# BaeHann/feature_level_style_transfer_for_TSC

Measured on AMD Instinct MI355X. Metric: train-step samples/sec (univariate TS, len=512, batch=256) at 1/2/4/8 MI355X, higher is better.
Workload: dtype bf16x3

## Files before the change

### feature_level_style_transfer_for_tsc_amd/_lib.py

```python
from __future__ import annotations

import ctypes
import os
from ctypes import POINTER, Structure, c_char_p, c_float, c_int, c_int32, c_int64, c_void_p
from typing import Optional

import torch

ABI_VERSION = 16
_LIB_NAME = "libfst_hip.so"
_HERE = os.path.dirname(os.path.abspath(__file__))
LIB_PATH = os.environ.get("FST_HIP_LIB", os.path.join(_HERE, _LIB_NAME))


class FstLibraryError(RuntimeError):
    pass


class WSrc(Structure):
    _fields_ = [("w", c_void_p), ("off0", c_int64), ("sm", c_int64), ("sc", c_int64), ("st", c_int64)]


_P = c_void_p
_I32P = c_void_p
_SIGNATURES = {
    "fst_version": (c_int, []),
    "fst_last_error": (c_char_p, []),
    "fst_pack_weights": (c_int, [_I32P, _I32P, c_int, POINTER(WSrc), POINTER(WSrc), c_int, c_int, c_int, c_int, _P, c_void_p]),
    "fst_pack_weights_bf16x3": (c_int, [_I32P, _I32P, c_int, POINTER(WSrc), POINTER(WSrc), c_int, c_int, c_int, c_int, _P, c_void_p]),
    "fst_unpack_weights": (c_int, [_I32P, _I32P, c_int, _P, c_int, _P, c_int64, c_int64, c_int64, c_int64,
                                   _P, c_int64, c_int64, c_int64, c_int64, c_int, c_void_p]),
    "fst_mask_taps": (c_int, [_P, _I32P, _I32P, c_int, c_int, c_int, c_void_p]),
    "fst_conv_gemm": (c_int, [_P, c_int64, _P, c_int64, _P, _I32P, _I32P, c_int, _P, _P, c_int64, _P, c_int64,
                              _P, c_int64, c_int, c_int, c_int, c_int, c_int, c_int, c_int, c_int, c_void_p]),
    "fst_conv_wgrad": (c_int, [_P, c_int64, _P, c_int64, _P, c_int64, _P, c_int64, c_int, _P, _I32P, _I32P, c_int,
                               c_int, c_int, c_int, c_int, c_int, c_int64, c_void_p]),
    "fst_conv_last_route": (c_int, [POINTER(c_int32)]),
    "fst_row_sum": (c_int, [_P, c_int64, c_int, c_int, c_int, _P, c_void_p]),
    "fst_bn_stats": (c_int, [_P, c_int, c_int, c_int, _P, c_int64, c_void_p]),
    "fst_bn_finalize": (c_int, [_P, c_int, _P, _P, _P, _P, c_int, c_int, c_float, c_float, _P, c_void_p]),
    "fst_bn_apply": (c_int, [_P, _P, _P, _P, _P, c_int, c_int, c_int, c_int, c_int64, c_void_p]),
    "fst_bn_bwd_reduce": (c_int, [_P, _P, _P, _P, c_int, c_int, c_int, c_int, _P, c_int64, c_void_p]),
    "fst_bn_bwd_apply": (c_int, [_P, _P, _P, _P, _P, c_int, _P, _P, _P, c_int, c_int, c_int, c_int, c_int, c_int, c_int64, c_void_p]),
    "fst_bn_bwd_reduce_join": (c_int, [_P, _P, _P, _P, _P, c_int, c_int, c_int, _P, _P, c_int64, c_void_p]),
    "fst_bn_bwd_apply_join": (c_int, [_P, _P, _P, _P, _P, _P, _P, c_int, _P, _P, _P, _P, _P, _P, c_int, c_int, c_int, c_int, c_int,
                                      c_int64, c_void_p]),
    "fst_gate_fwd": (c_int, [_P, _P, c_int, c_int, c_int, c_int64, c_void_p]),
    "fst_gate_bwd": (c_int, [_P, _P, _P, c_int, c_int, c_int, c_int64, c_void_p]),
    "fst_coupling_sum_slots": (c_int64, [c_int, c_int, c_int]),
    "fst_coupling_fwd": (c_int, [_P, _P, _P, c_int, c_int, c_int, c_int64, _P, c_void_p]),
    "fst_coupling_bwd": (c_int, [_P, _P, _P, _P, _P, _P, _P, _P, c_int, c_int, c_int, c_int64, c_void_p]),
    "fst_coupling_inv_fwd": (c_int, [_P, _P, _P, c_int, c_int, c_int, c_int64, c_void_p]),
    "fst_coupling_inv_bwd": (c_int, [_P, _P, _P, _P, _P, c_int, c_int, c_int, c_int64, c_void_p]),
    "fst_rmsprop_multi": (c_int, [_P, _P, _P, _P, _P, c_int, c_float, c_float, c_void_p]),
    "fst_adam_multi": (c_int, [_P, _P, _P, _P, _P, c_int, _P, c_float, c_float, c_float, c_float, c_void_p]),
    "fst_rmsprop_multi_dev": (c_int, [_P, _P, _P, _P, _P, c_int, c_float, c_float, c_void_p]),
    "fst_adam_multi_dev": (c_int, [_P, _P, _P, _P, _P, c_int, _P, _P, c_float, c_float, c_float, c_void_p]),
    "fst_wn_stack_fwd_ok": (c_int, [c_int, c_int, c_int, c_int]),
    "fst_wn_stack_fwd": (c_int, [_P, _P, _P, c_int64, _P, _P, _P, c_int64, _P, c_int, c_int, c_int, c_int, c_int, c_int64, c_void_p]),
    "fst_wn_stack_bwd_ok": (c_int, [c_int, c_int, c_int, c_int]),
    "fst_wn_stack_bwd": (c_int, [_P, _P, _P, _P, _P, _P, _P, _P, _P, c_int64, c_int, c_int, c_int, c_int, c_int, c_int64, c_void_p]),
    "fst_wn_wgrad_ok": (c_int, [c_int, c_int, c_int, c_int, c_int, c_int]),
    "fst_wn_wgrad_workspace_floats": (c_int64, [c_int, c_int, c_int, c_int, c_int, c_int]),
    "fst_wn_wgrad_in": (c_int, [_P, _P, _P, c_int, c_int64, _P, _P, _P, c_int64, c_int, c_int, c_int, c_int, c_int, c_int, c_int64,
                                c_void_p]),
    "fst_wn_wgrad_rs": (c_int, [_P, _P, _P, c_int, _P, _P, c_int64, c_int, c_int, c_int, c_int, c_int64, c_void_p]),
    "fst_nt_gemm_workspace_floats": (c_int64, [c_int, c_int, c_int]),
    "fst_nt_gemm": (c_int, [_P, _P, _P, _P, c_int64, c_int, c_int, c_int, _P, _P, c_int, c_float, _P, c_void_p]),
    "fst_tap_wgrad_ok": (c_int, [c_int, c_int, c_int, c_int, c_int, c_int, c_int]),
    "fst_tap_wgrad_workspace_floats": (c_int64, [c_int, c_int, c_int, c_int, c_int]),
    "fst_tap_wgrad": (c_int, [_P, _P, _P, _P, c_int64, c_int, c_int, c_int, c_int, c_int, c_int, c_int, c_int, c_int64, c_int64, c_void_p]),
    "fst_dense_tap_wgrad_ok": (c_int, [c_int, c_int, c_int, c_int, c_int, c_int]),
    "fst_dense_tap_wgrad_workspace_floats": (c_int64, [c_int, c_int, c_int, c_int, c_int]),
    "fst_dense_tap_wgrad": (c_int, [_P, _P, _P, _P, c_int64, c_int, c_int, c_int, c_int, c_int, c_int, c_int64, c_int64, c_void_p]),
    "fst_wn_last_route": (c_int, [POINTER(c_int32)]),
    "fst_relu_bwd": (c_int, [_P, _P, _P, c_int64, c_void_p]),
    "fst_gemm_workspace_floats": (c_int64, [c_int, c_int, c_int]),
    "fst_gemm": (c_int, [_P, c_int64, c_int, _P, c_int64, c_int, _P, c_int64, c_int, c_int, c_int, _P, c_int, c_float, _P, c_int64,
                         c_void_p]),
    "fst_act_bwd": (c_int, [_P, _P, _P, c_int64, c_float, c_void_p]),
    "fst_batch_sum": (c_int, [_P, _P, _P, c_int, c_int64, c_int, c_void_p]),
    "fst_noise_transfer_fwd": (c_int, [_P, c_int, c_int, _P, _P, c_float, c_float, _P, _P, _P, _P, _P, _P, _P, c_int, c_int, c_void_p]),
    "fst_bcast_add": (c_int, [_P, _P, _P, c_int, c_int64, c_void_p]),
    "fst_noise_transfer_bwd": (c_int, [_P, c_int, _P, _P, _P, _P, c_int, c_int, c_void_p]),
    "fst_noise_transfer_dw": (c_int, [_P, _P, _P, _P, c_int, c_int, c_void_p]),
    "fst_noise_transfer_bwd_apply": (c_int, [_P, _P, _P, _P, c_float, c_float, c_int, _P, _P, c_int64, c_void_p]),
    "fst_wn_fold_fwd": (c_int, [_P, c_int, _P, _P, c_void_p]),
    "fst_wn_fold_bwd": (c_int, [_P, c_int, _P, _P, _P, c_void_p]),
    "fst_logdet_inv": (c_int, [_P, c_int, _P, _P, c_void_p]),
    "fst_wn_image_bytes": (c_int64, [c_int, c_int]),
    "fst_wn_pack": (c_int, [_P, _P, _P, _P, _P, _P, c_int, c_int, c_int, c_int, _P, c_int64, c_void_p]),
    "fst_wn_layer_fwd": (c_int, [_P, c_int64, _P, c_int64, _P, c_int64, _P, _P, _P, _P, c_int, c_int, c_int, c_int, c_int, c_int,
                                 c_int, c_int64, c_void_p]),
    "fst_wn_bwd_image_bytes": (c_int64, [c_int, c_int]),
    "fst_wn_pack_bwd": (c_int, [_P, c_int, c_int, c_int, _P, c_int64, c_void_p]),
    "fst_wn_layer_bwd": (c_int, [_P, _P, _P, _P, c_int64, _P, _P, c_int64, c_int, c_int, c_int, c_int, c_int64, c_void_p]),
    "fst_wn_dgrad_image_bytes": (c_int64, [c_int]),
    "fst_wn_pack_dgrad": (c_int, [_P, _P, c_int, c_int, c_int, _P, c_int64, c_void_p]),
    "fst_wn_dgrad_fits": (c_int, [c_int, c_int, c_int]),
    "fst_wn_layer_dgrad": (c_int, [_P, _P, c_int64, _P, _P, _P, _P, c_int64, c_int, c_int, c_int, c_int, c_int, c_int64, c_int64,
                                   c_void_p]),
    "fst_gru_fwd": (c_int, [_P, _P, _P, _P, _P, _I32P, c_int, c_int, c_int, c_int, c_int64, c_void_p]),
    "fst_gru_bwd": (c_int, [_P, _P, _P, _P, _I32P, c_int, _P, _P, c_int, c_int, c_int, c_int64, c_void_p]),
    "fst_lstm2_fwd": (c_int, [_P, _P, _P, _P, c_int, c_int, c_int64, c_void_p]),
    "fst_lstm2_bwd": (c_int, [_P, _P, _P, _P, _P, c_int, c_int, c_int64, c_void_p]),
    "fst_axpy": (c_int, [_P, _P, c_float, c_int64, c_void_p]),
    "fst_add_slices": (c_int, [_P, c_int64, _P, c_int64, _P, c_int64, c_int, c_int, c_int, c_void_p]),
    "fst_cpc_workspace_floats": (c_int64, [c_int, c_int, c_int, c_int]),
    "fst_cpc_nce_slots": (c_int64, [c_int, c_int, c_int, c_int]),
    "fst_cpc_nce_fwd": (c_int, [_P, c_int64, c_int64, c_int64, _I32P, _P, c_int, c_int, c_int, c_int, c_int, _P, _P, _P, c_void_p]),
    "fst_cpc_nce_bwd": (c_int, [_P, c_int64, c_int64, c_int64, _I32P, _P, _P, c_int, c_int, c_int, c_int, c_int, _P, _P, _P,
                                c_void_p]),
}
EXPORTED_SYMBOLS = tuple(_SIGNATURES)

_lib: Optional[ctypes.CDLL] = None


def load(path: Optional[str] = None) -> ctypes.CDLL:
    global _lib
    if _lib is not None and path is None:
        return _lib
    p = path or LIB_PATH
    if not os.path.exists(p):
        raise FstLibraryError(
            f"{p} not found — build it with `python -c 'import __graft_entry__ as g; g.build()'` "
            "(hipcc --offload-arch=gfx950).  There is no CPU fallback.")
    try:
        lib = ctypes.CDLL(p)
    except OSError as e:
        raise FstLibraryError(f"cannot load {p}: {e}") from e
    for name, (res, args) in _SIGNATURES.items():
        try:
            fn = getattr(lib, name)
        except AttributeError as e:
            raise FstLibraryError(f"{p} does not export {name}; rebuild the library") from e
        fn.restype, fn.argtypes = res, args
    if lib.fst_version() != ABI_VERSION:
        raise FstLibraryError(f"{p}: ABI version {lib.fst_version()} != expected {ABI_VERSION}; rebuild")
    if path is None:
        _lib = lib
    return lib


def check(rc: int, what: str) -> None:
    if rc != 0:
        msg = load().fst_last_error()
        raise RuntimeError(f"{what} failed (rc={rc}): {msg.decode() if msg else '?'}")


def stream_ptr() -> int:
    return torch.cuda.current_stream().cuda_stream


def ptr(t: Optional[torch.Tensor]) -> Optional[int]:
    return None if t is None else t.data_ptr()


def require_gpu_tensor(t: torch.Tensor, name: str) -> None:
    if not t.is_cuda:
        raise FstLibraryError(f"{name} lives on {t.device}; the fst ops run on an MI355X only (no CPU fallback)")
    if t.dtype != torch.float32:
        raise TypeError(f"{name} must be float32, got {t.dtype}")
```

### feature_level_style_transfer_for_tsc_amd/csrc/wn_fused.hip

```cpp
#include "fst_device.h"
#include <type_traits>

#define WS_MAXL 10
#define WN_TN 128
#define WN_A_BYTES (8 * 2048)
#define WN_TILE_BYTES (32 * 36 * 4)
#define WN_FWD_LDS(NW) (3 * (WN_A_BYTES + 2 * (((NW) + 1) * 1024 + 128)))

__device__ __forceinline__ float wn_sigmoid(float x) {
  return __builtin_amdgcn_rcpf(1.0f + __builtin_amdgcn_exp2f(-1.44269504f * x));
}
__device__ __forceinline__ float wn_tanh(float x) {
  return 1.0f - 2.0f * __builtin_amdgcn_rcpf(1.0f + __builtin_amdgcn_exp2f(2.88539008f * x));
}

constexpr int WN_GRP = 2;
__host__ __device__ __forceinline__ void wn_stage_chunk_tap(int k, int CH, int& c, int& tap) {
  const int g = k / (3 * WN_GRP), rem = k - g * 3 * WN_GRP;
  const int gs = CH - g * WN_GRP < WN_GRP ? CH - g * WN_GRP : WN_GRP;
  tap = rem / gs;
  c = g * WN_GRP + rem - gs * tap;
}

struct WnPackParams {
  const float* in_w;
  const float* cond_w;
  const float* in_b;
  const float* cond_b;
  const float* rs_w;
  const float* rs_b;
  int n, h, last, CH, CH2;
  uint4* img;
};

__global__ __launch_bounds__(64) void wn_pack_kernel(WnPackParams p) {
  const int lane = threadIdx.x, blk = blockIdx.x & 7, st = blockIdx.x >> 3;
  const int S1 = 3 * p.CH + p.CH2, n = p.n, h = p.h;
  const int hh = lane >> 5, rowb = (blk & 3) * 32 + (lane & 31);
  const bool row_ok = rowb < n;
  float v[8];
  if (st < S1) {
    const int row = (blk < 4 ? 0 : n) + rowb;
#pragma unroll
    for (int j = 0; j < 8; ++j) {
      float w = 0.f;
      if (row_ok) {
        if (st < 3 * p.CH) {
          int cc, tap;
          wn_stage_chunk_tap(st, p.CH, cc, tap);
          const int c = cc * 16 + 8 * hh + j;
          if (c < n) w = p.in_w[((long long)row * n + c) * 3 + tap];
        } else {
          const int c = (st - 3 * p.CH) * 16 + 8 * hh + j;
          if (c < h) w = p.cond_w[(long long)row * h + c];
          else if (c == h) w = p.in_b[row] + p.cond_b[row];
        }
      }
      v[j] = w;
    }
  } else {
    const int ks = st - S1, kb = ks >> 1, s = ks & 1;
    const bool skip = blk >= 4;
    const bool live = row_ok && (!p.last || skip);
    const int row = (skip && !p.last ? n : 0) + rowb;
#pragma unroll
    for (int j = 0; j < 8; ++j) {
      const int k = kb * 32 + 16 * s + 8 * (j >> 2) + 4 * hh + (j & 3);
      float w = 0.f;
      if (live) {
        if (k < n) w = p.rs_w[(long long)row * n + k];
        else if (k == n) w = p.rs_b[row];
      }
      v[j] = w;
    }
  }
  unsigned hi[4], lo[4];
#pragma unroll
  for (int j = 0; j < 4; ++j) split_bf16_pair(v[2 * j], v[2 * j + 1], hi[j], lo[j]);
  uint4* dst = p.img + ((long long)st * 8 + blk) * 128 + lane;
  dst[0] = make_uint4(hi[0], hi[1], hi[2], hi[3]);
  dst[64] = make_uint4(lo[0], lo[1], lo[2], lo[3]);
  if (blockIdx.x == 0 && lane < 2) {
    const unsigned one = lane ? 0x3f800000u : 0u;
    p.img[(long long)(S1 + 8) * 8 * 128 + lane] = make_uint4(one, one, one, one);
  }
}

static inline int wn_ch(int n) { return (n + 15) / 16; }
static inline int wn_ch2(int h) { return (h + 1 + 15) / 16; }

extern "C" int64_t fst_wn_image_bytes(int n, int h) {
  if (n <= 0 || h <= 0) return -1;
  return (int64_t)(3 * wn_ch(n) + wn_ch2(h) + 8) * WN_A_BYTES + 32;
}

extern "C" int fst_wn_pack(const float* in_w, const float* cond_w, const float* in_b, const float* cond_b,
                           const float* rs_w, const float* rs_b, int n, int h, int ntaps, int last, void* image,
                           int64_t image_bytes, void* stream) {
  FST_REQUIRE(in_w && cond_w && in_b && cond_b && rs_w && rs_b && image, "fst_wn_pack: null operand");
  FST_REQUIRE(ntaps == 3, "fst_wn_pack: the fused WN kernels are 3-tap (in_w [2n][n][3]); got %d taps", ntaps);
  FST_REQUIRE(n > 0 && n < 128 && h > 0, "fst_wn_pack: needs 0 < n < 128 (one spare K row carries the bias), h > 0; n=%d h=%d", n, h);
  FST_REQUIRE(image_bytes == fst_wn_image_bytes(n, h), "fst_wn_pack: image is %lld bytes, expected %lld",
              (long long)image_bytes, (long long)fst_wn_image_bytes(n, h));
  FST_REQUIRE(fst_aligned16(image), "fst_wn_pack: image must be 16-byte aligned");
  WnPackParams p = {in_w, cond_w, in_b, cond_b, rs_w, rs_b, n, h, last ? 1 : 0, wn_ch(n), wn_ch2(h), static_cast<uint4*>(image)};
  const int stages = 3 * p.CH + p.CH2 + 8;
  hipLaunchKernelGGL(wn_pack_kernel, dim3((unsigned)(stages * 8)), dim3(64), 0, (hipStream_t)stream, p);
  FST_LAUNCH_CHECK();
  return 0;
}

#ifdef FST_STAMPS
__device__ unsigned long long wn_stamps[12];
extern "C" int fst_debug_wn_stamps(unsigned long long* out_host, int reset) { return fst_read_stamps(wn_stamps, out_host, reset); }
#endif

struct WnFwdParams {
  const float* a;
  long long a_bs;
  const float* u0;
  long long u0_bs;
  const char* img;
  float* ts;
  float* acts;
  float* a_next;
  float* out;
  int B, L, n, h, dil, first, last;
  int CH, CH2, tiles_per_seq, n_wg;
};

template <int MODE>
__device__ __forceinline__ void wn_store_tile(const float (&v)[16], float* tile, float* dst_rows, const float* res_rows,
                                              int rows_valid, int L, int t, int lane) {
  const int half = lane >> 5, l31 = lane & 31;
#pragma unroll
  for (int r = 0; r < 16; ++r) tile[((r & 3) + 8 * (r >> 2) + 4 * half) * 36 + l31] = v[r];
  const int rrow = lane >> 3, c4 = (lane & 7) * 4;
  const bool t_ok = t + c4 < L;
  float4 o[4], e[4];
#pragma unroll
  for (int j = 0; j < 4; ++j) {
    const int row = rrow + 8 * j;
    o[j] = *reinterpret_cast<const float4*>(tile + row * 36 + c4);
    e[j] = make_float4(0.f, 0.f, 0.f, 0.f);
    if (MODE != 0 && t_ok && row < rows_valid) {
      const float* src = (MODE == 1 ? res_rows : dst_rows) + (long long)row * L + t + c4;
      e[j] = *reinterpret_cast<const float4*>(src);
    }
  }
#pragma unroll
  for (int j = 0; j < 4; ++j) {
    const int row = rrow + 8 * j;
    if (t_ok && row < rows_valid) {
      float4 w = o[j];
      w.x += e[j].x; w.y += e[j].y; w.z += e[j].z; w.w += e[j].w;
      *reinterpret_cast<float4*>(dst_rows + (long long)row * L + t + c4) = w;
    }
  }
}

__device__ __forceinline__ void wn_fetch_tile(float4 (&q)[4], const float* src_rows, int rows_valid, int L, int t, int lane) {
  const int rrow = lane >> 3, c4 = (lane & 7) * 4;
  const bool t_ok = t + c4 < L;
#pragma unroll
  for (int j = 0; j < 4; ++j) {
    const int row = rrow + 8 * j;
    q[j] = make_float4(0.f, 0.f, 0.f, 0.f);
    if (t_ok && row < rows_valid) q[j] = *reinterpret_cast<const float4*>(src_rows + (long long)row * L + t + c4);
  }
}
__device__ __forceinline__ void wn_acc_load(f32x16& v, const float* src_rows, int rows_valid, int L, int t, int lane) {
  const int half = lane >> 5, l31 = lane & 31;
  const bool t_ok = t + l31 < L && src_rows != nullptr;
  const float* lp = src_rows + ((long long)(4 * half) * L + t + l31);
  const int rv = rows_valid - 4 * half;
#pragma unroll
  for (int r = 0; r < 16; ++r) {
    const int row = (r & 3) + 8 * (r >> 2);
    v[r] = (t_ok && row < rv) ? lp[(long long)row * L] : 0.f;
  }
}
__device__ __forceinline__ void wn_acc_store(const f32x16& v, float* dst_rows, int rows_valid, int L, int t, int lane) {
  const int half = lane >> 5, l31 = lane & 31;
  const bool t_ok = t + l31 < L;
  float* lp = dst_rows + ((long long)(4 * half) * L + t + l31);
  const int rv = rows_valid - 4 * half;
#pragma unroll
  for (int r = 0; r < 16; ++r) {
    const int row = (r & 3) + 8 * (r >> 2);
    if (t_ok && row < rv) lp[(long long)row * L] = v[r];
  }
}
__device__ __forceinline__ void wn_acc_store(const float (&v)[16], float* dst_rows, int rows_valid, int L, int t, int lane) {
  const int half = lane >> 5, l31 = lane & 31;
  const bool t_ok = t + l31 < L;
  float* lp = dst_rows + ((long long)(4 * half) * L + t + l31);
  const int rv = rows_valid - 4 * half;
#pragma unroll
  for (int r = 0; r < 16; ++r) {
    const int row = (r & 3) + 8 * (r >> 2);
    if (t_ok && row < rv) lp[(long long)row * L] = v[r];
  }
}
__device__ __forceinline__ void wn_tile_to_acc(float (&v)[16], const float4 (&q)[4], float* tile, int lane) {
  const int rrow = lane >> 3, c4 = (lane & 7) * 4, half = lane >> 5, l31 = lane & 31;
#pragma unroll
  for (int j = 0; j < 4; ++j) *reinterpret_cast<float4*>(tile + (rrow + 8 * j) * 36 + c4) = q[j];
#pragma unroll
  for (int r = 0; r < 16; ++r) v[r] = tile[((r & 3) + 8 * (r >> 2) + 4 * half) * 36 + l31];
}

#define WS_OOB 0x80000000u
__device__ __forceinline__ __amdgpu_buffer_rsrc_t ws_rsrc(const void* base) {
  return __builtin_amdgcn_make_buffer_rsrc(const_cast<void*>(base), 0, 0x40000000, 0x00020000);
}
struct WsLane { unsigned vo, vo_lo; };
__device__ __forceinline__ WsLane ws_lane(unsigned vlane, int tcol, int L, int lane) {
  WsLane w;
  w.vo = tcol + (lane & 31) < L ? vlane : WS_OOB;
  w.vo_lo = lane < 32 ? w.vo : WS_OOB;
  return w;
}
__device__ __forceinline__ int ws_opaque(int x) {
  asm volatile("" : "+s"(x));
  return x;
}
__device__ __forceinline__ void ws_acc_load(f32x16& v, __amdgpu_buffer_rsrc_t rs, const WsLane w, int row0, int tcol, int rv, int L) {
  L = ws_opaque(L);
  rv = ws_opaque(rv);
  const int sbase = (row0 * L + tcol) * 4;
  if (rv >= 32) {
#pragma unroll
    for (int r = 0; r < 16; ++r)
      v[r] = __builtin_bit_cast(float, __builtin_amdgcn_raw_buffer_load_b32(rs, w.vo, sbase + ((r & 3) + 8 * (r >> 2)) * L * 4, 0));
  } else {
#pragma unroll
    for (int r = 0; r < 16; ++r) {
      const int row = (r & 3) + 8 * (r >> 2);
      float x = 0.f;
      if (row < rv) x = __builtin_bit_cast(float, __builtin_amdgcn_raw_buffer_load_b32(rs, row + 4 < rv ? w.vo : w.vo_lo, sbase + row * L * 4, 0));
      v[r] = x;
    }
  }
}
template <class V>
__device__ __forceinline__ void ws_acc_store(const V& v, __amdgpu_buffer_rsrc_t rs, const WsLane w, int row0, int tcol, int rv, int L) {
  L = ws_opaque(L);
  rv = ws_opaque(rv);
  const int sbase = (row0 * L + tcol) * 4;
  if (rv >= 32) {
#pragma unroll
    for (int r = 0; r < 16; ++r)
      __builtin_amdgcn_raw_buffer_store_b32(__builtin_bit_cast(unsigned, (float)v[r]), rs, w.vo, sbase + ((r & 3) + 8 * (r >> 2)) * L * 4, 0);
  } else {
#pragma unroll
    for (int r = 0; r < 16; ++r) {
      const int row = (r & 3) + 8 * (r >> 2);
      if (row < rv)
        __builtin_amdgcn_raw_buffer_store_b32(__builtin_bit_cast(unsigned, (float)v[r]), rs, row + 4 < rv ? w.vo : w.vo_lo, sbase + row * L * 4, 0);
    }
// ... 224 lines not shown
#pragma unroll
    for (int mb = 0; mb < 8; ++mb) {
      if (mb + 1 < 8 && !(p.last && mb + 1 < 4)) a_frag(mb + 1);
      if (!(p.last && mb < 4)) mfma_bf3(acc[mb], fah[mb % 2], fal[mb % 2], bh2[ks], bl2[ks]);
      if (more && mb >= 4) {
        __builtin_amdgcn_sched_barrier(0);
        issue_piece(nxt, mb - 4);
        __builtin_amdgcn_sched_barrier(0);
      }
    }
    slot = slot == 2 ? 0 : slot + 1;
  }

  FST_T(tg2);
  FST_ACC(7, tg1, tg2);
#pragma unroll
  for (int blk = 0; blk < 4; ++blk) {
    const int rows_e = n - blk * 32;
    if (!p.last) ws_acc_store(acc[blk], an_rs, wl, blk * 32, tcol, rows_e, L);
    ws_acc_store(acc[blk + 4], out_rs, wl, blk * 32, tcol, rows_e, L);
  }
  FST_T(tg3);
  FST_ACC(8, tg2, tg3);
  FST_ACC(9, ts0, tg3);
  FST_FLUSH(wn_stamps);
}

template <int NW>
__global__ __launch_bounds__(64 * NW, NW == 4 ? 2 : 1) void wn_layer_fwd_kernel(WnFwdParams p) {
  extern __shared__ __attribute__((aligned(16))) float lds[];
  int wg = blockIdx.x;
  if ((p.n_wg & 7) == 0) wg = (wg & 7) * (p.n_wg >> 3) + (wg >> 3);
  const int b = wg / p.tiles_per_seq;
  const int t0 = (wg - b * p.tiles_per_seq) * (32 * NW);
  wn_fwd_tile<NW>(*(WnFwdArgs*)__builtin_amdgcn_kernarg_segment_ptr(), b, t0, reinterpret_cast<char*>(lds));
}

struct WnFwdStackParams {
  WnFwdParams layer[WS_MAXL];
  int nl;
};

__global__ __launch_bounds__(512, 1) void wn_stack_fwd_kernel(WnFwdStackParams ps_by_value) {
  extern __shared__ __attribute__((aligned(16))) float lds[];
  typedef const __attribute__((address_space(4))) WnFwdStackParams StackArgs;
  StackArgs& ps = *(StackArgs*)__builtin_amdgcn_kernarg_segment_ptr();
  (void)ps_by_value;
  char* const ldsb = reinterpret_cast<char*>(lds);
  const int B = ps.layer[0].B, passes = ps.layer[0].tiles_per_seq;
  for (int b = blockIdx.x; b < B; b += gridDim.x) {
    for (int layer = 0; layer < ps.nl; ++layer) {
      for (int pass = 0; pass < passes; ++pass) {
        WnFwdArgs* qp = &ps.layer[layer];
        asm volatile("" : "+s"(qp));
        wn_fwd_tile<8>(*qp, b, pass * 256, ldsb);
        wait_vmcnt<0>();
        __syncthreads();
      }
    }
  }
}

extern "C" int fst_wn_stack_fwd_ok(int n, int h, int L, int nl) {
  return n > 0 && n < 128 && h > 0 && L > 0 && L % 256 == 0 && nl >= 1 && nl <= WS_MAXL;
}

extern "C" int fst_wn_stack_fwd(const float* const* a_in, const int64_t* a_bs, const void* const* images, int64_t image_bytes,
                                float* const* ts, float* const* a_next, const float* u0, int64_t u0_bs, float* out, int nl, int B,
                                int L, int n, int h, int64_t numel_a, void* stream) {
  fst_wn_clear_route();
  FST_REQUIRE(a_in && a_bs && images && ts && a_next && u0 && out, "fst_wn_stack_fwd: null operand");
  FST_REQUIRE(fst_wn_stack_fwd_ok(n, h, L, nl) && B > 0, "fst_wn_stack_fwd: B=%d L=%d n=%d h=%d nl=%d (needs n < 128, L %% 256 == 0, "
              "1 <= nl <= %d)", B, L, n, h, nl, WS_MAXL);
  FST_REQUIRE((long long)B * n * L == (long long)numel_a, "fst_wn_stack_fwd: B*n*L = %d*%d*%d does not match the element count %lld "
              "of the [B, n, L] tensors", B, n, L, (long long)numel_a);
  FST_REQUIRE(image_bytes == fst_wn_image_bytes(n, h), "fst_wn_stack_fwd: images are %lld bytes, expected %lld",
              (long long)image_bytes, (long long)fst_wn_image_bytes(n, h));
  FST_REQUIRE(B == 1 || u0_bs >= (int64_t)h * L, "fst_wn_stack_fwd: batch stride of u0 smaller than a sample");
  FST_REQUIRE(u0_bs % 4 == 0 && fst_aligned16(u0) && fst_aligned16(out), "fst_wn_stack_fwd: needs 16-byte aligned tensors");
  WnFwdStackParams p = {};
  for (int i = 0; i < nl; ++i) {
    FST_REQUIRE(a_in[i] && images[i] && ts[i] && (a_next[i] || i == nl - 1), "fst_wn_stack_fwd: null operand of layer %d", i);
    FST_REQUIRE(a_bs[i] >= (int64_t)n * L && a_bs[i] % 4 == 0 && fst_aligned16(a_in[i]) && fst_aligned16(images[i]) && fst_aligned16(ts[i]) && fst_aligned16(a_next[i]),
                "fst_wn_stack_fwd: layer %d: batch stride %lld smaller than a sample, or an operand that is not 16-byte aligned", i,
                (long long)a_bs[i]);
    FST_REQUIRE(i == nl - 1 || a_in[i + 1] == a_next[i], "fst_wn_stack_fwd: the input of layer %d is not the a_next of layer %d",
                i + 1, i);
    WnFwdParams& q = p.layer[i];
    q.a = a_in[i]; q.a_bs = a_bs[i]; q.u0 = u0; q.u0_bs = u0_bs; q.img = static_cast<const char*>(images[i]);
    q.ts = ts[i]; q.acts = nullptr; q.a_next = i == nl - 1 ? nullptr : a_next[i]; q.out = out;
    q.B = B; q.L = L; q.n = n; q.h = h; q.dil = 1 << i; q.first = i == 0; q.last = i == nl - 1;
    q.CH = wn_ch(n); q.CH2 = wn_ch2(h); q.tiles_per_seq = L / 256; q.n_wg = 0;
  }
  p.nl = nl;
  const int cus = fst_cu_count_or(256);
  if (int rc = fst_allow_full_lds((const void*)wn_stack_fwd_kernel, "fst_wn_stack_fwd")) return rc;
  fst_wn_set_route(FST_WN_ROUTE_STACK_FWD, 8, 0, 0, 0, B < cus ? B : cus, 1, 1, L / 256, 3, nl, WN_FWD_LDS(8));
  hipLaunchKernelGGL(wn_stack_fwd_kernel, dim3((unsigned)(B < cus ? B : cus)), dim3(512), WN_FWD_LDS(8), (hipStream_t)stream, p);
  FST_LAUNCH_CHECK();
  return 0;
}

extern "C" int fst_wn_layer_fwd(const float* a, int64_t a_bs, const float* u0, int64_t u0_bs, const void* image,
                                int64_t image_bytes, float* ts, float* acts, float* a_next, float* out, int first, int last,
                                int B, int L, int n, int h, int dil, int64_t numel_a, void* stream) {
  fst_wn_clear_route();
  FST_REQUIRE(a && u0 && image && ts && out && (last || a_next), "fst_wn_layer_fwd: null operand");
  FST_REQUIRE(B > 0 && L > 0 && n > 0 && n < 128 && h > 0 && dil > 0, "fst_wn_layer_fwd: B=%d L=%d n=%d h=%d dil=%d (needs n < 128)",
              B, L, n, h, dil);
  FST_REQUIRE((long long)B * n * L == (long long)numel_a, "fst_wn_layer_fwd: B*n*L = %d*%d*%d does not match the element count %lld "
              "of the [B, n, L] tensors", B, n, L, (long long)numel_a);
  FST_REQUIRE(image_bytes == fst_wn_image_bytes(n, h), "fst_wn_layer_fwd: image is %lld bytes, expected %lld",
              (long long)image_bytes, (long long)fst_wn_image_bytes(n, h));
  FST_REQUIRE(B == 1 || (a_bs >= (int64_t)n * L && u0_bs >= (int64_t)h * L), "fst_wn_layer_fwd: batch stride smaller than a sample");
  FST_REQUIRE(L % 4 == 0 && a_bs % 4 == 0 && u0_bs % 4 == 0 && fst_aligned16(a) && fst_aligned16(u0) && fst_aligned16(image) && fst_aligned16(ts) && fst_aligned16(acts) &&
              fst_aligned16(a_next) && fst_aligned16(out), "fst_wn_layer_fwd: needs L %% 4 == 0 and 16-byte aligned tensors (L=%d)", L);
  WnFwdParams p;
  p.a = a; p.a_bs = a_bs; p.u0 = u0; p.u0_bs = u0_bs; p.img = static_cast<const char*>(image);
  p.ts = ts; p.acts = acts; p.a_next = a_next; p.out = out;
  p.B = B; p.L = L; p.n = n; p.h = h; p.dil = dil; p.first = first ? 1 : 0; p.last = last ? 1 : 0;
  p.CH = wn_ch(n); p.CH2 = wn_ch2(h);
  const int cus = fst_cu_count_or(256);
  const int nw = (L % 256 == 0 && (long long)B * (L / 256) >= cus) ? 8 : 4;
  const int tn = 32 * nw;
  p.tiles_per_seq = (L + tn - 1) / tn;
  p.n_wg = B * p.tiles_per_seq;
  if (nw == 8) {
    if (int rc = fst_allow_full_lds((const void*)wn_layer_fwd_kernel<8>, "fst_wn_layer_fwd")) return rc;
    fst_wn_set_route(FST_WN_ROUTE_LAYER_FWD, 8, 0, 0, 0, p.n_wg, 1, 1, p.tiles_per_seq, 3, 1, WN_FWD_LDS(8));
    hipLaunchKernelGGL(wn_layer_fwd_kernel<8>, dim3((unsigned)p.n_wg), dim3(512), WN_FWD_LDS(8), (hipStream_t)stream, p);
  } else {
    if (int rc = fst_allow_full_lds((const void*)wn_layer_fwd_kernel<4>, "fst_wn_layer_fwd")) return rc;
    fst_wn_set_route(FST_WN_ROUTE_LAYER_FWD, 4, 0, 0, 0, p.n_wg, 1, 1, p.tiles_per_seq, 3, 1, WN_FWD_LDS(4));
    hipLaunchKernelGGL(wn_layer_fwd_kernel<4>, dim3((unsigned)p.n_wg), dim3(256), WN_FWD_LDS(4), (hipStream_t)stream, p);
  }
  FST_LAUNCH_CHECK();
  return 0;
}

constexpr int WN_BWD_OCC = 2;
#define WN_BW_NB 4
#define WN_BW_GS (WN_BW_NB * 1024 + 128)
#define WN_BW_A (4 * 2048)
#define WN_BW_SLOT (WN_BW_A + 2 * WN_BW_GS)
#define WN_BW_LDS (3 * WN_BW_SLOT)

struct WnPackBwdParams {
  const float* rs_w;
  int n, last, CH;
  uint4* img;
  int acc_order;
};

__global__ __launch_bounds__(64) void wn_pack_bwd_kernel(WnPackBwdParams p) {
  const int lane = threadIdx.x, blk = blockIdx.x & 3, st = blockIdx.x >> 2;
  const int n = p.n, hh = lane >> 5, m = blk * 32 + (lane & 31);
  const int src = p.last ? 0 : st / p.CH, c = st - src * p.CH;
  float v[8];
#pragma unroll
  for (int j = 0; j < 8; ++j) {
    const bool perm = p.acc_order && !p.last && src == 0;
    const int ch = 16 * c + (perm ? 8 * (j >> 2) + 4 * hh + (j & 3) : 8 * hh + j);
    v[j] = (m < n && ch < n) ? p.rs_w[(long long)(src * n + ch) * n + m] : 0.f;
  }
  unsigned hi[4], lo[4];
#pragma unroll
  for (int j = 0; j < 4; ++j) split_bf16_pair(v[2 * j], v[2 * j + 1], hi[j], lo[j]);
  uint4* dst = p.img + ((long long)st * 4 + blk) * 128 + lane;
  dst[0] = make_uint4(hi[0], hi[1], hi[2], hi[3]);
  dst[64] = make_uint4(lo[0], lo[1], lo[2], lo[3]);
  if (blockIdx.x == 0 && lane == 0) p.img[(long long)gridDim.x * 128] = make_uint4(0u, 0u, 0u, 0u);
}

extern "C" int64_t fst_wn_bwd_image_bytes(int n, int last) {
  if (n <= 0) return -1;
  return (int64_t)(last ? 1 : 2) * wn_ch(n) * WN_BW_A + 16;
}

extern "C" int fst_wn_pack_bwd(const float* rs_w, int n, int last, int acc_order, void* image, int64_t image_bytes, void* stream) {
  FST_REQUIRE(rs_w && image && n > 0 && n <= 128, "fst_wn_pack_bwd: bad arguments (n=%d, needs n <= 128)", n);
  FST_REQUIRE(image_bytes == fst_wn_bwd_image_bytes(n, last), "fst_wn_pack_bwd: image is %lld bytes, expected %lld",
              (long long)image_bytes, (long long)fst_wn_bwd_image_bytes(n, last));
  FST_REQUIRE(fst_aligned16(image), "fst_wn_pack_bwd: image must be 16-byte aligned");
  WnPackBwdParams p = {rs_w, n, last ? 1 : 0, wn_ch(n), static_cast<uint4*>(image), acc_order ? 1 : 0};
  const int stages = (last ? 1 : 2) * p.CH;
  hipLaunchKernelGGL(wn_pack_bwd_kernel, dim3((unsigned)(stages * 4)), dim3(64), 0, (hipStream_t)stream, p);
  FST_LAUNCH_CHECK();
  return 0;
}

struct WnBwdParams {
  const float* d_a;
  const float* d_out;
  const float* ts;
  const char* img;
  float* dg;
  float* row_sums;
  int B, L, n, last, CH, tiles_per_seq, n_wg;
};

__device__ __forceinline__ void wn_bwd_multiply(f32x16 (&acc)[4], const char* base, int lane, bf16x8 bh, bf16x8 bl) {
#pragma unroll
  for (int mb = 0; mb < 4; ++mb) {
    bf16x8 ah, al;
    lds_read_a_frag(base, mb, lane, ah, al);
    mfma_bf3(acc[mb], ah, al, bh, bl);
  }
}

__device__ __forceinline__ void wn_reduce_row_sums(const float* rsum, int R, float* out, int stride, int col, int tid) {
  __syncthreads();
  if (tid < R) {
    float s8 = 0.f;
#pragma unroll
    for (int w = 0; w < 8; ++w) s8 += rsum[w * R + tid];
    out[(long long)tid * stride + col] = s8;
  }
}

__global__ __launch_bounds__(256, WN_BWD_OCC) void wn_layer_bwd_kernel(WnBwdParams p) {
  extern __shared__ __attribute__((aligned(16))) float lds[];
  char* const ldsb = reinterpret_cast<char*>(lds);
  const int tid = threadIdx.x, lane = tid & 63;
  const int half = lane >> 5, l31 = lane & 31;
  const int wave_s = __builtin_amdgcn_readfirstlane(tid >> 6);
  int wg = blockIdx.x;
  if ((p.n_wg & 7) == 0) wg = (wg & 7) * (p.n_wg >> 3) + (wg >> 3);
  const int b = wg / p.tiles_per_seq;
  const int t0 = (wg - b * p.tiles_per_seq) * WN_TN;
  const int wave_n0 = wave_s * 32;
  const int L = p.L, n = p.n, CH = p.CH;
  const int S3 = (p.last ? 1 : 2) * CH;
  const char* const zero16 = p.img + (long long)S3 * WN_BW_A;
  const float* const ts_b = p.ts + (long long)b * (2 * n) * L;
  const int tcol = t0 + wave_n0;

  auto issue = [&](int k, int slot) {
    char* const sl = ldsb + slot * WN_BW_SLOT;
    const char* asrc = p.img + (long long)k * WN_BW_A;
    const bool from_da = !p.last && k < CH;
    const int c = from_da ? k : k - (p.last ? 0 : CH);
    const float* xb = (from_da ? p.d_a : p.d_out) + ((long long)b * n + 16 * c) * L;
    const int c_count = min(16, n - 16 * c);
#pragma unroll
    for (int i = 0; i < 4; ++i) {
      const int idx = wave_s + 4 * i;
      if (idx < 8) {
        lds_dma16(asrc + idx * 1024 + lane * 16, sl + idx * 1024);
      } else {
        const int bi = idx - 8;
        const int gq = bi >> 2, m = bi & 3;
        const int row = 8 * gq + (lane >> 3);
        const int t = t0 + 32 * m + 4 * (lane & 7);
        const bool ok = row < c_count && t < L;
        const char* src = ok ? reinterpret_cast<const char*>(xb + ((long long)row * L + t)) : zero16;
        lds_dma16(src, sl + WN_BW_A + gq * WN_BW_GS + m * 1024);
      }
    }
  };

  f32x16 acc[4];
#pragma unroll
  for (int mb = 0; mb < 4; ++mb)
#pragma unroll
    for (int r = 0; r < 16; ++r) acc[mb][r] = 0.f;

  float4 qt[4], qs[4];
  wn_fetch_tile(qt, ts_b, n, L, tcol, lane);
  wn_fetch_tile(qs, ts_b + (long long)n * L, n, L, tcol, lane);
  asm volatile("" ::: "memory");
  issue(0, 0);
  if (S3 > 1) issue(1, 1);
  int slot = 0;
  for (int k = 0; k < S3; ++k) {
    if (k + 1 < S3) wait_vmcnt<4>(); else wait_vmcnt<0>();
    __builtin_amdgcn_s_barrier();
    if (k + 2 < S3) issue(k + 2, slot >= 1 ? slot - 1 : 2);
    const char* base = ldsb + slot * WN_BW_SLOT;
    const int colx = wave_n0 + l31;
    const char* bp = base + WN_BW_A + half * WN_BW_GS + (colx >> 5) * 1024 + (colx & 31) * 4;
    float v[8];
#pragma unroll
    for (int j = 0; j < 8; ++j) v[j] = *reinterpret_cast<const float*>(bp + j * 128);
    bf16x8 bh, bl;
    split_bf16x8(v, bh, bl);
    wn_bwd_multiply(acc, base, lane, bh, bl);
    slot = slot == 2 ? 0 : slot + 1;
  }
  __syncthreads();
  float* const tile = reinterpret_cast<float*>(ldsb + wave_s * WN_TILE_BYTES);
  float* const rsum = reinterpret_cast<float*>(ldsb + 4 * WN_TILE_BYTES);
  float* const rsum_w = rsum + wave_s * 256;
  if (p.row_sums) {
#pragma unroll
    for (int w = 0; w < 4; ++w) rsum[w * 256 + tid] = 0.f;
    __syncthreads();
  }
  float* const dg_b = p.dg + (long long)b * (2 * n) * L;
#pragma unroll
  for (int blk = 0; blk < 4; ++blk) {
    const int rows_valid = n - blk * 32;
    float tv[16], sv[16], gt[16], gs[16];
    wn_tile_to_acc(tv, qt, tile, lane);
    wn_tile_to_acc(sv, qs, tile, lane);
    if (blk < 3) {
      wn_fetch_tile(qt, ts_b + (long long)((blk + 1) * 32) * L, n - (blk + 1) * 32, L, tcol, lane);
      wn_fetch_tile(qs, ts_b + (long long)(n + (blk + 1) * 32) * L, n - (blk + 1) * 32, L, tcol, lane);
    }
#pragma unroll
    for (int r = 0; r < 16; ++r) {
      const float d = acc[blk][r], t = tv[r], s = sv[r];
      gt[r] = d * s * (1.f - t * t);
      gs[r] = d * t * s * (1.f - s);
    }
    wn_store_tile<0>(gt, tile, dg_b + (long long)(blk * 32) * L, nullptr, rows_valid, L, tcol, lane);
    if (p.row_sums) wn_tile_row_sums(tile, rsum_w, blk * 32, rows_valid, L, tcol, lane);
    wn_store_tile<0>(gs, tile, dg_b + (long long)(n + blk * 32) * L, nullptr, rows_valid, L, tcol, lane);
    if (p.row_sums) wn_tile_row_sums(tile, rsum_w, n + blk * 32, rows_valid, L, tcol, lane);
  }
  if (p.row_sums) {
    __syncthreads();
    p.row_sums[(long long)tid * p.n_wg + wg] = (rsum[tid] + rsum[256 + tid]) + (rsum[512 + tid] + rsum[768 + tid]);
  }
}

extern "C" int fst_wn_layer_bwd(const float* d_a, const float* d_out, const float* ts, const void* image, int64_t image_bytes,
                                float* dg, float* row_sums, int64_t row_sums_rows, int last, int B, int L, int n,
                                int64_t numel_a, void* stream) {
  fst_wn_clear_route();
  FST_REQUIRE(d_out && ts && image && dg && (last || d_a), "fst_wn_layer_bwd: null operand");
  FST_REQUIRE(B > 0 && L > 0 && n > 0 && n <= 128, "fst_wn_layer_bwd: B=%d L=%d n=%d (needs n <= 128)", B, L, n);
  FST_REQUIRE((long long)B * n * L == (long long)numel_a, "fst_wn_layer_bwd: B*n*L = %d*%d*%d does not match the element count %lld "
              "of the [B, n, L] tensors", B, n, L, (long long)numel_a);
  FST_REQUIRE(image_bytes == fst_wn_bwd_image_bytes(n, last), "fst_wn_layer_bwd: image is %lld bytes, expected %lld",
              (long long)image_bytes, (long long)fst_wn_bwd_image_bytes(n, last));
  FST_REQUIRE(L % 4 == 0 && fst_aligned16(d_a) && fst_aligned16(d_out) && fst_aligned16(ts) && fst_aligned16(image) && fst_aligned16(dg),
              "fst_wn_layer_bwd: needs L %% 4 == 0 and 16-byte aligned tensors (L=%d)", L);
  WnBwdParams p;
  p.d_a = last ? nullptr : d_a; p.d_out = d_out; p.ts = ts; p.img = static_cast<const char*>(image); p.dg = dg;
  p.row_sums = row_sums;
  p.B = B; p.L = L; p.n = n; p.last = last ? 1 : 0; p.CH = wn_ch(n);
  p.tiles_per_seq = (L + WN_TN - 1) / WN_TN;
  p.n_wg = B * p.tiles_per_seq;
  FST_REQUIRE(row_sums == nullptr || row_sums_rows == p.n_wg, "fst_wn_layer_bwd: row_sums has %lld rows, the launch has %d "
              "workgroups (B x ceil(L/128))", (long long)row_sums_rows, p.n_wg);
  if (int rc = fst_allow_full_lds((const void*)wn_layer_bwd_kernel, "fst_wn_layer_bwd")) return rc;
  fst_wn_set_route(FST_WN_ROUTE_LAYER_BWD, 0, 0, 0, 0, p.n_wg, 1, 1, p.tiles_per_seq, 3, 1, WN_BW_LDS);
  hipLaunchKernelGGL(wn_layer_bwd_kernel, dim3((unsigned)p.n_wg), dim3(256), WN_BW_LDS, (hipStream_t)stream, p);
  FST_LAUNCH_CHECK();
  return 0;
}

#define DG_NCB 2
#define DG_TN (8 * 32 * DG_NCB)
#define DG_A_BLOCKS 13
#define DG_A_BYTES (DG_A_BLOCKS * 2048)

struct WnPackDgradParams {
  const float* in_w;
  const float* cond_w;
  int n, h, CHK;
  uint4* img;
};

__global__ __launch_bounds__(64) void wn_pack_dgrad_kernel(WnPackDgradParams p) {
  const int lane = threadIdx.x, ab = blockIdx.x % DG_A_BLOCKS, c = blockIdx.x / DG_A_BLOCKS;
  const int n = p.n, h = p.h, hh = lane >> 5, l31 = lane & 31;
  int tap, blk;
  if (ab < 4) { tap = 0; blk = ab; } else if (ab < 9) { tap = 1; blk = ab - 4; } else { tap = 2; blk = ab - 9; }
  float v[8];
#pragma unroll
  for (int j = 0; j < 8; ++j) {
    const int k = 16 * c + 8 * hh + j;
    float w = 0.f;
    if (k < 2 * n) {
      if (blk < 4) {
        const int m = blk * 32 + l31;
        if (m < n) w = p.in_w[((long long)k * n + m) * 3 + tap];
      } else {
        if (l31 < h) w = p.cond_w[(long long)k * h + l31];
      }
    }
    v[j] = w;
  }
  unsigned hi[4], lo[4];
#pragma unroll
  for (int j = 0; j < 4; ++j) split_bf16_pair(v[2 * j], v[2 * j + 1], hi[j], lo[j]);
  uint4* dst = p.img + (long long)blockIdx.x * 128 + lane;
  dst[0] = make_uint4(hi[0], hi[1], hi[2], hi[3]);
  dst[64] = make_uint4(lo[0], lo[1], lo[2], lo[3]);
  if (blockIdx.x == 0 && lane == 0) p.img[(long long)gridDim.x * 128] = make_uint4(0u, 0u, 0u, 0u);
}

extern "C" int64_t fst_wn_dgrad_image_bytes(int n) {
  if (n <= 0) return -1;
  return (int64_t)((2 * n + 15) / 16) * DG_A_BYTES + 16;
}

extern "C" int fst_wn_pack_dgrad(const float* in_w, const float* cond_w, int n, int h, int ntaps, void* image, int64_t image_bytes,
                                 void* stream) {
  FST_REQUIRE(in_w && cond_w && image && n > 0 && n <= 128 && h > 0 && h <= 32, "fst_wn_pack_dgrad: needs n <= 128, h <= 32 (n=%d h=%d)", n, h);
  FST_REQUIRE(ntaps == 3, "fst_wn_pack_dgrad: the fused WN kernels are 3-tap (in_w [2n][n][3]); got %d taps", ntaps);
  FST_REQUIRE(image_bytes == fst_wn_dgrad_image_bytes(n), "fst_wn_pack_dgrad: image is %lld bytes, expected %lld",
              (long long)image_bytes, (long long)fst_wn_dgrad_image_bytes(n));
  FST_REQUIRE(fst_aligned16(image), "fst_wn_pack_dgrad: image must be 16-byte aligned");
  WnPackDgradParams p = {in_w, cond_w, n, h, (2 * n + 15) / 16, static_cast<uint4*>(image)};
  hipLaunchKernelGGL(wn_pack_dgrad_kernel, dim3((unsigned)(p.CHK * DG_A_BLOCKS)), dim3(64), 0, (hipStream_t)stream, p);
  FST_LAUNCH_CHECK();
  return 0;
}

__device__ __forceinline__ void wn_dgrad_issue(char* sl, const char* img, const float* dg_b, int c, int t0, int n, int L, int dil,
                                               int nblkw, int gsw, int wave_s, int lane) {
  const char* asrc = img + (long long)c * DG_A_BYTES;
  const char* const zero16 = img + (long long)((2 * n + 15) / 16) * DG_A_BYTES;
  const float* xb = dg_b + (long long)(16 * c) * L;
  const int c_count = min(16, 2 * n - 16 * c);
  const int w4 = (t0 - dil) & ~3;
  const int NI = DG_A_BLOCKS * 2 + 2 * nblkw;
  for (int idx = wave_s; idx < NI; idx += 8) {
    if (idx < 2 * DG_A_BLOCKS) {
      lds_dma16(asrc + idx * 1024 + lane * 16, sl + idx * 1024);
    } else {
      const int bi = idx - 2 * DG_A_BLOCKS;
      const int gq = bi >= nblkw ? 1 : 0, m = bi - gq * nblkw;
      const int row = 8 * gq + (lane >> 3);
      const int t = w4 + 32 * m + 4 * (lane & 7);
      const bool ok = row < c_count && t >= 0 && t < L;
      const char* src = ok ? reinterpret_cast<const char*>(xb + ((long long)row * L + t)) : zero16;
      lds_dma16(src, sl + DG_A_BYTES + gq * gsw + m * 1024);
    }
  }
}

__device__ __forceinline__ void wn_dgrad_stage(f32x16 (&acc)[5][DG_NCB], const char* base, int gsw, int wave_n0, int dil, int sub,
                                               int lane) {
  const int half = lane >> 5, l31 = lane & 31;
#pragma unroll
  for (int tap = 0; tap < 3; ++tap) {
    bf16x8 bh[DG_NCB], bl[DG_NCB];
#pragma unroll
    for (int cb = 0; cb < DG_NCB; ++cb) {
      const int colx = wave_n0 + 32 * cb + l31 + (2 - tap) * dil + sub;
      const char* bp = base + DG_A_BYTES + half * gsw + (colx >> 5) * 1024 + (colx & 31) * 4;
      float v8[8];
#pragma unroll
      for (int j = 0; j < 8; ++j) v8[j] = *reinterpret_cast<const float*>(bp + j * 128);
      split_bf16x8(v8, bh[cb], bl[cb]);
    }
    const char* ab = base + (tap == 0 ? 0 : (tap == 1 ? 4 : 9)) * 2048;
#pragma unroll
    for (int mb = 0; mb < 5; ++mb) {
      if (mb == 4 && tap != 1) continue;
      bf16x8 ah, al;
      lds_read_a_frag(ab, mb, lane, ah, al);
#pragma unroll
      for (int cb = 0; cb < DG_NCB; ++cb) mfma_bf3(acc[mb][cb], ah, al, bh[cb], bl[cb]);
    }
  }
}

struct WnDgradParams {
  const float* dg;
  const char* img;
  const float* d_a;
  float* d_a_new;
  float* d_u0;
  long long d_u0_bs;
  float* row_sums;
  int B, L, n, h, dil, CHK, tiles_per_seq, n_wg;
  int nblkw;
  int gsw;
  int slot;
  int ns;
};

template <int N>
__device__ __forceinline__ void wn_wait_sw(int n) {
  if (n == N) { wait_vmcnt<N>(); return; }
  if constexpr (N > 0) wn_wait_sw<N - 1>(n);
}

__global__ __launch_bounds__(512, 2) void wn_layer_dgrad_kernel(WnDgradParams p) {
  extern __shared__ __attribute__((aligned(16))) float lds[];
  char* const ldsb = reinterpret_cast<char*>(lds);
  const int tid = threadIdx.x, lane = tid & 63;
  const int half = lane >> 5, l31 = lane & 31;
  const int wave_s = __builtin_amdgcn_readfirstlane(tid >> 6);
  const int wave_n0 = wave_s * (32 * DG_NCB);
  const int L = p.L, n = p.n, CHK = p.CHK, dil = p.dil;
  const int NI = DG_A_BLOCKS * 2 + 2 * p.nblkw;
  const int my_pieces = (NI - wave_s + 7) >> 3;
  const int depth = p.ns - 1;

  auto tile_of = [&](int v, int& b, int& t0) {
    int wg = v;
    if ((p.n_wg & 7) == 0) wg = (wg & 7) * (p.n_wg >> 3) + (wg >> 3);
    b = wg / p.tiles_per_seq;
    t0 = (wg - b * p.tiles_per_seq) * DG_TN;
    return wg;
  };
  auto issue = [&](int b, int t0, int c, int slot) {
    wn_dgrad_issue(ldsb + slot * p.slot, p.img, p.dg + (long long)b * (2 * n) * L, c, t0, n, L, dil, p.nblkw, p.gsw, wave_s, lane);
  };

  int first_slot = 0;
  for (int v = blockIdx.x; v < p.n_wg; v += gridDim.x) {
    int b, t0;
    const int wg = tile_of(v, b, t0);
    const int sub = (t0 - dil) & 3;
    f32x16 acc[5][DG_NCB];
#pragma unroll
    for (int mb = 0; mb < 5; ++mb)
#pragma unroll
      for (int cb = 0; cb < DG_NCB; ++cb) {
        const float* src = mb < 4 ? (p.d_a ? p.d_a + ((long long)b * n + mb * 32) * L : nullptr) : p.d_u0 + (long long)b * p.d_u0_bs;
        const int rows = mb < 4 ? (p.d_a ? n - mb * 32 : 0) : p.h;
        wn_acc_load(acc[mb][cb], src, rows, L, t0 + wave_n0 + 32 * cb, lane);
      }
    if (first_slot == 0)
      for (int d = 0; d < depth && d < CHK; ++d) issue(b, t0, d, d);

    int slot = first_slot;
    for (int c = 0; c < CHK; ++c) {
      const int newer = min(depth - 1, CHK - 1 - c);
      wn_wait_sw<16>(newer * my_pieces);
      __builtin_amdgcn_s_barrier();
      if (c + depth < CHK) issue(b, t0, c + depth, (slot + depth) % p.ns);
      wn_dgrad_stage(acc, ldsb + slot * p.slot, p.gsw, wave_n0, dil, sub, lane);
      slot = slot + 1 == p.ns ? 0 : slot + 1;
    }
    __syncthreads();
    if (v + (int)gridDim.x < p.n_wg) {
      int bn, tn;
      tile_of(v + gridDim.x, bn, tn);
      for (int d = 0; d < depth && d < CHK; ++d) issue(bn, tn, d, 1 + d);
      first_slot = 1;
    }
    float* const tile = reinterpret_cast<float*>(ldsb + wave_s * WN_TILE_BYTES);
    float* const rsum = reinterpret_cast<float*>(ldsb + 8 * WN_TILE_BYTES);
    float* const rsum_w = rsum + wave_s * 128;
    if (p.row_sums) {
      rsum[tid] = 0.f; rsum[512 + tid] = 0.f;
      __syncthreads();
    }
#pragma unroll
    for (int k = 0; k < 5 * DG_NCB; ++k) {
      const int i = k / DG_NCB, cb = k % DG_NCB, tcol = t0 + wave_n0 + 32 * cb;
      float* dst = i < 4 ? p.d_a_new + ((long long)b * n + i * 32) * L : p.d_u0 + (long long)b * p.d_u0_bs;
      const int rows = i < 4 ? n - i * 32 : p.h;
      wn_acc_store(acc[i][cb], dst, rows, L, tcol, lane);
      if (p.row_sums && i < 4) {
#pragma unroll
        for (int r = 0; r < 16; ++r) tile[((r & 3) + 8 * (r >> 2) + 4 * half) * 36 + l31] = acc[i][cb][r];
        wn_tile_row_sums(tile, rsum_w, i * 32, rows, L, tcol, lane);
      }
    }
    if (p.row_sums) wn_reduce_row_sums(rsum, 128, p.row_sums, p.n_wg, wg, tid);
  }
}
// ... 349 lines not shown
```

### feature_level_style_transfer_for_tsc_amd/csrc/wn_wgrad.hip

```cpp
#include <stdlib.h>
#include <type_traits>

#include "fst_device.h"

#define WW_TT 32
#define WW_MROWS 256
#define WW_ND 3
#define WW_NX 2
#define WW_MAX_NX 5

__device__ __attribute__((aligned(16))) float ww_zero16[4] = {0.f, 0.f, 0.f, 0.f};

#define WW_MAX_SETS 3
struct WwSeg {
  const float* ptr[WW_MAX_SETS];
  long long bs;
  long long mul_off;
  int rows, shift;
  int out, out_off, out_sc, out_sm;
};

struct WwParams {
  WwSeg dy[2];
  WwSeg x[4];
// ... 239 lines not shown
      const int nxu = (p.xr * 4 > 512 + tid) ? 2 : 1;
#pragma unroll
      for (int i = 0; i < 2; ++i) {
        const int r = r0 + 128 * i;
        da[i][0] = dw + ww_lds_off(r, 2 * u); da[i][1] = dw + ww_lds_off(r, 2 * u + 1);
        d[i][0] = ww_lds_read16(ww_lds_addr(da[i][0])); d[i][1] = ww_lds_read16(ww_lds_addr(da[i][1]));
        xa[i][0] = xw + ww_lds_off(r, 2 * u); xa[i][1] = xw + ww_lds_off(r, 2 * u + 1);
        if (i < nxu && r < p.xr) {
          xq[i][0] = ww_lds_read16(ww_lds_addr(xa[i][0])); xq[i][1] = ww_lds_read16(ww_lds_addr(xa[i][1]));
          if constexpr (MUL) {
            xm[i][0] = ww_lds_read16(ww_lds_addr(xa[i][0] + (p.xr << 7))); xm[i][1] = ww_lds_read16(ww_lds_addr(xa[i][1] + (p.xr << 7)));
          }
        }
      }
      ww_lds_wait();
#pragma unroll
      for (int i = 0; i < 2; ++i) {
        const int r = r0 + 128 * i;
        if constexpr (NE > 0)
          ev[i] += (d[i][0].x * e0.x + d[i][0].y * e0.y) + (d[i][0].z * e0.z + d[i][0].w * e0.w) +
                   (d[i][1].x * e1.x + d[i][1].y * e1.y) + (d[i][1].z * e1.z + d[i][1].w * e1.w);
        u32x4 h4, l4;
        ww_split8u(d[i][0], d[i][1], h4, l4);
        ww_lds_write16(ww_lds_addr(da[i][0]), h4); ww_lds_write16(ww_lds_addr(da[i][1]), l4);
        if (i < nxu && r < p.xr) {
          if constexpr (MUL) { xq[i][0] *= xm[i][0]; xq[i][1] *= xm[i][1]; }
          ww_split8u(xq[i][0], xq[i][1], h4, l4);
          ww_lds_write16(ww_lds_addr(xa[i][0]), h4); ww_lds_write16(ww_lds_addr(xa[i][1]), l4);
        }
      }
      asm volatile("s_waitcnt lgkmcnt(0)" ::: "memory");
    }
    __builtin_amdgcn_s_barrier();
#pragma unroll
    for (int ks = 0; ks < 2; ++ks) {
      f32x4 araw[MT][2], braw[KT][2];
#pragma unroll
      for (int i = 0; i < MT; ++i) {
        const char* ap = dsl + a_off + ((i * 32) << 7);
        araw[i][0] = ww_lds_read16(ww_lds_addr(ap + pc[ks][0]));
        araw[i][1] = ww_lds_read16(ww_lds_addr(ap + pc[ks][1]));
      }
#pragma unroll
      for (int j = 0; j < KT; ++j) {
        const char* bp = xsl + x_off + ((j * 32) << 7);
        braw[j][0] = ww_lds_read16(ww_lds_addr(bp + pc[ks][0]));
        braw[j][1] = ww_lds_read16(ww_lds_addr(bp + pc[ks][1]));
      }
      ww_lds_wait();
      issue_pos(5 * ks);
#pragma unroll
      for (int j = 0; j < KT; ++j) {
        if (FULL || wk * KT + j < k_blocks_here) {
          const bf16x8 bh = __builtin_bit_cast(bf16x8, braw[j][0]), bl = __builtin_bit_cast(bf16x8, braw[j][1]);
#pragma unroll
          for (int i = 0; i < MT; ++i) {
            if (!FULL && wm * MT + i >= m_blocks) break;
            const bf16x8 ah = __builtin_bit_cast(bf16x8, araw[i][0]), al = __builtin_bit_cast(bf16x8, araw[i][1]);
            mfma_bf3(acc[i][j], ah, al, bh, bl);
          }
        }
        issue_pos(5 * ks + 1 + j);
      }
      if constexpr (KT < 3) issue_pos(5 * ks + 3);
      issue_pos(5 * ks + 4);
    }
    dslot = dslot == WW_ND - 1 ? 0 : dslot + 1;
    xslot ^= 1;
  }

  float* const slab = p.slab + (long long)blockIdx.x * WW_MROWS * p.Kcols;
#pragma unroll
  for (int i = 0; i < MT; ++i) {
    if (wm * MT + i >= m_blocks) break;
#pragma unroll
    for (int j = 0; j < KT; ++j) {
      if (wk * KT + j >= k_blocks_here) break;
      float* dst = slab + (long long)((wm * MT + i) * 32 + 4 * half) * p.Kcols + g * p.xr + (wk * KT + j) * 32 + l31;
#pragma unroll
      for (int r = 0; r < 16; ++r) dst[(long long)((r & 3) + 8 * (r >> 2)) * p.Kcols] = acc[i][j][r];
    }
  }
  if (do_extra) {
#pragma unroll
    for (int i = 0; i < 2; ++i) {
      float sv = ev[i];
      sv += __shfl_xor(sv, 1, 64);
      sv += __shfl_xor(sv, 2, 64);
      if ((tid & 3) == 0) p.slab_extra[((long long)blockIdx.x * WW_MROWS + (tid >> 2) + 128 * i) * 2] = sv;
    }
  }
}

__device__ __forceinline__ void ww_scatter(const WwParams& p, int m, int kk, float v) {
  int si = 0, c = kk;
#pragma unroll
  for (int j = 0; j < 3; ++j)
    if (si + 1 < p.n_x && c >= p.x[si].rows) { c -= p.x[si].rows; ++si; }
  int out = p.x[0].out, off = p.x[0].out_off, sc = p.x[0].out_sc, sm = p.x[0].out_sm;
  if (si == 1) { out = p.x[1].out; off = p.x[1].out_off; sc = p.x[1].out_sc; sm = p.x[1].out_sm; }
  if (si == 2) { out = p.x[2].out; off = p.x[2].out_off; sc = p.x[2].out_sc; sm = p.x[2].out_sm; }
  if (si == 3) { out = p.x[3].out; off = p.x[3].out_off; sc = p.x[3].out_sc; sm = p.x[3].out_sm; }
  float* w = out == 0 ? p.w[0] : p.w[1];
  const long long at = (long long)m * sm + (long long)c * sc + off;
  if (p.epi_p) {
    float sd = 0.f;
    for (int j = 0; j < p.epi_ncls; ++j) sd += p.epi_p[m * p.epi_ncls + j] * p.epi_r1[(long long)j * sm + c];
    if (p.epi_raw) p.epi_raw[at] = v;
    v = v * p.epi_scale * sd;
  }
  w[at] = v;
}

__global__ __launch_bounds__(256) void wn_wgrad_reduce_kernel(WwParams p) {
  __shared__ float4 part[4][64];
  const int m = blockIdx.y, cx = threadIdx.x & 63, sg = threadIdx.x >> 6;
  const int kk0 = blockIdx.x * 256 + cx * 4;
  float4 s = make_float4(0.f, 0.f, 0.f, 0.f);
  if (kk0 < p.Kcols) {
    const long long st = (long long)WW_MROWS * p.Kcols;
    const float* q = p.slab + (long long)m * p.Kcols + kk0;
    int sl = sg;
    for (; sl + 28 < p.ksplit; sl += 32) {
      float4 v[8];
#pragma unroll
      for (int u = 0; u < 8; ++u) v[u] = *reinterpret_cast<const float4*>(q + (sl + 4 * u) * st);
#pragma unroll
      for (int u = 0; u < 8; ++u) { s.x += v[u].x; s.y += v[u].y; s.z += v[u].z; s.w += v[u].w; }
    }
    for (; sl < p.ksplit; sl += 4) {
      const float4 v = *reinterpret_cast<const float4*>(q + sl * st);
      s.x += v.x; s.y += v.y; s.z += v.z; s.w += v.w;
    }
  }
  part[sg][cx] = s;
  __syncthreads();
  if (sg == 0 && kk0 < p.Kcols) {
    float4 t = part[0][cx];
#pragma unroll
    for (int g2 = 1; g2 < 4; ++g2) { const float4 o = part[g2][cx]; t.x += o.x; t.y += o.y; t.z += o.z; t.w += o.w; }
    const float tv[4] = {t.x, t.y, t.z, t.w};
#pragma unroll
    for (int j = 0; j < 4; ++j)
      if (kk0 + j < p.K_main) ww_scatter(p, m, kk0 + j, tv[j]);
  }
  if (blockIdx.x == gridDim.x - 1 && sg == 1 && cx < p.n_extra && p.K_main < p.K) {
    const float* q = p.slab_extra + (long long)m * 2 + cx;
    float e = 0.f;
    for (int sl = 0; sl < p.ksplit; ++sl) e += q[(long long)sl * WW_MROWS * 2];
    ww_scatter(p, m, p.K_main + cx, e);
  }
}


static thread_local int32_t g_wn_route[FST_WN_ROUTE_LEN] = {0};

void fst_wn_set_route(int family, int t1, int t2, int t3, int t4, int gx, int gy, int gz, int a8, int a9, int a10, int lds) {
  const int32_t r[FST_WN_ROUTE_LEN] = {family, t1, t2, t3, t4, gx, gy, gz, a8, a9, a10, lds};
  for (int i = 0; i < FST_WN_ROUTE_LEN; ++i) g_wn_route[i] = r[i];
}

extern "C" int fst_wn_last_route(int32_t out[FST_WN_ROUTE_LEN]) {
  FST_REQUIRE(out != nullptr, "fst_wn_last_route: null output");
  for (int i = 0; i < FST_WN_ROUTE_LEN; ++i) out[i] = g_wn_route[i];
  return g_wn_route[0] != 0 ? 0 : -1;
}

static int ww_geometry(int kind, int B, int L, int n, int h, int last, int n_sets, WwParams* p) {
  const int KT = kind == 0 ? 3 : 2;
  p->M = kind == 0 ? 2 * n : (last ? n : 2 * n);
  p->K = kind == 0 ? 3 * n + h : n;
  const int rem = p->K & 31;
  p->n_extra = (kind == 0 && rem == 1) ? 1 : 0;
  p->K_main = p->n_extra ? p->K - rem : p->K;
  p->xr = 32 * 2 * KT;
  const int kb = (p->K_main + 31) / 32;
  p->n_groups = (kb + 2 * KT - 1) / (2 * KT);
  p->mul = kind == 1;
  p->RX = p->xr * (1 + p->mul) + (p->n_extra ? 8 : 0);
  p->Kcols = p->n_groups * p->xr;
  p->B = B; p->L = L;
  p->tiles_per_seq = L / WW_TT;
  p->n_tiles = B * p->tiles_per_seq;
  const int cus = fst_cu_count_or(256);
  int ks = cus / p->n_groups;
  if (ks > p->n_tiles * n_sets) ks = p->n_tiles * n_sets;
  if (ks < n_sets) ks = n_sets;
  p->ksplit = ks;
  p->n_sets = n_sets;
  return KT;
}

extern "C" int fst_wn_wgrad_ok(int kind, int B, int L, int n, int h, int dil) {
  if (!(B > 0 && L > 0 && L % WW_TT == 0 && n > 0 && n < 128)) return 0;
  if (kind == 0) {
    if (!(h > 0 && h <= 32 && dil > 0 && (3 * n + h + 31) / 32 <= 18)) return 0;
    return dil % 4 == 0 ? 1 : (dil < 4 ? 2 : 0);
  }
  return kind == 1;
}

extern "C" int64_t fst_wn_wgrad_workspace_floats(int kind, int B, int L, int n, int h, int last) {
  if (!fst_wn_wgrad_ok(kind, B, L, n, h, 4)) return -1;
  WwParams p;
  ww_geometry(kind, B, L, n, h, last, WW_MAX_SETS, &p);
  return (int64_t)p.ksplit * WW_MROWS * (p.Kcols + 2);
}

static int ww_launch(WwParams& p, int KT, void* stream, bool reduce = true) {
  const size_t lds = (size_t)WW_ND * WW_MROWS * 128 + (size_t)WW_NX * p.RX * 128;
  FST_REQUIRE(lds <= 160 * 1024 && (p.RX >> 3) <= 8 * WW_MAX_NX, "fst_wn_wgrad: %d staged k-rows per stage do not fit (LDS %zu B)", p.RX, lds);
  const bool full = (p.M + 31) / 32 == 8 && ((p.K_main + 31) / 32) % (2 * KT) == 0;
  void (*fn)(WwParams);
  if (KT == 3) {
    if (p.n_extra) fn = full ? wn_wgrad_kernel<2, 3, true, false, 1> : wn_wgrad_kernel<2, 3, false, false, 1>;
    else fn = full ? wn_wgrad_kernel<2, 3, true, false, 0> : wn_wgrad_kernel<2, 3, false, false, 0>;
  } else if (p.mul) {
    fn = full ? wn_wgrad_kernel<2, 2, true, true, 0> : wn_wgrad_kernel<2, 2, false, true, 0>;
  } else {
    fn = full ? wn_wgrad_kernel<2, 2, true, false, 0> : wn_wgrad_kernel<2, 2, false, false, 0>;
  }
  if (int rc = fst_allow_full_lds((const void*)fn, "fst_wn_wgrad")) return rc;
  fst_wn_set_route(FST_WN_ROUTE_WGRAD, KT, (int)full, p.mul, p.n_extra, p.ksplit, p.n_groups, 1, p.n_sets, p.misaligned, (int)reduce, (int)lds);
  hipLaunchKernelGGL(fn, dim3((unsigned)p.ksplit, (unsigned)p.n_groups), dim3(512), lds, (hipStream_t)stream, p);
  FST_LAUNCH_CHECK();
  if (!reduce) return 0;
  hipLaunchKernelGGL(wn_wgrad_reduce_kernel, dim3((unsigned)((p.Kcols + 255) / 256), (unsigned)p.M), dim3(256), 0, (hipStream_t)stream, p);
  FST_LAUNCH_CHECK();
  return 0;
}

extern "C" int fst_wn_wgrad_in(const float* const* dg, const float* const* a, const float* const* u0, int n_sets, int64_t u0_bs,
                               float* dw_in, float* dw_cond, float* workspace, int64_t workspace_floats, int B, int L, int n, int h,
                               int dil, int a_slack, int64_t numel_a, void* stream) {
  fst_wn_clear_route();
  FST_REQUIRE(dg && a && u0 && dw_in && dw_cond && workspace, "fst_wn_wgrad_in: null operand");
  FST_REQUIRE(n_sets >= 1 && n_sets <= WW_MAX_SETS, "fst_wn_wgrad_in: %d operand sets (1..%d)", n_sets, WW_MAX_SETS);
  const int served = fst_wn_wgrad_ok(0, B, L, n, h, dil);
  FST_REQUIRE(served == 1 || (served == 2 && a_slack), "fst_wn_wgrad_in: unsupported shape B=%d L=%d n=%d h=%d dil=%d (needs L %% 32 == 0, "
              "n < 128, h <= 32, and dil %% 4 == 0 or — with 16 readable bytes either side of a — dil < 4)", B, L, n, h, dil);
  FST_REQUIRE((long long)B * n * L == (long long)numel_a, "fst_wn_wgrad_in: B*n*L does not match the element count %lld of a", (long long)numel_a);
  FST_REQUIRE(B == 1 || u0_bs >= (int64_t)h * L, "fst_wn_wgrad_in: u0 batch stride %lld < h*L", (long long)u0_bs);
  FST_REQUIRE(u0_bs % 4 == 0 && fst_aligned16(workspace), "fst_wn_wgrad_in: operands must be 16-byte aligned");
  WwParams p = {};
  const int KT = ww_geometry(0, B, L, n, h, 0, n_sets, &p);
  FST_REQUIRE(workspace_floats >= (int64_t)p.ksplit * WW_MROWS * (p.Kcols + 2), "fst_wn_wgrad_in: workspace of %lld floats is too small",
              (long long)workspace_floats);
  p.n_dy = 1;
  p.dy[0] = {{}, (long long)2 * n * L, 0, 2 * n, 0, 0, 0, 0, 0};
  p.n_x = 4;
  for (int tap = 0; tap < 3; ++tap) p.x[tap] = {{}, (long long)n * L, 0, n, (tap - 1) * dil, 0, tap, 3, 3 * n};
  p.x[3] = {{}, (long long)u0_bs, 0, h, 0, 1, 0, 1, h};
  for (int s = 0; s < n_sets; ++s) {
    FST_REQUIRE(dg[s] && a[s] && u0[s], "fst_wn_wgrad_in: null operand in set %d", s);
    FST_REQUIRE(fst_aligned16(dg[s]) && fst_aligned16(a[s]) && fst_aligned16(u0[s]), "fst_wn_wgrad_in: operands must be 16-byte aligned");
    p.dy[0].ptr[s] = dg[s];
    for (int tap = 0; tap < 3; ++tap) p.x[tap].ptr[s] = a[s];
    p.x[3].ptr[s] = u0[s];
  }
  p.misaligned = dil % 4 != 0;
  p.slab = workspace;
  p.slab_extra = workspace + (long long)p.ksplit * WW_MROWS * p.Kcols;
  p.w[0] = dw_in; p.w[1] = dw_cond;
  return ww_launch(p, KT, stream);
}

extern "C" int fst_wn_wgrad_rs(const float* const* d_a, const float* const* d_out, const float* const* ts, int n_sets, float* dw_rs,
                               float* workspace, int64_t workspace_floats, int last, int B, int L, int n, int64_t numel_a,
                               void* stream) {
  fst_wn_clear_route();
  FST_REQUIRE(d_out && ts && dw_rs && workspace && (last || d_a), "fst_wn_wgrad_rs: null operand");
  FST_REQUIRE(n_sets >= 1 && n_sets <= WW_MAX_SETS, "fst_wn_wgrad_rs: %d operand sets (1..%d)", n_sets, WW_MAX_SETS);
  FST_REQUIRE(fst_wn_wgrad_ok(1, B, L, n, 0, 4), "fst_wn_wgrad_rs: unsupported shape B=%d L=%d n=%d (needs L %% 32 == 0, n < 128)", B, L, n);
  FST_REQUIRE((long long)B * n * L == (long long)numel_a, "fst_wn_wgrad_rs: B*n*L does not match the element count %lld", (long long)numel_a);
  FST_REQUIRE(fst_aligned16(workspace), "fst_wn_wgrad_rs: operands must be 16-byte aligned");
  WwParams p = {};
  const int KT = ww_geometry(1, B, L, n, 0, last, n_sets, &p);
  FST_REQUIRE(workspace_floats >= (int64_t)p.ksplit * WW_MROWS * (p.Kcols + 2), "fst_wn_wgrad_rs: workspace of %lld floats is too small",
              (long long)workspace_floats);
  p.n_dy = last ? 1 : 2;
  p.dy[0] = {{}, (long long)n * L, 0, n, 0, 0, 0, 0, 0};
  p.dy[1] = {{}, (long long)n * L, 0, n, 0, 0, 0, 0, 0};
  p.n_x = 1;
  p.x[0] = {{}, (long long)2 * n * L, (long long)n * L, n, 0, 0, 0, 1, n};
  for (int s = 0; s < n_sets; ++s) {
    FST_REQUIRE(d_out[s] && ts[s] && (last || d_a[s]), "fst_wn_wgrad_rs: null operand in set %d", s);
    FST_REQUIRE(fst_aligned16(d_out[s]) && fst_aligned16(ts[s]) && (last || fst_aligned16(d_a[s])), "fst_wn_wgrad_rs: operands must be 16-byte aligned");
    if (last) p.dy[0].ptr[s] = d_out[s];
    else { p.dy[0].ptr[s] = d_a[s]; p.dy[1].ptr[s] = d_out[s]; }
    p.x[0].ptr[s] = ts[s];
  }
  p.slab = workspace;
  p.slab_extra = workspace + (long long)p.ksplit * WW_MROWS * p.Kcols;
  p.w[0] = dw_rs; p.w[1] = nullptr;
  return ww_launch(p, KT, stream);
}

extern "C" int64_t fst_nt_gemm_workspace_floats(int M, int N, int K) {
  if (!(M > 0 && M <= WW_MROWS && N > 0 && K > 0 && K % WW_TT == 0)) return -1;
  const int n_groups = ((N + 31) / 32 + 3) / 4;
  const int cus = fst_cu_count_or(256);
  int ks = cus / n_groups;
  if (ks > K / WW_TT) ks = K / WW_TT;
  if (ks < 1) ks = 1;
  return (int64_t)ks * WW_MROWS * (n_groups * 128 + 2);
}

extern "C" int fst_nt_gemm(const float* A, const float* Bm, float* C, float* workspace, int64_t workspace_floats, int M, int N, int K,
                           const float* epi_p, const float* epi_r1, int epi_ncls, float epi_scale, float* epi_raw, void* stream) {
  fst_wn_clear_route();
  FST_REQUIRE(A && Bm && C && workspace, "fst_nt_gemm: null operand");
  FST_REQUIRE(M > 0 && M <= WW_MROWS && N > 0 && K > 0 && K % WW_TT == 0, "fst_nt_gemm: M=%d N=%d K=%d (needs M <= 256, K %% 32 == 0)", M, N, K);
  FST_REQUIRE((long long)N * K < (1LL << 31) * 4 && (long long)M * N < (1LL << 31), "fst_nt_gemm: operand too large");
  FST_REQUIRE(fst_aligned16(A) && fst_aligned16(Bm) && fst_aligned16(workspace), "fst_nt_gemm: operands must be 16-byte aligned");
  FST_REQUIRE((epi_p == nullptr) == (epi_r1 == nullptr) && (epi_p == nullptr || epi_ncls > 0) && (epi_p != nullptr || epi_raw == nullptr),
              "fst_nt_gemm: the epilogue takes p [M][ncls] and r1 [ncls][N] together (and the raw product only with them)");
  WwParams p = {};
  p.M = M; p.K = N; p.K_main = N; p.n_extra = 0;
  p.xr = 128;
  p.n_groups = ((N + 31) / 32 + 3) / 4;
  p.mul = 0;
  p.RX = p.xr;
  p.Kcols = p.n_groups * p.xr;
  p.B = 1; p.L = K;
  p.tiles_per_seq = K / WW_TT;
  p.n_tiles = p.tiles_per_seq;
  const int cus = fst_cu_count_or(256);
  int ks = cus / p.n_groups;
  if (ks > p.n_tiles) ks = p.n_tiles;
  if (ks < 1) ks = 1;
  p.ksplit = ks;
  p.n_sets = 1;
  FST_REQUIRE(workspace_floats >= (int64_t)p.ksplit * WW_MROWS * (p.Kcols + 2), "fst_nt_gemm: workspace of %lld floats is too small",
              (long long)workspace_floats);
  p.n_dy = 1;
  p.dy[0] = {{A, nullptr, nullptr}, 0, 0, M, 0, 0, 0, 0, 0};
  p.n_x = 1;
  p.x[0] = {{Bm, nullptr, nullptr}, 0, 0, N, 0, 0, 0, 1, N};
  p.slab = workspace;
  p.slab_extra = workspace + (long long)p.ksplit * WW_MROWS * p.Kcols;
  p.w[0] = C; p.w[1] = nullptr;
  p.epi_p = epi_p; p.epi_r1 = epi_r1; p.epi_ncls = epi_ncls; p.epi_scale = epi_scale; p.epi_raw = epi_raw;
  const bool direct = p.ksplit == 1 && M == WW_MROWS && p.Kcols == N && !epi_p;
  if (direct) p.slab = C;
  return ww_launch(p, 2, stream, !direct);
}

extern "C" int fst_tap_wgrad_ok(int B, int L, int M, int C, int ntaps, int dil, int pad_left) {
  if (!(B > 0 && L > 0 && L % WW_TT == 0 && M > 0 && M <= WW_MROWS && C > 0 && ntaps >= 1 && ntaps <= 4 && dil > 0)) return 0;
  if (((long long)ntaps * C + 31) / 32 > 18) return 0;
  int need_slack = 0;
  for (int tap = 0; tap < ntaps; ++tap) {
    const int sh = tap * dil - pad_left;
    if (sh % 4 != 0) {
      if (sh <= -4 || sh >= 4) return 0;
      need_slack = 1;
    }
  }
  return need_slack ? 2 : 1;
}

static void tap_geometry(int B, int L, int M, int C, int ntaps, WwParams* p) {
  p->M = M; p->K = ntaps * C; p->K_main = p->K; p->n_extra = 0;
  p->xr = 192;
  p->n_groups = ((p->K + 31) / 32 + 5) / 6;
  p->mul = 0;
  p->RX = p->xr;
  p->Kcols = p->n_groups * p->xr;
  p->B = B; p->L = L;
  p->tiles_per_seq = L / WW_TT;
  p->n_tiles = B * p->tiles_per_seq;
  const int cus = fst_cu_count_or(256);
  int ks = cus / p->n_groups;
  if (ks > p->n_tiles) ks = p->n_tiles;
  if (ks < 1) ks = 1;
  p->ksplit = ks;
  p->n_sets = 1;
}

extern "C" int64_t fst_tap_wgrad_workspace_floats(int B, int L, int M, int C, int ntaps) {
  if (!fst_tap_wgrad_ok(B, L, M, C, ntaps, 4, 0)) return -1;
  WwParams p = {};
  tap_geometry(B, L, M, C, ntaps, &p);
  return (int64_t)p.ksplit * WW_MROWS * (p.Kcols + 2);
}

extern "C" int fst_tap_wgrad(const float* dy, const float* x, float* dw, float* workspace, int64_t workspace_floats, int B, int L, int M,
                             int C, int ntaps, int dil, int pad_left, int x_slack, int64_t numel_dy, int64_t numel_x, void* stream) {
  fst_wn_clear_route();
  FST_REQUIRE(dy && x && dw && workspace, "fst_tap_wgrad: null operand");
  const int served = fst_tap_wgrad_ok(B, L, M, C, ntaps, dil, pad_left);
  FST_REQUIRE(served == 1 || (served == 2 && x_slack), "fst_tap_wgrad: unsupported shape B=%d L=%d M=%d C=%d ntaps=%d dil=%d pad_left=%d "
              "(needs L %% 32 == 0, M <= 256, at most 4 taps, tap shifts multiples of 4 or — with 16 readable bytes either side of x — "
              "within 3 samples)", B, L, M, C, ntaps, dil, pad_left);
  FST_REQUIRE((long long)B * M * L == (long long)numel_dy && (long long)B * C * L == (long long)numel_x,
              "fst_tap_wgrad: B*M*L / B*C*L do not match the element counts %lld / %lld", (long long)numel_dy, (long long)numel_x);
  FST_REQUIRE(fst_aligned16(dy) && fst_aligned16(x) && fst_aligned16(workspace), "fst_tap_wgrad: operands must be 16-byte aligned");
  WwParams p = {};
  tap_geometry(B, L, M, C, ntaps, &p);
  FST_REQUIRE(workspace_floats >= (int64_t)p.ksplit * WW_MROWS * (p.Kcols + 2), "fst_tap_wgrad: workspace of %lld floats is too small",
              (long long)workspace_floats);
  p.n_dy = 1;
  p.dy[0] = {{dy, nullptr, nullptr}, (long long)M * L, 0, M, 0, 0, 0, 0, 0};
  p.n_x = ntaps;
  p.misaligned = 0;
  for (int tap = 0; tap < ntaps; ++tap) {
    const int sh = tap * dil - pad_left;
    p.x[tap] = {{x, nullptr, nullptr}, (long long)C * L, 0, C, sh, 0, tap, ntaps, C * ntaps};
    if (sh % 4 != 0) p.misaligned = 1;
  }
  p.slab = workspace;
  p.slab_extra = workspace + (long long)p.ksplit * WW_MROWS * p.Kcols;
  p.w[0] = dw; p.w[1] = nullptr;
  return ww_launch(p, 3, stream);
}

#define TZ_CPB 288
#define TZ_XRAW 1024
#define TZ_ND 4

struct TzParams {
  const float* dy;
  const float* x;
  float* slab;
  float* dw;
  int B, L, M, C, K, P4;
  int off0;
  int n_groups, ksplit, tiles_per_seq, n_tiles, Kcols;
  int m_halves;
};

#ifdef FST_STAMPS
__device__ unsigned long long tz_stamps[12];
extern "C" int fst_debug_tz_stamps(unsigned long long* out_host, int reset) { return fst_read_stamps(tz_stamps, out_host, reset); }
#endif


template <int MP, bool FULL>
__global__ __launch_bounds__(512, 2) void tz_wgrad_kernel(TzParams p) {
  constexpr int CW = 8 / MP;
  constexpr int NDW = MP == 2 ? 2 : 1;
  constexpr int DSLOT = (MP == 2 ? 128 : 64) * 128;
  constexpr int XSLOT = CW * TZ_XRAW;
  constexpr int LO = CW * 8 * TZ_CPB, COPIES = 2 * LO;
  constexpr int X0 = TZ_ND * DSLOT, C0 = X0 + TZ_ND * XSLOT;
  constexpr int XU = (128 * CW) / 512;
  extern __shared__ __attribute__((aligned(16))) char tz_lds[];
  const unsigned lds0 = ww_lds_addr(tz_lds);
// ... 296 lines not shown
```

### feature_level_style_transfer_for_tsc_amd/ops.py

```python
from __future__ import annotations

import ctypes
import math
import os
from typing import Dict, List, Optional, Sequence, Tuple

import torch

from . import _lib
from . import dist as _dist
from ._lib import WSrc, check, ptr, stream_ptr
from .plan import Plan, Segment, build_plan, pick_mb

EPI_RELU, EPI_ACC2, EPI_ATOMIC, EPI_ACC1 = 1, 2, 4, 8
GEMM_BF16X3 = 16
WGRAD_SLABS = 32
MATH = os.environ.get("FST_MATH", "bf16x3")
LDS_BUDGET = 96 * 1024
LDS_MULTI_CHUNK = 44 * 1024
PIPE_C = 16

_PARTIAL_BACKWARD = False


# ... 696 lines not shown
        return None, red[C:], red[:C]
    dx = torch.empty_like(y)
    rs = torch.empty(B, C, device=y.device, dtype=torch.float32)
    if training and _dist.global_batch_active():
        red = part.sum(dim=2).view(2 * C)
        red_g = red.clone()
        B_total = _dist.sum_over_ranks_(red_g) * B
        check(lib.fst_bn_bwd_apply(ptr(dy), ptr(y), ptr(out), ptr(stats), ptr(red_g), 1, None, ptr(dx), ptr(rs), B, C, L, int(relu),
                                   int(training), B_total, _same_numel(dy, y, out, dx), stream_ptr()), "fst_bn_bwd_apply")
    else:
        red = torch.empty(2 * C, device=y.device, dtype=torch.float32)
        check(lib.fst_bn_bwd_apply(ptr(dy), ptr(y), ptr(out), ptr(stats), ptr(part), BN_SLOTS, ptr(red), ptr(dx), ptr(rs), B, C, L,
                                   int(relu), int(training), B, _same_numel(dy, y, out, dx), stream_ptr()), "fst_bn_bwd_apply")
    _ROW_SUMS.attach(dx, rs)
    return dx, red[C:], red[:C]


def _bn_backward_join(dy: Tensor, ya: Tensor, yb: Tensor, sa: Tensor, sb: Tensor, training: bool, need_dxa: bool,
                      need_dxb: bool):
    lib = _lib.load()
    B, C, L = ya.shape
    dev = ya.device
    parts = torch.empty(2, 2, C, BN_SLOTS, device=dev, dtype=torch.float32)
    check(lib.fst_bn_bwd_reduce_join(ptr(dy), ptr(ya), ptr(yb), ptr(sa), ptr(sb), B, C, L, ptr(parts[0]), ptr(parts[1]),
                                     _same_numel(dy, ya, yb), stream_ptr()), "fst_bn_bwd_reduce_join")
    need = (need_dxa, need_dxb)
    dx = [torch.empty_like(y) if n else None for y, n in zip((ya, yb), need)]
    rs = [torch.empty(B, C, device=dev, dtype=torch.float32) if n else None for n in need]
    red = [None, None]
    if any(need):
        if training and _dist.global_batch_active():
            local = parts.sum(dim=3).view(2, 2 * C)
            red_g = local.clone()
            B_total = _dist.sum_over_ranks_(red_g) * B
            check(lib.fst_bn_bwd_apply_join(ptr(dy), ptr(ya), ptr(yb), ptr(sa), ptr(sb), ptr(red_g[0]), ptr(red_g[1]), 1, None, None,
                                            ptr(dx[0]), ptr(dx[1]), ptr(rs[0]), ptr(rs[1]), B, C, L, int(training), B_total,
                                            _same_numel(dy, ya, yb, *dx), stream_ptr()), "fst_bn_bwd_apply_join")
            red = [local[i] if need[i] else None for i in range(2)]
        else:
            sums = torch.empty(2, 2 * C, device=dev, dtype=torch.float32)
            check(lib.fst_bn_bwd_apply_join(ptr(dy), ptr(ya), ptr(yb), ptr(sa), ptr(sb), ptr(parts[0]), ptr(parts[1]), BN_SLOTS,
                                            ptr(sums[0]) if need[0] else None, ptr(sums[1]) if need[1] else None,
                                            ptr(dx[0]), ptr(dx[1]), ptr(rs[0]), ptr(rs[1]), B, C, L, int(training), B,
                                            _same_numel(dy, ya, yb, *dx), stream_ptr()), "fst_bn_bwd_apply_join")
            red = [sums[i] if need[i] else None for i in range(2)]
    res = []
    for i in range(2):
        if need[i]:
            _ROW_SUMS.attach(dx[i], rs[i])
        else:
            red[i] = _bn_slot_sum(parts[i]).view(2 * C)
        res.append((dx[i], red[i][C:], red[i][:C]))
    return res


class BNActFn(torch.autograd.Function):

    @staticmethod
    def forward(ctx, y, gamma, beta, rmean, rvar, training: bool, relu: bool, eps: float, momentum: float):
        lib = _lib.load()
        y = y.contiguous()
        B, C, L = y.shape
        stats = _bn_stats(y, gamma, beta, rmean, rvar, training, eps, momentum)
        out = torch.empty_like(y)
        check(lib.fst_bn_apply(ptr(y), ptr(stats), None, None, ptr(out), B, C, L, int(relu), _same_numel(y, out), stream_ptr()),
              "fst_bn_apply")
        ctx.save_for_backward(y, stats)
        ctx.relu, ctx.training = relu, training
        return out

    @staticmethod
    def backward(ctx, dout):
        y, stats = ctx.saved_tensors
        dx, dg, db = _bn_backward(dout.contiguous(), y, None, stats, ctx.relu, ctx.training, ctx.needs_input_grad[0])
        return dx, dg, db, None, None, None, None, None, None


class BNAddBNReluFn(torch.autograd.Function):

    @staticmethod
    def forward(ctx, ya, ga, ba, rma, rva, yb, gb, bb, rmb, rvb, training: bool, eps: float, momentum: float):
        lib = _lib.load()
        ya, yb = ya.contiguous(), yb.contiguous()
        B, C, L = ya.shape
        sa = _bn_stats(ya, ga, ba, rma, rva, training, eps, momentum)
        sb = _bn_stats(yb, gb, bb, rmb, rvb, training, eps, momentum)
        out = torch.empty_like(ya)
        check(lib.fst_bn_apply(ptr(ya), ptr(sa), ptr(yb), ptr(sb), ptr(out), B, C, L, 1, _same_numel(ya, yb, out), stream_ptr()),
              "fst_bn_apply")
        ctx.save_for_backward(ya, yb, sa, sb)
        ctx.training = training
        return out

    @staticmethod
    def backward(ctx, dout):
        ya, yb, sa, sb = ctx.saved_tensors
        (dxa, dga, dba), (dxb, dgb, dbb) = _bn_backward_join(dout.contiguous(), ya, yb, sa, sb, ctx.training,
                                                             ctx.needs_input_grad[0], ctx.needs_input_grad[5])
        return dxa, dga, dba, None, None, dxb, dgb, dbb, None, None, None, None, None


class WNSpecs:

    def __init__(self, h: int, n: int, n_layers: int = 8, kernel: int = 3):
        self.h, self.n, self.n_layers, self.kernel = h, n, n_layers, kernel
        self.start = ConvSpec(n, h)
        self.ins = [ConvSpec(2 * n, n, kernel, 2 ** i, int((kernel * 2 ** i - 2 ** i) / 2), C1=h) for i in range(n_layers)]
        self.rs = [ConvSpec(2 * n if i < n_layers - 1 else n, n) for i in range(n_layers)]
        self.end = ConvSpec(2 * h, n)
        self.rs_T = build_plan(n, [Segment(0, n, 0, 1), Segment(1, n, 0, 1)], 1, 1, 0, chunk_c=PIPE_C)
        self.rs_T_last = build_plan(n, [Segment(0, n, 0, 1)], 1, 1, 0, chunk_c=PIPE_C)
        nl = n_layers
        self.shapes = ([(n, h, 1), (n,), (2 * n * nl, h, 1), (2 * n * nl,), (2 * h, n, 1), (2 * h,)]
                       + [(2 * n, n, kernel)] * nl + [(2 * n,)] * nl
                       + [(2 * n if i < nl - 1 else n, n, 1) for i in range(nl)] + [(2 * n if i < nl - 1 else n,) for i in range(nl)])
        self.offsets = [0]
        for sh in self.shapes:
            self.offsets.append(self.offsets[-1] + int(math.prod(sh)))
        self.flat_numel = self.offsets[-1]

    def flatten(self, weights: Sequence[Tensor]) -> Tensor:
        assert len(weights) == len(self.shapes) and all(tuple(w.shape) == sh for w, sh in zip(weights, self.shapes))
        return torch.cat([w.reshape(-1) for w in weights])

    def unflatten(self, flat: Tensor) -> List[Tensor]:
        assert flat.numel() == self.flat_numel and flat.is_contiguous()
        return [flat[self.offsets[i]: self.offsets[i + 1]].view(sh) for i, sh in enumerate(self.shapes)]


def wn_wgrad_ok(kind: int, B: int, L: int, n: int, h: int, dil: int, a: Optional[Tensor] = None) -> bool:
    if MATH != "bf16x3" or os.environ.get("FST_WN_WGRAD", "1") == "0":
        return False
    served = _lib.load().fst_wn_wgrad_ok(kind, B, L, n, h, dil)
    return served == 1 or (served == 2 and a is not None and has_slack(a))


def empty_with_slack(B: int, C: int, L: int, device) -> Tensor:
    buf = torch.empty(B * C * L + 8, device=device, dtype=torch.float32)
    return buf[4: 4 + B * C * L].view(B, C, L)


def has_slack(t: Tensor) -> bool:
    off = t.storage_offset()
    return t.is_contiguous() and off >= 4 and t.untyped_storage().nbytes() >= (off + t.numel() + 4) * 4


WN_WGRAD_MAX_SETS = 3


def _sets(x) -> list:
    return list(x) if isinstance(x, (list, tuple)) else [x]


def wn_wgrad_in(dg, a, u0, dw_in: Tensor, dw_cond: Tensor, n: int, h: int, dil: int) -> None:
    lib = _lib.load()
    dgs, as_, u0s = _sets(dg), _sets(a), _sets(u0)
    if not (1 <= len(dgs) <= WN_WGRAD_MAX_SETS and len(as_) == len(dgs) and len(u0s) == len(dgs)):
        raise ValueError(f"wn_wgrad_in: {len(dgs)}/{len(as_)}/{len(u0s)} operand sets (1..{WN_WGRAD_MAX_SETS}, equally many)")
    B, _, L = dgs[0].shape
    u0_bs, _ = _ncl(u0s[0], "u0")
    numel = _same_numel(*as_)
    slack = True
    for dg_s, a_s, u0_s in zip(dgs, as_, u0s):
        if dg_s.numel() != 2 * numel or not dg_s.is_contiguous() or tuple(a_s.shape) != (B, n, L) or tuple(u0_s.shape) != (B, h, L):
            raise ValueError("wn_wgrad_in: dg must be contiguous [B, 2n, L], a [B, n, L], u0 [B, h, L]")
        if _ncl(u0_s, "u0")[0] != u0_bs:
            raise ValueError("wn_wgrad_in: the operand sets' u0 tensors must share one batch stride")
        slack = slack and has_slack(a_s)
    for t, sh in ((dw_in, (2 * n, n, 3)), (dw_cond, (2 * n, h, 1))):
        if tuple(t.shape) != sh or not t.is_contiguous() or t.dtype != torch.float32:
            raise ValueError(f"wn_wgrad_in: gradient target of shape {tuple(t.shape)}, expected contiguous {sh}")
    ws_n = lib.fst_wn_wgrad_workspace_floats(0, B, L, n, h, 0)
    ws = torch.empty(ws_n, device=dgs[0].device, dtype=torch.float32)
    ns = len(dgs)
    t0 = KERNEL_TIMER.begin() if KERNEL_TIMER is not None else None
    check(lib.fst_wn_wgrad_in(_ptr_sets(dgs), _ptr_sets(as_), _ptr_sets(u0s), ns, u0_bs, ptr(dw_in), ptr(dw_cond), ptr(ws), ws_n, B, L,
                              n, h, dil, int(slack), numel, stream_ptr()), "fst_wn_wgrad_in")
    if t0 is not None:
        KERNEL_TIMER.end("wn_wgrad_kernel<2, 3> bf3", t0, 2.0 * ns * B * L * 2 * n * (3 * n + h), 4.0 * ns * B * L * (2 * n + n + h))


def wn_wgrad_rs(d_a, d_out, ts, dw_rs: Tensor, last: bool, n: int) -> None:
    lib = _lib.load()
    d_outs, tss = _sets(d_out), _sets(ts)
    d_as = [None] * len(d_outs) if d_a is None else _sets(d_a)
    if not (1 <= len(d_outs) <= WN_WGRAD_MAX_SETS and len(tss) == len(d_outs) and len(d_as) == len(d_outs)):
        raise ValueError(f"wn_wgrad_rs: {len(d_as)}/{len(d_outs)}/{len(tss)} operand sets (1..{WN_WGRAD_MAX_SETS}, equally many)")
    B, _, L = d_outs[0].shape
    numel = _same_numel(*d_outs, *[t for t in d_as if t is not None])
    M = n if last else 2 * n
    for da_s, ts_s in zip(d_as, tss):
        if ts_s.numel() != 2 * numel or not ts_s.is_contiguous() or (da_s is None) != bool(last):
            raise ValueError("wn_wgrad_rs: ts must be contiguous [B, 2n, L]; d_a is None exactly on the last layer")
    if tuple(dw_rs.shape) != (M, n, 1) or not dw_rs.is_contiguous() or dw_rs.dtype != torch.float32:
        raise ValueError(f"wn_wgrad_rs: gradient target of shape {tuple(dw_rs.shape)}, expected contiguous {(M, n, 1)}")
    ws_n = lib.fst_wn_wgrad_workspace_floats(1, B, L, n, 0, int(last))
    ws = torch.empty(ws_n, device=d_outs[0].device, dtype=torch.float32)
    ns = len(d_outs)
    t0 = KERNEL_TIMER.begin() if KERNEL_TIMER is not None else None
    check(lib.fst_wn_wgrad_rs(None if last else _ptr_sets(d_as), _ptr_sets(d_outs), _ptr_sets(tss), ns, ptr(dw_rs), ptr(ws), ws_n,
                              int(last), B, L, n, numel, stream_ptr()), "fst_wn_wgrad_rs")
    if t0 is not None:
        KERNEL_TIMER.end("wn_wgrad_kernel<2, 2> bf3", t0, 2.0 * ns * B * L * M * n, 4.0 * ns * B * L * (M + 2 * n))


def dense_tap_wgrad(dy: Tensor, x: Tensor, dw: Tensor, M: int, C: int, K: int, pad_left: int) -> None:
    lib = _lib.load()
    B, _, L = dy.shape
    if tuple(dy.shape) != (B, M, L) or tuple(x.shape) != (B, C, L) or not (dy.is_contiguous() and x.is_contiguous()):
        raise ValueError(f"dense_tap_wgrad: dy {tuple(dy.shape)} / x {tuple(x.shape)} must be contiguous [B, {M}, L] / [B, {C}, L]")
    if tuple(dw.shape) != (M, C, K) or not dw.is_contiguous() or dw.dtype != torch.float32:
        raise ValueError(f"dense_tap_wgrad: gradient target of shape {tuple(dw.shape)}, expected contiguous {(M, C, K)}")
    ws_n = lib.fst_dense_tap_wgrad_workspace_floats(B, L, M, C, K)
    if ws_n <= 0:
        raise ValueError(f"dense_tap_wgrad: unsupported shape B={B} L={L} M={M} C={C} K={K}")
    ws = torch.empty(ws_n, device=dy.device, dtype=torch.float32)
    t0 = KERNEL_TIMER.begin() if KERNEL_TIMER is not None else None
    check(lib.fst_dense_tap_wgrad(ptr(dy), ptr(x), ptr(dw), ptr(ws), ws_n, B, L, M, C, K, pad_left, dy.numel(), x.numel(), stream_ptr()),
          "fst_dense_tap_wgrad")
    if t0 is not None:
        KERNEL_TIMER.end(f"tz_wgrad_kernel M={M} C={C} bf3", t0, 2.0 * B * L * M * C * K, 4.0 * B * L * (M + C))


def tap_wgrad(dy: Tensor, x: Tensor, dw: Tensor, M: int, C: int, ntaps: int, dil: int, pad_left: int) -> None:
    lib = _lib.load()
    B, _, L = dy.shape
    if tuple(dy.shape) != (B, M, L) or tuple(x.shape) != (B, C, L) or not (dy.is_contiguous() and x.is_contiguous()):
        raise ValueError(f"tap_wgrad: dy {tuple(dy.shape)} / x {tuple(x.shape)} must be contiguous [B, {M}, L] / [B, {C}, L]")
    if tuple(dw.shape) != (M, C, ntaps) or not dw.is_contiguous() or dw.dtype != torch.float32:
        raise ValueError(f"tap_wgrad: gradient target of shape {tuple(dw.shape)}, expected contiguous {(M, C, ntaps)}")
    ws_n = lib.fst_tap_wgrad_workspace_floats(B, L, M, C, ntaps)
    if ws_n <= 0:
        raise ValueError(f"tap_wgrad: unsupported shape B={B} L={L} M={M} C={C} ntaps={ntaps}")
    ws = torch.empty(ws_n, device=dy.device, dtype=torch.float32)
    t0 = KERNEL_TIMER.begin() if KERNEL_TIMER is not None else None
    check(lib.fst_tap_wgrad(ptr(dy), ptr(x), ptr(dw), ptr(ws), ws_n, B, L, M, C, ntaps, dil, pad_left, int(has_slack(x)), dy.numel(),
                            x.numel(), stream_ptr()), "fst_tap_wgrad")
    if t0 is not None:
        KERNEL_TIMER.end("tap_wgrad (wn_wgrad_kernel<2, 3>) bf3", t0, 2.0 * B * L * M * C * ntaps, 4.0 * B * L * (M + C))


def _ptr_sets(ts: Sequence[Tensor]):
    arr = (ctypes.c_void_p * len(ts))()
    for i, t in enumerate(ts):
        if t.dtype != torch.float32 or not t.is_cuda:
            raise ValueError("operand sets must be fp32 device tensors")
        arr[i] = t.data_ptr()
    return arr


class WNGradPool:

    def __init__(self):
        self.pending: dict = {}
        self.task = None

    def add(self, key, operands) -> None:
        task = torch._C._current_graph_task_id()
        if task != self.task:
            self.pending, self.task = {}, task
        self.pending.setdefault(key, []).append(operands)

    def take(self) -> dict:
        pending, self.pending = self.pending, {}
        return pending if self.task == torch._C._current_graph_task_id() else {}


class WGradJoinFn(torch.autograd.Function):

    @staticmethod
    def forward(ctx, pool: WNGradPool, specs: "WNSpecs", flat: Tensor):
        ctx.pool, ctx.specs = pool, specs
        return flat.view_as(flat)

    @staticmethod
    def backward(ctx, g):
        S, pool = ctx.specs, ctx.pool
        pending = pool.take()
        if not pending:
            return None, None, g
        g = g.contiguous()
        nl, n, h = S.n_layers, S.n, S.h
        dw = S.unflatten(g)
        g_cond_w, g_in_w, g_rs_w = dw[2], dw[6: 6 + nl], dw[6 + 2 * nl: 6 + 3 * nl]
        for (kind, i), sets in pending.items():
            for c0 in range(0, len(sets), WN_WGRAD_MAX_SETS):
                chunk = sets[c0: c0 + WN_WGRAD_MAX_SETS]
                cols = [list(col) for col in zip(*chunk)]
                if kind == 0:
                    t_in, t_cond = g_in_w[i], g_cond_w[2 * n * i: 2 * n * (i + 1)]
                    if c0:
                        t_in, t_cond = torch.empty_like(t_in), torch.empty_like(t_cond)
                    wn_wgrad_in(cols[0], cols[1], cols[2], t_in, t_cond, n, h, 2 ** i)
                    if c0:
                        g_in_w[i].add_(t_in)
                        g_cond_w[2 * n * i: 2 * n * (i + 1)].add_(t_cond)
                else:
                    last = i == nl - 1
                    t_rs = torch.empty_like(g_rs_w[i]) if c0 else g_rs_w[i]
                    wn_wgrad_rs(None if last else cols[0], cols[1], cols[2], t_rs, last, n)
                    if c0:
                        g_rs_w[i].add_(t_rs)
        return None, None, g


class WNFoldPlan:

    def __init__(self, specs: "WNSpecs", normed: Sequence[bool]):
        assert len(normed) == len(specs.shapes)
        self.specs, self.normed = specs, list(normed)
        self._key, self._table = None, None
        self.n_rows = sum(sh[0] if nm else 1 for sh, nm in zip(specs.shapes, normed))
        self.grad_offsets, off = [], 0
        for sh, nm in zip(specs.shapes, normed):
            numel = int(math.prod(sh))
            self.grad_offsets.append(off)
            off += numel
            if nm:
                self.grad_offsets.append(off)
                off += sh[0]
        self.grad_numel = off

    def n_inputs(self) -> int:
        return len(self.grad_offsets)

    def table(self, tensors: Sequence[Tensor]) -> Tensor:
        import numpy as np
        key = tuple(t.data_ptr() for t in tensors) + (str(tensors[0].device),)
        if key == self._key:
            return self._table
        rows, it, gi = [], iter(tensors), 0
        for i, (sh, nm) in enumerate(zip(self.specs.shapes, self.normed)):
            dst, numel = self.specs.offsets[i], int(math.prod(sh))
            if nm:
                v, g = next(it), next(it)
                M, rowlen = sh[0], numel // sh[0]
                assert v.is_contiguous() and g.is_contiguous() and tuple(v.shape) == tuple(sh) and g.numel() == M
                m = np.arange(M, dtype=np.int64)
                blk = np.stack([v.data_ptr() + 4 * rowlen * m, g.data_ptr() + 4 * m, dst + rowlen * m, np.full(M, rowlen, np.int64),
                                self.grad_offsets[gi] + rowlen * m, self.grad_offsets[gi + 1] + m], axis=1)
                gi += 2
            else:
                t = next(it)
                assert t.is_contiguous() and t.numel() == numel
                blk = np.array([[t.data_ptr(), 0, dst, numel, self.grad_offsets[gi], 0]], dtype=np.int64)
                gi += 1
            rows.append(blk)
        tab = np.concatenate(rows, axis=0)
        assert tab.shape == (self.n_rows, 6)
        self._table = torch.from_numpy(tab).to(tensors[0].device)
        self._key = key
        return self._table


class WNFoldFn(torch.autograd.Function):

    @staticmethod
    def forward(ctx, plan: WNFoldPlan, *tensors: Tensor):
        lib = _lib.load()
        assert len(tensors) == plan.n_inputs()
        for t in tensors:
            _lib.require_gpu_tensor(t, "WN parameter")
        tab = plan.table(tensors)
        dev = tensors[0].device
        flat = torch.empty(plan.specs.flat_numel, device=dev, dtype=torch.float32)
        norms = torch.empty(plan.n_rows, device=dev, dtype=torch.float32)
        check(lib.fst_wn_fold_fwd(ptr(tab), plan.n_rows, ptr(flat), ptr(norms), stream_ptr()), "fst_wn_fold_fwd")
        ctx.plan, ctx.tab = plan, tab
        ctx.shapes = [tuple(t.shape) for t in tensors]
        ctx.save_for_backward(norms)
        return flat

    @staticmethod
    def backward(ctx, d_flat):
        lib = _lib.load()
        (norms,) = ctx.saved_tensors
        plan: WNFoldPlan = ctx.plan
        d_flat = d_flat.contiguous()
        dpar = torch.empty(plan.grad_numel, device=d_flat.device, dtype=torch.float32)
        check(lib.fst_wn_fold_bwd(ptr(ctx.tab), plan.n_rows, ptr(d_flat), ptr(norms), ptr(dpar), stream_ptr()), "fst_wn_fold_bwd")
        grads = []
        for off, sh in zip(plan.grad_offsets, ctx.shapes):
            grads.append(dpar[off: off + int(math.prod(sh))].view(sh))
        return (None, *grads)


def wn_fused_ok(n: int, h: int, L: int, *tensors: Tensor, kernel: int = 3) -> bool:
    if MATH != "bf16x3" or kernel != 3 or not (0 < n < 128) or L % 4 != 0 or os.environ.get("FST_WN_FUSED", "1") == "0":
        return False
    return all(t.data_ptr() % 16 == 0 and t.stride(0) % 4 == 0 for t in tensors)


def wn_pack_layer(in_w: Tensor, cond_w: Tensor, in_b: Tensor, cond_b: Tensor, rs_w: Tensor, rs_b: Tensor, n: int, h: int,
                  last: bool) -> Tensor:
    lib = _lib.load()
    if in_w.dim() != 3 or in_w.size(0) != 2 * n or in_w.size(1) != n:
        raise ValueError(f"wn_pack_layer: in_w must be [2n, n, taps], got {tuple(in_w.shape)} for n={n}")
    key = None
    if _PACK_CACHE is not None:
        key = ("wn", n, h, last) + tuple((t.data_ptr(), t._version) for t in (in_w, cond_w, in_b, cond_b, rs_w, rs_b))
        hit = _PACK_CACHE.get(key)
        if hit is not None:
            return hit[0]
    nbytes = lib.fst_wn_image_bytes(n, h)
    img = torch.empty(nbytes // 4, device=in_w.device, dtype=torch.float32)
    src = [t.contiguous() for t in (in_w, cond_w, in_b, cond_b, rs_w, rs_b)]
    check(lib.fst_wn_pack(*[ptr(t) for t in src], n, h, in_w.size(2), int(last), ptr(img), nbytes, stream_ptr()), "fst_wn_pack")
    if key is not None:
        _PACK_CACHE[key] = (img, in_w, cond_w, in_b, cond_b, rs_w, rs_b, src)
    return img


def wn_layer_fwd(a: Tensor, u0: Tensor, img: Tensor, ts: Tensor, acts: Optional[Tensor], a_next: Optional[Tensor], out: Tensor,
                 first: bool, last: bool, n: int, h: int, dil: int) -> None:
    lib = _lib.load()
    a_bs, L = _ncl(a, "a")
    u0_bs, _ = _ncl(u0, "u0")
    B = a.size(0)
    numel = _same_numel(a, out, acts, a_next)
    if ts.numel() != 2 * numel or not ts.is_contiguous():
        raise ValueError("wn_layer_fwd: ts must be the contiguous [B, 2n, L] partner of a")
    t0 = KERNEL_TIMER.begin() if KERNEL_TIMER is not None else None
    check(lib.fst_wn_layer_fwd(ptr(a), a_bs, ptr(u0), u0_bs, ptr(img), img.numel() * 4, ptr(ts), ptr(acts), ptr(a_next), ptr(out),
                               int(first), int(last), B, L, n, h, dil, numel, stream_ptr()), "fst_wn_layer_fwd")
    if t0 is not None:
        rs_rows = n if last else 2 * n
        flops = 2.0 * B * L * (2 * n * (3 * n + h) + rs_rows * n)
        rows = n + h + (0 if first else n) + (0 if last else n) + n + 2 * n + (n if acts is not None else 0)
        KERNEL_TIMER.end("wn_layer_fwd_kernel", t0, flops, 4.0 * B * L * rows)


def wn_pack_bwd(rs_w: Tensor, n: int, last: bool, acc_order: bool = False) -> Tensor:
    lib = _lib.load()
    key = None
    if _PACK_CACHE is not None:
        key = ("wn_bwd", n, last, acc_order, rs_w.data_ptr(), rs_w._version)
        hit = _PACK_CACHE.get(key)
        if hit is not None:
            return hit[0]
    nbytes = lib.fst_wn_bwd_image_bytes(n, int(last))
    img = torch.empty(nbytes // 4, device=rs_w.device, dtype=torch.float32)
    src = rs_w.contiguous()
    check(lib.fst_wn_pack_bwd(ptr(src), n, int(last), int(acc_order), ptr(img), nbytes, stream_ptr()), "fst_wn_pack_bwd")
    if key is not None:
        _PACK_CACHE[key] = (img, rs_w, src)
    return img


def wn_bwd_partials(n_layers: int, B: int, L: int, device) -> Tensor:
    return torch.empty(n_layers, 256, B * ((L + 127) // 128), device=device, dtype=torch.float32)


def wn_layer_bwd(d_a: Optional[Tensor], d_out: Tensor, ts: Tensor, img: Tensor, dg: Tensor, last: bool, n: int,
                 want_row_sums: bool = False, sums_out: Optional[Tensor] = None, part: Optional[Tensor] = None) -> Optional[Tensor]:
    lib = _lib.load()
    B, _, L = d_out.shape
    deferred = part is not None
    if part is None and want_row_sums:
        part = torch.empty(256, B * ((L + 127) // 128), device=dg.device, dtype=torch.float32)
    numel = _same_numel(d_out, d_a)
    for t in (ts, dg):
        if t.numel() != 2 * numel or not t.is_contiguous():
            raise ValueError("wn_layer_bwd: ts / dg must be contiguous [B, 2n, L]")
    if part is not None and (part.shape != (256, B * ((L + 127) // 128)) or not part.is_contiguous()):
        raise ValueError(f"wn_layer_bwd: partial-sum slab of shape {tuple(part.shape)}")
    t0 = KERNEL_TIMER.begin() if KERNEL_TIMER is not None else None
    check(lib.fst_wn_layer_bwd(ptr(d_a), ptr(d_out), ptr(ts), ptr(img), img.numel() * 4, ptr(dg), ptr(part),
                               0 if part is None else part.size(1), int(last), B, L, n, numel, stream_ptr()), "fst_wn_layer_bwd")
    if t0 is not None:
        k = n if last else 2 * n
        KERNEL_TIMER.end("wn_layer_bwd_kernel", t0, 2.0 * B * L * n * k, 4.0 * B * L * (k + 4 * n))
    if part is None or deferred:
        return None
    if sums_out is not None:
        return torch.sum(part[: 2 * n], dim=1, out=sums_out)
    return part.sum(dim=1)[: 2 * n]


def wn_pack_dgrad(in_w: Tensor, cond_w: Tensor, n: int, h: int) -> Tensor:
    lib = _lib.load()
    key = None
    if _PACK_CACHE is not None:
        key = ("wn_dgrad", n, h, in_w.data_ptr(), in_w._version, cond_w.data_ptr(), cond_w._version)
        hit = _PACK_CACHE.get(key)
        if hit is not None:
            return hit[0]
    nbytes = lib.fst_wn_dgrad_image_bytes(n)
    img = torch.empty(nbytes // 4, device=in_w.device, dtype=torch.float32)
    src = (in_w.contiguous(), cond_w.contiguous())
    check(lib.fst_wn_pack_dgrad(ptr(src[0]), ptr(src[1]), n, h, in_w.size(2), ptr(img), nbytes, stream_ptr()), "fst_wn_pack_dgrad")
    if key is not None:
        _PACK_CACHE[key] = (img, in_w, cond_w, src)
    return img


WN_DGRAD_TILE = 512


def wn_dgrad_ok(n: int, h: int, dil: int) -> bool:
    return bool(_lib.load().fst_wn_dgrad_fits(n, h, dil))


def wn_dgrad_partials(n_layers: int, B: int, L: int, device) -> Tensor:
    return torch.empty(n_layers, 128, B * ((L + WN_DGRAD_TILE - 1) // WN_DGRAD_TILE), device=device, dtype=torch.float32)


def wn_layer_dgrad(dg: Tensor, img: Tensor, d_a: Optional[Tensor], d_u0: Tensor, n: int, h: int, dil: int,
                   want_row_sums: bool = False, sums_out: Optional[Tensor] = None, part: Optional[Tensor] = None):
    lib = _lib.load()
    B, _, L = dg.shape
    deferred = part is not None
    if part is None and want_row_sums:
        part = torch.empty(128, B * ((L + WN_DGRAD_TILE - 1) // WN_DGRAD_TILE), device=dg.device, dtype=torch.float32)
    d_a_new = torch.empty(B, n, L, device=dg.device, dtype=torch.float32)
    numel = _same_numel(d_a_new, d_a)
    if dg.numel() != 2 * numel or not dg.is_contiguous():
        raise ValueError("wn_layer_dgrad: dg must be contiguous [B, 2n, L]")
    d_u0_bs, _ = _ncl(d_u0, "d_u0")
    if tuple(d_u0.shape) != (B, h, L):
        raise ValueError(f"wn_layer_dgrad: d_u0 must be [B, h, L] = {(B, h, L)}, got {tuple(d_u0.shape)}")
    if part is not None and (part.shape != (128, B * ((L + WN_DGRAD_TILE - 1) // WN_DGRAD_TILE)) or not part.is_contiguous()):
        raise ValueError(f"wn_layer_dgrad: partial-sum slab of shape {tuple(part.shape)}")
    t0 = KERNEL_TIMER.begin() if KERNEL_TIMER is not None else None
    check(lib.fst_wn_layer_dgrad(ptr(dg), ptr(img), img.numel() * 4, ptr(d_a), ptr(d_a_new), ptr(d_u0), ptr(part),
                                 0 if part is None else part.size(1), B, L, n, h, dil, numel, d_u0_bs, stream_ptr()),
          "fst_wn_layer_dgrad")
    if t0 is not None:
        KERNEL_TIMER.end("wn_layer_dgrad_kernel", t0, 2.0 * B * L * 2 * n * (3 * n + h),
                         4.0 * B * L * (2 * n + (n if d_a is not None else 0) + n + 2 * h))
    if part is None:
        return d_a_new
    if deferred:
        return d_a_new, None
    if sums_out is not None:
        return d_a_new, torch.sum(part[:n], dim=1, out=sums_out)
    return d_a_new, part.sum(dim=1)[:n]


def wn_stack_bwd_ok(n: int, h: int, L: int, nl: int) -> bool:
    if os.environ.get("FST_WN_STACK", "1") == "0":
        return False
    return bool(_lib.load().fst_wn_stack_bwd_ok(n, h, L, nl))


def wn_stack_fwd_ok(n: int, h: int, L: int, nl: int, B: int) -> bool:
    if os.environ.get("FST_WN_STACK_FWD", "1") == "0":
        return False
    lib = _lib.load()
    return bool(lib.fst_wn_stack_fwd_ok(n, h, L, nl)) and B * (L // 256) >= 2 * 256 and B >= 256


def wn_stack_fwd(a_list: Sequence[Tensor], u0: Tensor, imgs: Sequence[Tensor], ts_list: Sequence[Tensor], out: Tensor, n: int,
                 h: int) -> None:
    lib = _lib.load()
    nl = len(imgs)
    B, L = u0.size(0), u0.size(2)
    u0_bs, _ = _ncl(u0, "u0")
    numel = _same_numel(out, *a_list)
    bs = (ctypes.c_int64 * nl)(*[_ncl(a, "a")[0] for a in a_list])
    for ts in ts_list:
        if ts.numel() != 2 * numel or not ts.is_contiguous():
            raise ValueError("wn_stack_fwd: every ts must be the contiguous [B, 2n, L] partner of a")
    t0 = KERNEL_TIMER.begin() if KERNEL_TIMER is not None else None
    check(lib.fst_wn_stack_fwd(_ptr_table(a_list), bs, _ptr_table(imgs), imgs[0].numel() * 4, _ptr_table(ts_list),
                               _ptr_table(list(a_list[1:]) + [None]), ptr(u0), u0_bs, ptr(out), nl, B, L, n, h, numel, stream_ptr()),
          "fst_wn_stack_fwd")
    if t0 is not None:
        flops = 2.0 * B * L * (nl * 2 * n * (3 * n + h) + (2 * nl - 1) * n * n)
        rows = nl * (n + h + 2 * n) + (nl - 1) * (n + 2 * n) + n
        KERNEL_TIMER.end("wn_stack_fwd_kernel", t0, flops, 4.0 * B * L * rows)


def _ptr_table(ts: Sequence[Optional[Tensor]]):
    arr = (ctypes.c_void_p * len(ts))()
    for i, t in enumerate(ts):
        arr[i] = None if t is None else t.data_ptr()
    return arr


def wn_stack_bwd(ts_list: Sequence[Tensor], imgs_b: Sequence[Tensor], imgs_d: Sequence[Tensor], dgs: Sequence[Tensor],
                 da_out: Sequence[Optional[Tensor]], d_out: Tensor, d_u0: Tensor, n: int, h: int,
                 part_b: Optional[Tensor] = None, part_d: Optional[Tensor] = None) -> None:
    lib = _lib.load()
    nl = len(ts_list)
    B, _, L = d_out.shape
    numel = _same_numel(d_out, *[t for t in da_out if t is not None])
    for t in list(ts_list) + list(dgs):
        if t.numel() != 2 * numel or not t.is_contiguous():
            raise ValueError("wn_stack_bwd: ts / dg must be contiguous [B, 2n, L]")
    d_u0_bs, _ = _ncl(d_u0, "d_u0")
    if tuple(d_u0.shape) != (B, h, L):
        raise ValueError(f"wn_stack_bwd: d_u0 must be [B, h, L] = {(B, h, L)}, got {tuple(d_u0.shape)}")
    if (part_b is None) != (part_d is None):
        raise ValueError("wn_stack_bwd: row sums of both kinds or of neither")
    if part_b is not None and (tuple(part_b.shape) != (nl, 256, B) or tuple(part_d.shape) != (nl, 128, B)
                               or not (part_b.is_contiguous() and part_d.is_contiguous())):
        raise ValueError("wn_stack_bwd: row-sum slabs must be contiguous [nl, 256, B] and [nl, 128, B]")
    t0 = KERNEL_TIMER.begin() if KERNEL_TIMER is not None else None
    rs_b = None if part_b is None else _ptr_table([part_b[i] for i in range(nl)])
    rs_d = None if part_d is None else _ptr_table([part_d[i] for i in range(nl)])
    check(lib.fst_wn_stack_bwd(_ptr_table(ts_list), _ptr_table(imgs_b), _ptr_table(imgs_d), _ptr_table(dgs), _ptr_table(da_out),
                               rs_b, rs_d, ptr(d_out), ptr(d_u0), d_u0_bs, nl, B, L, n, h, numel, stream_ptr()),
          "fst_wn_stack_bwd")
    if t0 is not None:
        flops = 2.0 * B * L * (n * (2 * n * nl - n) + nl * 2 * n * (3 * n + h))
        rows = nl * (2 * n + n + 2 * 2 * n + 2 * h) + n * sum(t is not None for t in da_out)
        KERNEL_TIMER.end("wn_stack_bwd_kernel", t0, flops, 4.0 * B * L * rows)


def _wn_layer(S: WNSpecs, ts: Sequence[Tensor], i: int):
    n, nl = S.n, S.n_layers
    rows = slice(2 * n * i, 2 * n * (i + 1))
    return ts[6 + i], ts[2][rows], ts[6 + nl + i], ts[3][rows], ts[6 + 2 * nl + i], ts[6 + 3 * nl + i]


def _wn_forward(specs: WNSpecs, u0: Tensor, flat: Tensor):
    S, nl, n, h = specs, specs.n_layers, specs.n, specs.h
    flat = flat.contiguous()
    W = S.unflatten(flat)
    B, _, L = u0.shape
    dev = u0.device
    a = S.start.forward(u0, None, W[0], None, W[1], y=empty_with_slack(B, n, L, dev))
    fused = wn_fused_ok(n, h, L, a, u0, kernel=S.kernel)
    if fused:
        out = torch.empty(B, n, L, device=dev, dtype=torch.float32)
        imgs = [wn_pack_layer(*_wn_layer(S, W, i), n, h, i == nl - 1) for i in range(nl)]
        a_list = [a] + [empty_with_slack(B, n, L, dev) for _ in range(nl - 1)]
        ts_list = [torch.empty(B, 2 * n, L, device=dev, dtype=torch.float32) for _ in range(nl)]
        if wn_stack_fwd_ok(n, h, L, nl, B):
            wn_stack_fwd(a_list, u0, imgs, ts_list, out, n, h)
        else:
            for i in range(nl):
                last = i == nl - 1
                wn_layer_fwd(a_list[i], u0, imgs[i], ts_list[i], None, None if last else a_list[i + 1], out, i == 0, last, n,
                             h, 2 ** i)
        acts_list = ts_list
    else:
        lib = _lib.load()
        out = torch.zeros(B, n, L, device=dev, dtype=torch.float32)
        bias_g = torch.stack(W[6 + nl: 6 + 2 * nl]) + W[3].view(nl, 2 * n)
        a_list, ts_list, acts_list = [a], [], []
        for i in range(nl):
            in_w, cond_w, _, _, rs_w, rs_b = _wn_layer(S, W, i)
            g = S.ins[i].forward(a, u0, in_w, cond_w, bias_g[i])
            acts = torch.empty(B, n, L, device=dev, dtype=torch.float32)
            check(lib.fst_gate_fwd(ptr(g), ptr(acts), B, n, L, _gate_numel(acts, g), stream_ptr()), "fst_gate_fwd")
            ts_list.append(g)
            acts_list.append(acts)
            if i < nl - 1:
                a_next = torch.empty_like(a)
                S.rs[i].forward(acts, None, rs_w, None, rs_b, y=a_next, res=a, y2=out, msplit=n, flags=EPI_ACC2)
                a = a_next
                a_list.append(a)
            else:
                S.rs[i].forward(acts, None, rs_w, None, rs_b, y=None, y2=out, msplit=0, flags=EPI_ACC2)
    o = S.end.forward(out, None, W[4], None, W[5])
    return o, fused, (u0, out, *a_list, *ts_list, *acts_list, flat)


def _wn_backward(S: WNSpecs, fused: bool, sv, do: Tensor, d_u0: Tensor, need_w: bool, pool: Optional["WNGradPool"] = None):
    nl, h, n = S.n_layers, S.h, S.n
    u0, out, flat = sv[0], sv[1], sv[2 + 3 * nl]
    a_list, ts_list, acts_list = sv[2: 2 + nl], sv[2 + nl: 2 + 2 * nl], sv[2 + 2 * nl: 2 + 3 * nl]
    W = S.unflatten(flat)
    B, _, L = u0.shape
    deferring = need_w and pool is not None and fused and any(
        wn_wgrad_ok(0, B, L, n, h, 2 ** i, a_list[i]) or wn_wgrad_ok(1, B, L, n, h, 2 ** i) for i in range(nl))
    d_flat = (torch.zeros_like(flat) if deferring else torch.empty_like(flat)) if need_w else None
    G = S.unflatten(d_flat) if need_w else None
    do = do.contiguous()

    d_out = S.end.grad_x0(do, W[4])
    da_sums = None
    if need_w:
        S.end.grad_w(out, None, do, out0=G[4])
        row_sum(do, out=G[5])
        d_out_sum = row_sum(d_out, out=G[6 + 4 * nl - 1])
        o0 = S.offsets[6 + 3 * nl]
        d_rs_b = d_flat[o0: o0 + (nl - 1) * 2 * n].view(nl - 1, 2 * n)
        d_rs_b[:, n:] = d_out_sum
        da_sums = [G[1]] + [d_rs_b[i, :n] for i in range(nl - 1)]
    part_b = part_d = None
    if not fused:
        d_a = _wn_backward_unfused(S, W, G, a_list, ts_list, acts_list, u0, d_out, d_u0, da_sums)
    elif all(wn_dgrad_ok(n, h, 2 ** i) for i in range(nl)) and wn_stack_bwd_ok(n, h, L, nl):
        d_a, part_b, part_d = _wn_backward_stack(S, W, G, a_list, ts_list, u0, d_out, d_u0, pool)
    else:
        d_a, part_b, part_d = _wn_backward_layers(S, W, G, a_list, ts_list, u0, d_out, d_u0, da_sums, pool)
    S.start.grad_x0(d_a, W[0], out=d_u0, flags=EPI_ACC1)
    if need_w:
        S.start.grad_w(u0, None, d_a, out0=G[0])
        o0 = S.offsets[6 + nl]
        if part_b is not None:
            torch.sum(part_b[:, : 2 * n, :], dim=2, out=d_flat[o0: o0 + nl * 2 * n].view(nl, 2 * n))
        if part_d is not None:
            if nl > 1:
                torch.sum(part_d[1:, :n, :], dim=2, out=d_rs_b[:, :n])
            torch.sum(part_d[0, :n, :], dim=1, out=G[1])
        G[3].copy_(d_flat[o0: o0 + nl * 2 * n])
    return d_flat


def _wn_wgrad_rs(S: WNSpecs, i: int, d_a: Optional[Tensor], d_out: Tensor, ts: Tensor, G, pool) -> None:
    n, B, L, last, g_rs_w = S.n, d_out.size(0), d_out.size(2), i == S.n_layers - 1, _wn_layer(S, G, i)[4]
    if wn_wgrad_ok(1, B, L, n, S.h, 2 ** i):
        if pool is not None:
            pool.add((1, i), (d_a, d_out, ts))
        else:
            wn_wgrad_rs(d_a, d_out, ts, g_rs_w, last, n)
    elif last:
        S.rs[i].grad_w(ts[:, :n], None, d_out, x0_mul_off=n * L, out0=g_rs_w)
    else:
        S.rs[i].grad_w(ts[:, :n], None, d_a, d_out, msplit=n, x0_mul_off=n * L, out0=g_rs_w)


def _wn_wgrad_in(S: WNSpecs, i: int, dg: Tensor, a: Tensor, u0: Tensor, G, pool) -> None:
    n, h, B, L = S.n, S.h, dg.size(0), dg.size(2)
    g_in_w, g_cond_w = _wn_layer(S, G, i)[:2]
    if wn_wgrad_ok(0, B, L, n, h, 2 ** i, a):
        if pool is not None:
            pool.add((0, i), (dg, a, u0))
        else:
            wn_wgrad_in(dg, a, u0, g_in_w, g_cond_w, n, h, 2 ** i)
    else:
        S.ins[i].grad_w(a, u0, dg, out0=g_in_w, out1=g_cond_w)


def _wn_backward_stack(S: WNSpecs, W, G, a_list, ts_list, u0: Tensor, d_out: Tensor, d_u0: Tensor, pool):
    nl, n, h = S.n_layers, S.n, S.h
    B, _, L = d_out.shape
    imgs_b = [wn_pack_bwd(_wn_layer(S, W, i)[4], n, i == nl - 1, acc_order=True) for i in range(nl)]
    imgs_d = [wn_pack_dgrad(*_wn_layer(S, W, i)[:2], n, h) for i in range(nl)]
    new = lambda *shape: torch.empty(*shape, device=d_out.device, dtype=torch.float32)
    if G is None:
        dgs, da_out = [new(B, 2 * n, L)] * nl, [new(B, n, L)] + [None] * (nl - 1)
        part_b = part_d = None
    else:
        dgs, da_out = [new(B, 2 * n, L) for _ in range(nl)], [new(B, n, L) for _ in range(nl)]
        part_b, part_d = new(nl, 256, B), new(nl, 128, B)
    wn_stack_bwd(ts_list, imgs_b, imgs_d, dgs, da_out, d_out, d_u0, n, h, part_b, part_d)
    if G is not None:
        for i in range(nl):
            _wn_wgrad_rs(S, i, da_out[i + 1] if i + 1 < nl else None, d_out, ts_list[i], G, pool)
            _wn_wgrad_in(S, i, dgs[i], a_list[i], u0, G, pool)
    return da_out[0], part_b, part_d


def _wn_backward_layers(S: WNSpecs, W, G, a_list, ts_list, u0: Tensor, d_out: Tensor, d_u0: Tensor, da_sums, pool):
    nl, n, h = S.n_layers, S.n, S.h
    B, _, L = d_out.shape
    dev = d_out.device
    fused_dg = [wn_dgrad_ok(n, h, 2 ** i) for i in range(nl)]
    part_b = wn_bwd_partials(nl, B, L, dev) if G is not None else None
    part_d = wn_dgrad_partials(nl, B, L, dev) if G is not None and all(fused_dg) else None
    d_a = None
    for i in reversed(range(nl)):
        last = i == nl - 1
        in_w, cond_w, _, _, rs_w, _ = _wn_layer(S, W, i)
        if G is not None:
            _wn_wgrad_rs(S, i, d_a, d_out, ts_list[i], G, pool)
        dg = torch.empty(B, 2 * n, L, device=dev, dtype=torch.float32)
        wn_layer_bwd(d_a, d_out, ts_list[i], wn_pack_bwd(rs_w, n, last), dg, last, n, part=None if part_b is None else part_b[i])
        if G is not None:
            _wn_wgrad_in(S, i, dg, a_list[i], u0, G, pool)
        if not fused_dg[i]:
            d_a = S.ins[i].grad_x01(dg, in_w, cond_w, d_a, d_u0)
            if G is not None:
                row_sum(d_a, out=da_sums[i])
        elif G is None:
            d_a = wn_layer_dgrad(dg, wn_pack_dgrad(in_w, cond_w, n, h), d_a, d_u0, n, h, 2 ** i)
        else:
            d_a = wn_layer_dgrad(dg, wn_pack_dgrad(in_w, cond_w, n, h), d_a, d_u0, n, h, 2 ** i, want_row_sums=True,
                                 sums_out=da_sums[i], part=None if part_d is None else part_d[i])[0]
    return d_a, part_b, part_d


def _wn_backward_unfused(S: WNSpecs, W, G, a_list, g_list, acts_list, u0: Tensor, d_out: Tensor, d_u0: Tensor, da_sums) -> Tensor:
    lib = _lib.load()
    nl, n = S.n_layers, S.n
    B, _, L = d_out.shape
    d_a = None
    for i in reversed(range(nl)):
        last = i == nl - 1
        in_w, cond_w, _, _, rs_w, _ = _wn_layer(S, W, i)
        dacts = torch.empty(B, n, L, device=d_out.device, dtype=torch.float32)
        plan = S.rs_T_last if last else S.rs_T
        bf3 = bf3_ok(plan, L)
        a_pk = pack_weights(plan, n, rs_w, (0, 1, n, 0), *(() if last else (rs_w, (n * n, 1, n, 0))), bf3=bf3)
        conv_gemm(plan, a_pk, d_out if last else d_a, None if last else d_out, None, B, L, n, dacts,
                  nb=S.start.nb_for(B, L, pick_mb(n), 0, 0), bf3=bf3)
        if G is not None:
            g_in_w, g_cond_w, g_in_b, _, g_rs_w, _ = _wn_layer(S, G, i)
            if last:
                S.rs[i].grad_w(acts_list[i], None, d_out, out0=g_rs_w)
            else:
                S.rs[i].grad_w(acts_list[i], None, d_a, d_out, msplit=n, out0=g_rs_w)
        dg = torch.empty(B, 2 * n, L, device=d_out.device, dtype=torch.float32)
        check(lib.fst_gate_bwd(ptr(g_list[i]), ptr(dacts), ptr(dg), B, n, L, _gate_numel(dacts, dg, g_list[i]), stream_ptr()),
              "fst_gate_bwd")
        if G is not None:
            S.ins[i].grad_w(a_list[i], u0, dg, out0=g_in_w, out1=g_cond_w)
            row_sum(dg, out=g_in_b)
        d_a = S.ins[i].grad_x01(dg, in_w, cond_w, d_a, d_u0)
        if G is not None:
            row_sum(d_a, out=da_sums[i])
    return d_a


class WNFn(torch.autograd.Function):

    @staticmethod
    def forward(ctx, specs: WNSpecs, u0: Tensor, flat: Tensor):
        o, fused, saved = _wn_forward(specs, u0, flat)
        ctx.specs, ctx.fused = specs, fused
        ctx.save_for_backward(*saved)
        return o

    @staticmethod
    def backward(ctx, do):
        u0 = ctx.saved_tensors[0]
        d_u0 = torch.zeros(u0.size(0), ctx.specs.h, u0.size(2), device=u0.device, dtype=torch.float32)
        d_flat = _wn_backward(ctx.specs, ctx.fused, ctx.saved_tensors, do, d_u0, ctx.needs_input_grad[2] and _want_weight_grad())
        return None, (d_u0 if ctx.needs_input_grad[1] else None), d_flat


def _coupling_forward(u: Tensor, o: Tensor):
    lib = _lib.load()
    B, C, L = u.shape
    xn = torch.empty_like(u)
    part = torch.empty(lib.fst_coupling_sum_slots(B, C // 2, L), 2, device=u.device, dtype=torch.float32)
    check(lib.fst_coupling_fwd(ptr(u), ptr(o), ptr(xn), B, C // 2, L, _same_numel(u, o, xn), ptr(part), stream_ptr()),
          "fst_coupling_fwd")
    sums = part.sum(dim=0)
    return xn, sums[0], sums[1]


def _scalar_f32(g: Optional[Tensor]) -> Optional[Tensor]:
    return None if g is None else g.contiguous().float()


def _coupling_backward(u: Tensor, o: Tensor, dxn: Optional[Tensor], g_ls: Optional[Tensor], g_sq: Optional[Tensor]):
    lib = _lib.load()
    B, C, L = u.shape
    if dxn is None and g_ls is None and g_sq is None:
        return torch.zeros_like(u), torch.zeros_like(o)
    du, d_o = torch.empty_like(u), torch.empty_like(o)
    dxn = None if dxn is None else dxn.contiguous()
    g_ls, g_sq = _scalar_f32(g_ls), _scalar_f32(g_sq)
    check(lib.fst_coupling_bwd(ptr(u), ptr(o), ptr(dxn), None, ptr(g_ls), ptr(g_sq), ptr(du), ptr(d_o), B, C // 2, L,
                               _same_numel(u, o, dxn, du, d_o), stream_ptr()), "fst_coupling_bwd")
    return du, d_o


class CouplingFn(torch.autograd.Function):

    @staticmethod
    def forward(ctx, u, o):
        u, o = u.contiguous(), o.contiguous()
        ctx.save_for_backward(u, o)
        ctx.set_materialize_grads(False)
        return _coupling_forward(u, o)

    @staticmethod
    def backward(ctx, dxn, g_ls, g_sq):
        u, o = ctx.saved_tensors
        return _coupling_backward(u, o, dxn, g_ls, g_sq)


class FlowFn(torch.autograd.Function):

    @staticmethod
    def forward(ctx, specs: WNSpecs, x: Tensor, flat: Tensor, inverse: bool, pool: Optional[WNGradPool] = None):
        lib = _lib.load()
        ctx.pool = pool
        x = x.contiguous()
        h = specs.h
        assert x.size(1) == 2 * h
        o, fused, saved = _wn_forward(specs, x[:, :h], flat)
        B, C, L = x.shape
        if inverse:
            xn = torch.empty_like(x)
            check(lib.fst_coupling_inv_fwd(ptr(x), ptr(o), ptr(xn), B, h, L, _same_numel(x, o, xn), stream_ptr()), "fst_coupling_inv_fwd")
            s_ls = s_sq = None
            keep = xn
        else:
# ... 354 lines not shown
```

### include/fst_hip.h

```cpp
#ifndef FST_HIP_H
#define FST_HIP_H

#include <stdint.h>

#ifdef __cplusplus
extern "C" {
#endif

#define FST_ABI_VERSION 16

int fst_version(void);
const char* fst_last_error(void);

#define FST_PLAN_HEADER 16

typedef struct {
  const float* w;
  int64_t off0, sm, sc, st;
} fst_wsrc;

int fst_pack_weights(const int32_t* plan_dev, const int32_t* plan_host, int plan_len,
                     const fst_wsrc* src0_host, const fst_wsrc* src1_host,
                     int M, int g_begin, int g_end , int row_base ,
                     float* a_packed, void* stream);

int fst_pack_weights_bf16x3(const int32_t* plan_dev, const int32_t* plan_host, int plan_len,
                            const fst_wsrc* src0_host, const fst_wsrc* src1_host,
                            int M, int g_begin, int g_end, int row_base, void* a_image, void* stream);

int fst_unpack_weights(const int32_t* plan_dev, const int32_t* plan_host, int plan_len,
                       const float* a_packed, int M,
                       float* dw0, int64_t off0_0, int64_t sm0, int64_t sc0, int64_t st0,
                       float* dw1, int64_t off0_1, int64_t sm1, int64_t sc1, int64_t st1,
                       int n_slabs ,
                       void* stream);

int fst_mask_taps(float* w, const int32_t* live_lo, const int32_t* live_hi, int M, int C, int K, void* stream);

#define FST_EPI_RELU    1
#define FST_EPI_ACC2    2
#define FST_EPI_ATOMIC  4
#define FST_EPI_ACC1    8
#define FST_GEMM_BF16X3 16
#define FST_WGRAD_SLABS 32
int fst_conv_gemm(const float* x0, int64_t x0_bs, const float* x1, int64_t x1_bs,
                  const float* a_packed, const int32_t* plan_dev, const int32_t* plan_host, int plan_len,
                  const float* bias,
                  float* y, int64_t y_bs, const float* res, int64_t res_bs,
                  float* y2, int64_t y2_bs, int msplit, int m2_start ,
                  int B, int L, int M, int nb_cfg, int ksplit, int flags, void* stream);

int fst_conv_wgrad(const float* x0, int64_t x0_bs, const float* x1, int64_t x1_bs,
                   const float* dy, int64_t dy_bs, const float* dy2, int64_t dy2_bs, int msplit,
                   float* da_packed, const int32_t* plan_dev, const int32_t* plan_host, int plan_len,
                   int B, int L, int M, int ksplit, int flags , int64_t x0_mul_off, void* stream);

#define FST_ROUTE_GEMM      1
#define FST_ROUTE_PIPE      2
#define FST_ROUTE_BF3       3
#define FST_ROUTE_WIN_BF3   4
#define FST_ROUTE_WIN_ROWS  5
#define FST_ROUTE_WGRAD     6
#define FST_ROUTE_EPI_PLAIN   0
#define FST_ROUTE_EPI_ADD     1
#define FST_ROUTE_EPI_ATOMIC  2
#define FST_ROUTE_EPI_VEC     3
#define FST_ROUTE_EPI_VEC_ADD 4
int fst_conv_last_route(int32_t out[8]);

int fst_row_sum(const float* x, int64_t x_bs, int B, int C, int L, float* out, void* stream);

#define FST_BN_SLOTS 16
int fst_bn_stats(const float* y, int B, int C, int L, float* part , int64_t numel, void* stream);
int fst_bn_finalize(const float* part, int n_slots, const float* gamma, const float* beta,
                    float* running_mean, float* running_var, int train, int C, float eps, float momentum,
                    float* stats, void* stream);
int fst_bn_apply(const float* y, const float* stats, const float* res, const float* res_stats,
                 float* out, int B, int C, int L, int relu, int64_t numel, void* stream);
int fst_bn_bwd_reduce(const float* dy, const float* y, const float* out, const float* stats,
                      int B, int C, int L, int relu, float* red , int64_t numel, void* stream);
int fst_bn_bwd_apply(const float* dy, const float* y, const float* out, const float* stats, const float* red, int n_slots,
                     float* red_out, float* dx, float* row_sums, int B, int C, int L, int relu, int train, int B_total,
                     int64_t numel, void* stream);
int fst_bn_bwd_reduce_join(const float* dy, const float* ya, const float* yb, const float* stats_a, const float* stats_b,
                           int B, int C, int L, float* red_a, float* red_b, int64_t numel, void* stream);
int fst_bn_bwd_apply_join(const float* dy, const float* ya, const float* yb, const float* stats_a, const float* stats_b,
                          const float* red_a, const float* red_b, int n_slots, float* red_out_a, float* red_out_b,
                          float* dxa, float* dxb, float* row_sums_a, float* row_sums_b, int B, int C, int L, int train,
                          int B_total, int64_t numel, void* stream);

int fst_gate_fwd(float* g_ts, float* acts, int B, int n, int L, int64_t numel_acts, void* stream);
int fst_gate_bwd(const float* ts, const float* dacts, float* dg, int B, int n, int L, int64_t numel_acts, void* stream);
int64_t fst_coupling_sum_slots(int B, int h, int L);
int fst_coupling_fwd(const float* u, const float* o, float* xn, int B, int h, int L, int64_t numel, float* sums, void* stream);
int fst_coupling_bwd(const float* u, const float* o, const float* dxn, const float* dlogs, const float* g_ls, const float* g_sq,
                     float* du, float* d_o, int B, int h, int L, int64_t numel, void* stream);
int fst_coupling_inv_fwd(const float* x, const float* o, float* xn, int B, int h, int L, int64_t numel, void* stream);
int fst_coupling_inv_bwd(const float* xn, const float* o, const float* dxn,
                         float* dx, float* d_o, int B, int h, int L, int64_t numel, void* stream);

int fst_wn_fold_fwd(const int64_t* table_dev, int n_rows, float* flat, float* norms , void* stream);
int fst_wn_fold_bwd(const int64_t* table_dev, int n_rows, const float* d_flat, const float* norms, float* dpar, void* stream);

int fst_logdet_inv(const float* W, int n, float* out , float* inv_t , void* stream);

int64_t fst_wn_image_bytes(int n, int h);
int fst_wn_pack(const float* in_w, const float* cond_w, const float* in_b, const float* cond_b,
                const float* rs_w, const float* rs_b, int n, int h, int ntaps , int last, void* image, int64_t image_bytes, void* stream);
int fst_wn_layer_fwd(const float* a, int64_t a_bs, const float* u0, int64_t u0_bs, const void* image, int64_t image_bytes,
                     float* ts, float* acts, float* a_next, float* out, int first, int last,
                     int B, int L, int n, int h, int dil, int64_t numel_a, void* stream);

int64_t fst_wn_bwd_image_bytes(int n, int last);
int fst_wn_pack_bwd(const float* rs_w, int n, int last,
                    int acc_order ,
                    void* image, int64_t image_bytes, void* stream);
int fst_wn_layer_bwd(const float* d_a_next , const float* d_out, const float* ts, const void* image,
                     int64_t image_bytes, float* dg,
                     float* row_sums ,
                     int64_t row_sums_rows, int last, int B, int L, int n, int64_t numel_a, void* stream);

int64_t fst_wn_dgrad_image_bytes(int n);
int fst_wn_pack_dgrad(const float* in_w, const float* cond_w, int n, int h, int ntaps , void* image,
                      int64_t image_bytes, void* stream);
int fst_wn_dgrad_fits(int n, int h, int dil);
int fst_wn_layer_dgrad(const float* dg, const void* image, int64_t image_bytes, const float* d_a, float* d_a_new, float* d_u0,
                       float* row_sums , int64_t row_sums_rows,
                       int B, int L, int n, int h, int dil, int64_t numel_a, int64_t d_u0_bs, void* stream);

int fst_wn_stack_fwd_ok(int n, int h, int L, int nl);
int fst_wn_stack_fwd(const float* const* a_in, const int64_t* a_bs, const void* const* images, int64_t image_bytes, float* const* ts,
                     float* const* a_next, const float* u0, int64_t u0_bs, float* out, int nl, int B, int L, int n, int h,
                     int64_t numel_a, void* stream);

int fst_wn_stack_bwd_ok(int n, int h, int L, int nl);
int fst_wn_stack_bwd(const float* const* ts, const void* const* img_b, const void* const* img_d, float* const* dg,
                     float* const* da_out, float* const* rs_b , float* const* rs_d ,
                     const float* d_out, float* d_u0, int64_t d_u0_bs, int nl, int B, int L, int n, int h, int64_t numel_a,
                     void* stream);

int fst_wn_wgrad_ok(int kind, int B, int L, int n, int h, int dil);
int64_t fst_wn_wgrad_workspace_floats(int kind, int B, int L, int n, int h, int last);
int fst_wn_wgrad_in(const float* const* dg, const float* const* a, const float* const* u0, int n_sets, int64_t u0_bs, float* dw_in,
                    float* dw_cond, float* workspace, int64_t workspace_floats, int B, int L, int n, int h, int dil, int a_slack,
                    int64_t numel_a, void* stream);
int fst_wn_wgrad_rs(const float* const* d_a , const float* const* d_out, const float* const* ts, int n_sets,
                    float* dw_rs, float* workspace, int64_t workspace_floats, int last, int B, int L, int n, int64_t numel_a,
                    void* stream);

int64_t fst_nt_gemm_workspace_floats(int M, int N, int K);
int fst_nt_gemm(const float* A, const float* Bm, float* C, float* workspace, int64_t workspace_floats, int M, int N, int K,
                const float* epi_p , const float* epi_r1 , int epi_ncls, float epi_scale,
                float* epi_raw , void* stream);

int fst_tap_wgrad_ok(int B, int L, int M, int C, int ntaps, int dil, int pad_left);
int64_t fst_tap_wgrad_workspace_floats(int B, int L, int M, int C, int ntaps);
int fst_tap_wgrad(const float* dy, const float* x, float* dw , float* workspace, int64_t workspace_floats,
                  int B, int L, int M, int C, int ntaps, int dil, int pad_left, int x_slack, int64_t numel_dy, int64_t numel_x,
                  void* stream);

int fst_dense_tap_wgrad_ok(int B, int L, int M, int C, int K, int pad_left);
int64_t fst_dense_tap_wgrad_workspace_floats(int B, int L, int M, int C, int K);
int fst_dense_tap_wgrad(const float* dy, const float* x, float* dw , float* workspace, int64_t workspace_floats,
                        int B, int L, int M, int C, int K, int pad_left, int64_t numel_dy, int64_t numel_x, void* stream);

#define FST_WN_ROUTE_LEN         12
#define FST_WN_ROUTE_WGRAD       1
#define FST_WN_ROUTE_TZ          2
#define FST_WN_ROUTE_LAYER_FWD   3
#define FST_WN_ROUTE_STACK_FWD   4
#define FST_WN_ROUTE_LAYER_BWD   5
#define FST_WN_ROUTE_LAYER_DGRAD 6
#define FST_WN_ROUTE_STACK_BWD   7
int fst_wn_last_route(int32_t out[FST_WN_ROUTE_LEN]);

int fst_batch_sum(const float* x0, const float* x1, float* part, int B, int64_t N, int S, void* stream);
int fst_noise_transfer_fwd(const float* part, int S, int B, const float* r_t_dev, const float* r_s_dev, float r_t, float r_s,
                           float* avg_t, float* avg_s, const float* W, const float* bias, float* dist, float* pre, float* learned,
                           int C, int L, void* stream);
int fst_bcast_add(float* out, const float* x, const float* v, int B, int64_t N, void* stream);
int fst_noise_transfer_bwd(const float* part, int S, const float* pre, const float* W, float* dpre, float* dd, int C, int L,
                           void* stream);
int fst_noise_transfer_dw(const float* dpre, const float* dist, float* dW, float* dbias, int C, int L, void* stream);
int fst_noise_transfer_bwd_apply(const float* g, const float* dd, const float* r_t_dev, const float* r_s_dev, float r_t, float r_s,
                                 int B, float* dz_t, float* dz_s, int64_t N, void* stream);

int fst_relu_bwd(const float* dy, const float* y, float* out, int64_t n, void* stream);

#define FST_ACT_NONE  0
#define FST_ACT_RELU  1
#define FST_ACT_LEAKY 2
int64_t fst_gemm_workspace_floats(int M, int N, int K);
int fst_gemm(const float* A, int64_t lda, int ta, const float* B, int64_t ldb, int tb, float* C, int64_t ldc, int M, int N, int K,
             const float* bias, int act, float slope, float* workspace, int64_t workspace_floats, void* stream);
int fst_act_bwd(const float* dy, const float* y, float* out, int64_t n, float slope, void* stream);
int fst_axpy(float* y, const float* x, float alpha, int64_t n, void* stream);
int fst_add_slices(float* dst, int64_t dst_bs, const float* a, int64_t a_bs, const float* b, int64_t b_bs,
                   int B, int C, int L, void* stream);

int64_t fst_cpc_workspace_floats(int T, int B, int C, int Bc);
int64_t fst_cpc_nce_slots(int T, int B, int C, int Bc);
int fst_cpc_nce_fwd(const float* enc, int64_t s_i, int64_t s_b, int64_t s_c, const int32_t* t0_dev ,
                    const float* pred , int T, int B, int C,
                    int Bc , int col_off ,
                    float* lse , float* nce_sum , float* workspace ,
                    void* stream);
int fst_cpc_nce_bwd(const float* enc, int64_t s_i, int64_t s_b, int64_t s_c, const int32_t* t0_dev ,
                    const float* pred, const float* lse, int T, int B, int C, int Bc, int col_off, const float* gout,
                    float* denc , float* dpred , void* stream);

int fst_gru_fwd(const float* xproj, const float* w_hh, const float* b_hh, float* h_all, float* gates,
                const int32_t* t_last_dev, int t_last, int B, int S, int H, int64_t numel_h, void* stream);
int fst_gru_bwd(const float* w_hh, const float* h_all, const float* gates, const float* dout,
                const int32_t* t_last_dev, int t_last, float* dxproj, float* dgh, int B, int S, int H,
                int64_t numel_h, void* stream);

int fst_lstm2_fwd(const float* xproj, const float* w_hh_t, float* h2, float* save, int B, int H, int64_t numel_xproj, void* stream);
int fst_lstm2_bwd(const float* w_hh, const float* save, const float* dh2, float* dxproj, float* dpre2, int B, int H,
                  int64_t numel_xproj, void* stream);

int fst_rmsprop_multi(float* const* p_host, const float* const* g_host, float* const* v_host, const int64_t* numel_host,
                      const float* lr_host, int n_tensors, float alpha, float eps, void* stream);
int fst_adam_multi(float* const* p_host, const float* const* g_host, float* const* m_host, float* const* v_host,
                   const int64_t* numel_host, int n_tensors, const float* step_dev, float lr, float beta1, float beta2, float eps,
                   void* stream);
int fst_rmsprop_multi_dev(float* const* p_host, const float* const* g_host, float* const* v_host, const int64_t* numel_host,
                          const float* const* lr_dev_host, int n_tensors, float alpha, float eps, void* stream);
int fst_adam_multi_dev(float* const* p_host, const float* const* g_host, float* const* m_host, float* const* v_host,
                       const int64_t* numel_host, int n_tensors, const float* step_dev, const float* lr_dev, float beta1, float beta2,
                       float eps, void* stream);

#ifdef __cplusplus
}
#endif
#endif
```

Measured before the change: 3590.

## Batch WN weight packing and wgrad split-K reductions into multi-layer launches

Adds stacked pack kernels that pack forward, backward and dgrad weight images for all WaveNet layers in one launch each, indexed by blockIdx.y, instead of one launch per layer. It also splits the input and residual-skip weight-gradient kernels into slab-producing passes plus a single reduce_many kernel that sums the split-K partials for up to 16 entries at once. Deferred gradient accumulation is handled by adding temporaries after the batched reduce. The aim is to cut kernel launch count and host overhead per step, at the cost of larger parameter structs, more workspace held live and more complex caching logic.

After: 3634 (median of 6 runs). +1.2%, better.

```diff
diff --git a/feature_level_style_transfer_for_tsc_amd/_lib.py b/feature_level_style_transfer_for_tsc_amd/_lib.py
--- a/feature_level_style_transfer_for_tsc_amd/_lib.py
+++ b/feature_level_style_transfer_for_tsc_amd/_lib.py
@@ -7,7 +7,7 @@
 
 import torch
 
-ABI_VERSION = 16
+ABI_VERSION = 17
 _LIB_NAME = "libfst_hip.so"
 _HERE = os.path.dirname(os.path.abspath(__file__))
 LIB_PATH = os.environ.get("FST_HIP_LIB", os.path.join(_HERE, _LIB_NAME))
@@ -65,6 +65,10 @@
     "fst_wn_wgrad_in": (c_int, [_P, _P, _P, c_int, c_int64, _P, _P, _P, c_int64, c_int, c_int, c_int, c_int, c_int, c_int, c_int64,
                                 c_void_p]),
     "fst_wn_wgrad_rs": (c_int, [_P, _P, _P, c_int, _P, _P, c_int64, c_int, c_int, c_int, c_int, c_int64, c_void_p]),
+    "fst_wn_wgrad_in_slabs": (c_int, [_P, _P, _P, c_int, c_int64, _P, c_int64, c_int, c_int, c_int, c_int, c_int, c_int, c_int64,
+                                      c_void_p]),
+    "fst_wn_wgrad_rs_slabs": (c_int, [_P, _P, _P, c_int, _P, c_int64, c_int, c_int, c_int, c_int, c_int64, c_void_p]),
+    "fst_wn_wgrad_reduce_many": (c_int, [_I32P, _I32P, _I32P, _P, _P, _P, _P, c_int, c_int, c_int, c_int, c_int, c_void_p]),
     "fst_nt_gemm_workspace_floats": (c_int64, [c_int, c_int, c_int]),
     "fst_nt_gemm": (c_int, [_P, _P, _P, _P, c_int64, c_int, c_int, c_int, _P, _P, c_int, c_float, _P, c_void_p]),
     "fst_tap_wgrad_ok": (c_int, [c_int, c_int, c_int, c_int, c_int, c_int, c_int]),
@@ -90,13 +94,16 @@
     "fst_logdet_inv": (c_int, [_P, c_int, _P, _P, c_void_p]),
     "fst_wn_image_bytes": (c_int64, [c_int, c_int]),
     "fst_wn_pack": (c_int, [_P, _P, _P, _P, _P, _P, c_int, c_int, c_int, c_int, _P, c_int64, c_void_p]),
+    "fst_wn_pack_stack": (c_int, [_P, _P, _P, _P, _P, _P, c_int, c_int, c_int, c_int, _P, c_int64, c_void_p]),
     "fst_wn_layer_fwd": (c_int, [_P, c_int64, _P, c_int64, _P, c_int64, _P, _P, _P, _P, c_int, c_int, c_int, c_int, c_int, c_int,
                                  c_int, c_int64, c_void_p]),
     "fst_wn_bwd_image_bytes": (c_int64, [c_int, c_int]),
     "fst_wn_pack_bwd": (c_int, [_P, c_int, c_int, c_int, _P, c_int64, c_void_p]),
+    "fst_wn_pack_bwd_stack": (c_int, [_P, c_int, c_int, c_int, _P, c_int64, c_void_p]),
     "fst_wn_layer_bwd": (c_int, [_P, _P, _P, _P, c_int64, _P, _P, c_int64, c_int, c_int, c_int, c_int, c_int64, c_void_p]),
     "fst_wn_dgrad_image_bytes": (c_int64, [c_int]),
     "fst_wn_pack_dgrad": (c_int, [_P, _P, c_int, c_int, c_int, _P, c_int64, c_void_p]),
+    "fst_wn_pack_dgrad_stack": (c_int, [_P, _P, c_int, c_int, c_int, c_int, _P, c_int64, c_void_p]),
     "fst_wn_dgrad_fits": (c_int, [c_int, c_int, c_int]),
     "fst_wn_layer_dgrad": (c_int, [_P, _P, c_int64, _P, _P, _P, _P, c_int64, c_int, c_int, c_int, c_int, c_int, c_int64, c_int64,
                                    c_void_p]),
diff --git a/feature_level_style_transfer_for_tsc_amd/csrc/wn_fused.hip b/feature_level_style_transfer_for_tsc_amd/csrc/wn_fused.hip
--- a/feature_level_style_transfer_for_tsc_amd/csrc/wn_fused.hip
+++ b/feature_level_style_transfer_for_tsc_amd/csrc/wn_fused.hip
@@ -33,8 +33,8 @@
   uint4* img;
 };
 
-__global__ __launch_bounds__(64) void wn_pack_kernel(WnPackParams p) {
-  const int lane = threadIdx.x, blk = blockIdx.x & 7, st = blockIdx.x >> 3;
+__device__ __forceinline__ void wn_pack_body(const WnPackParams& p, int bx) {
+  const int lane = threadIdx.x, blk = bx & 7, st = bx >> 3;
   const int S1 = 3 * p.CH + p.CH2, n = p.n, h = p.h;
   const int hh = lane >> 5, rowb = (blk & 3) * 32 + (lane & 31);
   const bool row_ok = rowb < n;
@@ -80,10 +80,30 @@
   uint4* dst = p.img + ((long long)st * 8 + blk) * 128 + lane;
   dst[0] = make_uint4(hi[0], hi[1], hi[2], hi[3]);
   dst[64] = make_uint4(lo[0], lo[1], lo[2], lo[3]);
-  if (blockIdx.x == 0 && lane < 2) {
+  if (bx == 0 && lane < 2) {
     const unsigned one = lane ? 0x3f800000u : 0u;
     p.img[(long long)(S1 + 8) * 8 * 128 + lane] = make_uint4(one, one, one, one);
   }
+}
+
+__global__ __launch_bounds__(64) void wn_pack_kernel(WnPackParams p) { wn_pack_body(p, blockIdx.x); }
+
+struct WnPackStackParams {
+  const float* in_w[WS_MAXL];
+  const float* cond_w[WS_MAXL];
+  const float* in_b[WS_MAXL];
+  const float* cond_b[WS_MAXL];
+  const float* rs_w[WS_MAXL];
+  const float* rs_b[WS_MAXL];
+  uint4* img[WS_MAXL];
+  int n, h, nl, CH, CH2;
+};
+
+__global__ __launch_bounds__(64) void wn_pack_stack_kernel(WnPackStackParams s) {
+  const int i = blockIdx.y;
+  const WnPackParams p = {s.in_w[i], s.cond_w[i], s.in_b[i], s.cond_b[i], s.rs_w[i], s.rs_b[i], s.n, s.h, i == s.nl - 1 ? 1 : 0,
+                          s.CH, s.CH2, s.img[i]};
+  wn_pack_body(p, blockIdx.x);
 }
 
 static inline int wn_ch(int n) { return (n + 15) / 16; }
@@ -106,6 +126,29 @@
   WnPackParams p = {in_w, cond_w, in_b, cond_b, rs_w, rs_b, n, h, last ? 1 : 0, wn_ch(n), wn_ch2(h), static_cast<uint4*>(image)};
   const int stages = 3 * p.CH + p.CH2 + 8;
   hipLaunchKernelGGL(wn_pack_kernel, dim3((unsigned)(stages * 8)), dim3(64), 0, (hipStream_t)stream, p);
+  FST_LAUNCH_CHECK();
+  return 0;
+}
+
+extern "C" int fst_wn_pack_stack(const float* const* in_w, const float* const* cond_w, const float* const* in_b,
+                                 const float* const* cond_b, const float* const* rs_w, const float* const* rs_b, int nl, int n, int h,
+                                 int ntaps, void* const* images, int64_t image_bytes, void* stream) {
+  FST_REQUIRE(in_w && cond_w && in_b && cond_b && rs_w && rs_b && images, "fst_wn_pack_stack: null table");
+  FST_REQUIRE(nl >= 1 && nl <= WS_MAXL, "fst_wn_pack_stack: %d layers (1..%d)", nl, WS_MAXL);
+  FST_REQUIRE(ntaps == 3, "fst_wn_pack_stack: the fused WN kernels are 3-tap (in_w [2n][n][3]); got %d taps", ntaps);
+  FST_REQUIRE(n > 0 && n < 128 && h > 0, "fst_wn_pack_stack: needs 0 < n < 128 (one spare K row carries the bias), h > 0; n=%d h=%d", n, h);
+  FST_REQUIRE(image_bytes == fst_wn_image_bytes(n, h), "fst_wn_pack_stack: images are %lld bytes, expected %lld",
+              (long long)image_bytes, (long long)fst_wn_image_bytes(n, h));
+  WnPackStackParams s = {};
+  for (int i = 0; i < nl; ++i) {
+    FST_REQUIRE(in_w[i] && cond_w[i] && in_b[i] && cond_b[i] && rs_w[i] && rs_b[i] && images[i], "fst_wn_pack_stack: null operand in layer %d", i);
+    FST_REQUIRE(fst_aligned16(images[i]), "fst_wn_pack_stack: images must be 16-byte aligned");
+    s.in_w[i] = in_w[i]; s.cond_w[i] = cond_w[i]; s.in_b[i] = in_b[i]; s.cond_b[i] = cond_b[i]; s.rs_w[i] = rs_w[i]; s.rs_b[i] = rs_b[i];
+    s.img[i] = static_cast<uint4*>(images[i]);
+  }
+  s.n = n; s.h = h; s.nl = nl; s.CH = wn_ch(n); s.CH2 = wn_ch2(h);
+  const int stages = 3 * s.CH + s.CH2 + 8;
+  hipLaunchKernelGGL(wn_pack_stack_kernel, dim3((unsigned)(stages * 8), (unsigned)nl), dim3(64), 0, (hipStream_t)stream, s);
   FST_LAUNCH_CHECK();
   return 0;
 }
@@ -636,8 +679,8 @@
   int acc_order;
 };
 
-__global__ __launch_bounds__(64) void wn_pack_bwd_kernel(WnPackBwdParams p) {
-  const int lane = threadIdx.x, blk = blockIdx.x & 3, st = blockIdx.x >> 2;
+__device__ __forceinline__ void wn_pack_bwd_body(const WnPackBwdParams& p, int bx, int n_blocks) {
+  const int lane = threadIdx.x, blk = bx & 3, st = bx >> 2;
   const int n = p.n, hh = lane >> 5, m = blk * 32 + (lane & 31);
   const int src = p.last ? 0 : st / p.CH, c = st - src * p.CH;
   float v[8];
@@ -653,7 +696,22 @@
   uint4* dst = p.img + ((long long)st * 4 + blk) * 128 + lane;
   dst[0] = make_uint4(hi[0], hi[1], hi[2], hi[3]);
   dst[64] = make_uint4(lo[0], lo[1], lo[2], lo[3]);
-  if (blockIdx.x == 0 && lane == 0) p.img[(long long)gridDim.x * 128] = make_uint4(0u, 0u, 0u, 0u);
+  if (bx == 0 && lane == 0) p.img[(long long)n_blocks * 128] = make_uint4(0u, 0u, 0u, 0u);
+}
+
+__global__ __launch_bounds__(64) void wn_pack_bwd_kernel(WnPackBwdParams p) { wn_pack_bwd_body(p, blockIdx.x, gridDim.x); }
+
+struct WnPackBwdStackParams {
+  const float* rs_w[WS_MAXL];
+  uint4* img[WS_MAXL];
+  int n, nl, CH, acc_order;
+};
+
+__global__ __launch_bounds__(64) void wn_pack_bwd_stack_kernel(WnPackBwdStackParams s) {
+  const int i = blockIdx.y, last = i == s.nl - 1 ? 1 : 0, n_blocks = (last ? 1 : 2) * s.CH * 4;
+  if ((int)blockIdx.x >= n_blocks) return;
+  const WnPackBwdParams p = {s.rs_w[i], s.n, last, s.CH, s.img[i], s.acc_order};
+  wn_pack_bwd_body(p, blockIdx.x, n_blocks);
 }
 
 extern "C" int64_t fst_wn_bwd_image_bytes(int n, int last) {
@@ -669,6 +727,26 @@
   WnPackBwdParams p = {rs_w, n, last ? 1 : 0, wn_ch(n), static_cast<uint4*>(image), acc_order ? 1 : 0};
   const int stages = (last ? 1 : 2) * p.CH;
   hipLaunchKernelGGL(wn_pack_bwd_kernel, dim3((unsigned)(stages * 4)), dim3(64), 0, (hipStream_t)stream, p);
+  FST_LAUNCH_CHECK();
+  return 0;
+}
+
+extern "C" int fst_wn_pack_bwd_stack(const float* const* rs_w, int nl, int n, int acc_order, void* const* images, int64_t image_bytes,
+                                     void* stream) {
+  FST_REQUIRE(rs_w && images && n > 0 && n <= 128, "fst_wn_pack_bwd_stack: bad arguments (n=%d, needs n <= 128)", n);
+  FST_REQUIRE(nl >= 1 && nl <= WS_MAXL, "fst_wn_pack_bwd_stack: %d layers (1..%d)", nl, WS_MAXL);
+  FST_REQUIRE(image_bytes == fst_wn_bwd_image_bytes(n, 0), "fst_wn_pack_bwd_stack: images are %lld bytes, expected %lld",
+              (long long)image_bytes, (long long)fst_wn_bwd_image_bytes(n, 0));
+  WnPackBwdStackParams s = {};
+  for (int i = 0; i < nl; ++i) {
+    FST_REQUIRE(rs_w[i] && images[i], "fst_wn_pack_bwd_stack: null operand in layer %d", i);
+    FST_REQUIRE(fst_aligned16(images[i]), "fst_wn_pack_bwd_stack: images must be 16-byte aligned");
+    s.rs_w[i] = rs_w[i];
+    s.img[i] = static_cast<uint4*>(images[i]);
+  }
+  s.n = n; s.nl = nl; s.CH = wn_ch(n); s.acc_order = acc_order ? 1 : 0;
+  const int stages = (nl > 1 ? 2 : 1) * s.CH;
+  hipLaunchKernelGGL(wn_pack_bwd_stack_kernel, dim3((unsigned)(stages * 4), (unsigned)nl), dim3(64), 0, (hipStream_t)stream, s);
   FST_LAUNCH_CHECK();
   return 0;
 }
@@ -847,8 +925,8 @@
   uint4* img;
 };
 
-__global__ __launch_bounds__(64) void wn_pack_dgrad_kernel(WnPackDgradParams p) {
-  const int lane = threadIdx.x, ab = blockIdx.x % DG_A_BLOCKS, c = blockIdx.x / DG_A_BLOCKS;
+__device__ __forceinline__ void wn_pack_dgrad_body(const WnPackDgradParams& p, int bx, int n_blocks) {
+  const int lane = threadIdx.x, ab = bx % DG_A_BLOCKS, c = bx / DG_A_BLOCKS;
   const int n = p.n, h = p.h, hh = lane >> 5, l31 = lane & 31;
   int tap, blk;
   if (ab < 4) { tap = 0; blk = ab; } else if (ab < 9) { tap = 1; blk = ab - 4; } else { tap = 2; blk = ab - 9; }
@@ -870,10 +948,25 @@
   unsigned hi[4], lo[4];
 #pragma unroll
   for (int j = 0; j < 4; ++j) split_bf16_pair(v[2 * j], v[2 * j + 1], hi[j], lo[j]);
-  uint4* dst = p.img + (long long)blockIdx.x * 128 + lane;
+  uint4* dst = p.img + (long long)bx * 128 + lane;
   dst[0] = make_uint4(hi[0], hi[1], hi[2], hi[3]);
   dst[64] = make_uint4(lo[0], lo[1], lo[2], lo[3]);
-  if (blockIdx.x == 0 && lane == 0) p.img[(long long)gridDim.x * 128] = make_uint4(0u, 0u, 0u, 0u);
+  if (bx == 0 && lane == 0) p.img[(long long)n_blocks * 128] = make_uint4(0u, 0u, 0u, 0u);
+}
+
+__global__ __launch_bounds__(64) void wn_pack_dgrad_kernel(WnPackDgradParams p) { wn_pack_dgrad_body(p, blockIdx.x, gridDim.x); }
+
+struct WnPackDgradStackParams {
+  const float* in_w[WS_MAXL];
+  const float* cond_w[WS_MAXL];
+  uint4* img[WS_MAXL];
+  int n, h, CHK;
+};
+
+__global__ __launch_bounds__(64) void wn_pack_dgrad_stack_kernel(WnPackDgradStackParams s) {
+  const int i = blockIdx.y;
+  const WnPackDgradParams p = {s.in_w[i], s.cond_w[i], s.n, s.h, s.CHK, s.img[i]};
+  wn_pack_dgrad_body(p, blockIdx.x, gridDim.x);
 }
 
 extern "C" int64_t fst_wn_dgrad_image_bytes(int n) {
@@ -890,6 +983,26 @@
   FST_REQUIRE(fst_aligned16(image), "fst_wn_pack_dgrad: image must be 16-byte aligned");
   WnPackDgradParams p = {in_w, cond_w, n, h, (2 * n + 15) / 16, static_cast<uint4*>(image)};
   hipLaunchKernelGGL(wn_pack_dgrad_kernel, dim3((unsigned)(p.CHK * DG_A_BLOCKS)), dim3(64), 0, (hipStream_t)stream, p);
+  FST_LAUNCH_CHECK();
+  return 0;
+}
+
+extern "C" int fst_wn_pack_dgrad_stack(const float* const* in_w, const float* const* cond_w, int nl, int n, int h, int ntaps,
+                                       void* const* images, int64_t image_bytes, void* stream) {
+  FST_REQUIRE(in_w && cond_w && images && n > 0 && n <= 128 && h > 0 && h <= 32, "fst_wn_pack_dgrad_stack: needs n <= 128, h <= 32 (n=%d h=%d)", n, h);
+  FST_REQUIRE(nl >= 1 && nl <= WS_MAXL, "fst_wn_pack_dgrad_stack: %d layers (1..%d)", nl, WS_MAXL);
+  FST_REQUIRE(ntaps == 3, "fst_wn_pack_dgrad_stack: the fused WN kernels are 3-tap (in_w [2n][n][3]); got %d taps", ntaps);
+  FST_REQUIRE(image_bytes == fst_wn_dgrad_image_bytes(n), "fst_wn_pack_dgrad_stack: images are %lld bytes, expected %lld",
+              (long long)image_bytes, (long long)fst_wn_dgrad_image_bytes(n));
+  WnPackDgradStackParams s = {};
+  for (int i = 0; i < nl; ++i) {
+    FST_REQUIRE(in_w[i] && cond_w[i] && images[i], "fst_wn_pack_dgrad_stack: null operand in layer %d", i);
+    FST_REQUIRE(fst_aligned16(images[i]), "fst_wn_pack_dgrad_stack: images must be 16-byte aligned");
+    s.in_w[i] = in_w[i]; s.cond_w[i] = cond_w[i];
+    s.img[i] = static_cast<uint4*>(images[i]);
+  }
+  s.n = n; s.h = h; s.CHK = (2 * n + 15) / 16;
+  hipLaunchKernelGGL(wn_pack_dgrad_stack_kernel, dim3((unsigned)(s.CHK * DG_A_BLOCKS), (unsigned)nl), dim3(64), 0, (hipStream_t)stream, s);
   FST_LAUNCH_CHECK();
   return 0;
 }
diff --git a/feature_level_style_transfer_for_tsc_amd/csrc/wn_wgrad.hip b/feature_level_style_transfer_for_tsc_amd/csrc/wn_wgrad.hip
--- a/feature_level_style_transfer_for_tsc_amd/csrc/wn_wgrad.hip
+++ b/feature_level_style_transfer_for_tsc_amd/csrc/wn_wgrad.hip
@@ -415,6 +415,89 @@
   }
 }
 
+#define WW_MAX_RED 16
+struct WwRedSeg { int rows, out, out_off, out_sc, out_sm; };
+struct WwRedEntry {
+  const float* slab;
+  const float* slab_extra;
+  float* w[2];
+  int ksplit, Kcols, K_main, K, n_extra, M, n_x;
+  int quad_blocks;
+  WwRedSeg x[4];
+};
+struct WwRedParams { WwRedEntry e[WW_MAX_RED]; };
+
+__device__ __forceinline__ void ww_scatter_entry(const WwRedEntry& e, int m, int kk, float v) {
+  int si = 0, c = kk;
+#pragma unroll
+  for (int j = 0; j < 3; ++j)
+    if (si + 1 < e.n_x && c >= e.x[si].rows) { c -= e.x[si].rows; ++si; }
+  int out = e.x[0].out, off = e.x[0].out_off, sc = e.x[0].out_sc, sm = e.x[0].out_sm;
+  if (si == 1) { out = e.x[1].out; off = e.x[1].out_off; sc = e.x[1].out_sc; sm = e.x[1].out_sm; }
+  if (si == 2) { out = e.x[2].out; off = e.x[2].out_off; sc = e.x[2].out_sc; sm = e.x[2].out_sm; }
+  if (si == 3) { out = e.x[3].out; off = e.x[3].out_off; sc = e.x[3].out_sc; sm = e.x[3].out_sm; }
+  float* w = out == 0 ? e.w[0] : e.w[1];
+  w[(long long)m * sm + (long long)c * sc + off] = v;
+}
+
+__global__ __launch_bounds__(256) void wn_wgrad_reduce_many_kernel(WwRedParams p) {
+  __shared__ float4 part[4][64];
+  const WwRedEntry& e = p.e[blockIdx.z];
+  const int bx = blockIdx.x;
+  if (bx >= e.quad_blocks) {
+    const int it = (bx - e.quad_blocks) * 256 + threadIdx.x;
+    if (e.K_main < e.K && it < e.M * e.n_extra) {
+      const int m = it / e.n_extra, j = it - m * e.n_extra;
+      const float* q = e.slab_extra + (long long)m * 2 + j;
+      float s = 0.f;
+      int sl = 0;
+      for (; sl + 8 <= e.ksplit; sl += 8) {
+        float v[8];
+#pragma unroll
+        for (int u = 0; u < 8; ++u) v[u] = q[(long long)(sl + u) * WW_MROWS * 2];
+#pragma unroll
+        for (int u = 0; u < 8; ++u) s += v[u];
+      }
+      for (; sl < e.ksplit; ++sl) s += q[(long long)sl * WW_MROWS * 2];
+      ww_scatter_entry(e, m, e.K_main + j, s);
+    }
+    return;
+  }
+  const int cx = threadIdx.x & 63, sg = threadIdx.x >> 6;
+  const int qpr = e.Kcols >> 2;
+  const int quad = bx * 64 + cx;
+  const bool live = quad < e.M * qpr;
+  float4 s = make_float4(0.f, 0.f, 0.f, 0.f);
+  if (live) {
+    const long long st = (long long)WW_MROWS * e.Kcols;
+    const float* q = e.slab + (long long)quad * 4;
+    int sl = sg;
+    for (; sl + 28 < e.ksplit; sl += 32) {
+      float4 v[8];
+#pragma unroll
+      for (int u = 0; u < 8; ++u) v[u] = *reinterpret_cast<const float4*>(q + (sl + 4 * u) * st);
+#pragma unroll
+      for (int u = 0; u < 8; ++u) { s.x += v[u].x; s.y += v[u].y; s.z += v[u].z; s.w += v[u].w; }
+    }
+    for (; sl < e.ksplit; sl += 4) {
+      const float4 v = *reinterpret_cast<const float4*>(q + sl * st);
+      s.x += v.x; s.y += v.y; s.z += v.z; s.w += v.w;
+    }
+  }
+  part[sg][cx] = s;
+  __syncthreads();
+  if (sg == 0 && live) {
+    float4 t = part[0][cx];
+#pragma unroll
+    for (int g2 = 1; g2 < 4; ++g2) { const float4 o = part[g2][cx]; t.x += o.x; t.y += o.y; t.z += o.z; t.w += o.w; }
+    const float tv[4] = {t.x, t.y, t.z, t.w};
+    const int m = quad / qpr, kk0 = (quad - m * qpr) * 4;
+#pragma unroll
+    for (int j = 0; j < 4; ++j)
+      if (kk0 + j < e.K_main) ww_scatter_entry(e, m, kk0 + j, tv[j]);
+  }
+}
+
 
 static thread_local int32_t g_wn_route[FST_WN_ROUTE_LEN] = {0};
 
@@ -493,11 +576,27 @@
   return 0;
 }
 
-extern "C" int fst_wn_wgrad_in(const float* const* dg, const float* const* a, const float* const* u0, int n_sets, int64_t u0_bs,
-                               float* dw_in, float* dw_cond, float* workspace, int64_t workspace_floats, int B, int L, int n, int h,
-                               int dil, int a_slack, int64_t numel_a, void* stream) {
+static void ww_in_segments(WwParams& p, int n, int h, int L, int dil, long long u0_bs) {
+  p.n_dy = 1;
+  p.dy[0] = {{}, (long long)2 * n * L, 0, 2 * n, 0, 0, 0, 0, 0};
+  p.n_x = 4;
+  for (int tap = 0; tap < 3; ++tap) p.x[tap] = {{}, (long long)n * L, 0, n, (tap - 1) * dil, 0, tap, 3, 3 * n};
+  p.x[3] = {{}, u0_bs, 0, h, 0, 1, 0, 1, h};
+}
+
+static void ww_rs_segments(WwParams& p, int n, int L, int last) {
+  p.n_dy = last ? 1 : 2;
+  p.dy[0] = {{}, (long long)n * L, 0, n, 0, 0, 0, 0, 0};
+  p.dy[1] = {{}, (long long)n * L, 0, n, 0, 0, 0, 0, 0};
+  p.n_x = 1;
+  p.x[0] = {{}, (long long)2 * n * L, (long long)n * L, n, 0, 0, 0, 1, n};
+}
+
+static int ww_in(const float* const* dg, const float* const* a, const float* const* u0, int n_sets, int64_t u0_bs, float* dw_in,
+                 float* dw_cond, float* workspace, int64_t workspace_floats, int B, int L, int n, int h, int dil, int a_slack,
+                 int64_t numel_a, void* stream, bool reduce) {
   fst_wn_clear_route();
-  FST_REQUIRE(dg && a && u0 && dw_in && dw_cond && workspace, "fst_wn_wgrad_in: null operand");
+  FST_REQUIRE(dg && a && u0 && workspace && (!reduce || (dw_in && dw_cond)), "fst_wn_wgrad_in: null operand");
   FST_REQUIRE(n_sets >= 1 && n_sets <= WW_MAX_SETS, "fst_wn_wgrad_in: %d operand sets (1..%d)", n_sets, WW_MAX_SETS);
   const int served = fst_wn_wgrad_ok(0, B, L, n, h, dil);
   FST_REQUIRE(served == 1 || (served == 2 && a_slack), "fst_wn_wgrad_in: unsupported shape B=%d L=%d n=%d h=%d dil=%d (needs L %% 32 == 0, "
@@ -509,11 +608,7 @@
   const int KT = ww_geometry(0, B, L, n, h, 0, n_sets, &p);
   FST_REQUIRE(workspace_floats >= (int64_t)p.ksplit * WW_MROWS * (p.Kcols + 2), "fst_wn_wgrad_in: workspace of %lld floats is too small",
               (long long)workspace_floats);
-  p.n_dy = 1;
-  p.dy[0] = {{}, (long long)2 * n * L, 0, 2 * n, 0, 0, 0, 0, 0};
-  p.n_x = 4;
-  for (int tap = 0; tap < 3; ++tap) p.x[tap] = {{}, (long long)n * L, 0, n, (tap - 1) * dil, 0, tap, 3, 3 * n};
-  p.x[3] = {{}, (long long)u0_bs, 0, h, 0, 1, 0, 1, h};
+  ww_in_segments(p, n, h, L, dil, (long long)u0_bs);
   for (int s = 0; s < n_sets; ++s) {
     FST_REQUIRE(dg[s] && a[s] && u0[s], "fst_wn_wgrad_in: null operand in set %d", s);
     FST_REQUIRE(fst_aligned16(dg[s]) && fst_aligned16(a[s]) && fst_aligned16(u0[s]), "fst_wn_wgrad_in: operands must be 16-byte aligned");
@@ -525,14 +620,25 @@
   p.slab = workspace;
   p.slab_extra = workspace + (long long)p.ksplit * WW_MROWS * p.Kcols;
   p.w[0] = dw_in; p.w[1] = dw_cond;
-  return ww_launch(p, KT, stream);
-}
-
-extern "C" int fst_wn_wgrad_rs(const float* const* d_a, const float* const* d_out, const float* const* ts, int n_sets, float* dw_rs,
-                               float* workspace, int64_t workspace_floats, int last, int B, int L, int n, int64_t numel_a,
-                               void* stream) {
+  return ww_launch(p, KT, stream, reduce);
+}
+
+extern "C" int fst_wn_wgrad_in(const float* const* dg, const float* const* a, const float* const* u0, int n_sets, int64_t u0_bs,
+                               float* dw_in, float* dw_cond, float* workspace, int64_t workspace_floats, int B, int L, int n, int h,
+                               int dil, int a_slack, int64_t numel_a, void* stream) {
+  return ww_in(dg, a, u0, n_sets, u0_bs, dw_in, dw_cond, workspace, workspace_floats, B, L, n, h, dil, a_slack, numel_a, stream, true);
+}
+
+extern "C" int fst_wn_wgrad_in_slabs(const float* const* dg, const float* const* a, const float* const* u0, int n_sets, int64_t u0_bs,
+                                     float* workspace, int64_t workspace_floats, int B, int L, int n, int h, int dil, int a_slack,
+                                     int64_t numel_a, void* stream) {
+  return ww_in(dg, a, u0, n_sets, u0_bs, nullptr, nullptr, workspace, workspace_floats, B, L, n, h, dil, a_slack, numel_a, stream, false);
+}
+
+static int ww_rs(const float* const* d_a, const float* const* d_out, const float* const* ts, int n_sets, float* dw_rs, float* workspace,
+                 int64_t workspace_floats, int last, int B, int L, int n, int64_t numel_a, void* stream, bool reduce) {
   fst_wn_clear_route();
-  FST_REQUIRE(d_out && ts && dw_rs && workspace && (last || d_a), "fst_wn_wgrad_rs: null operand");
+  FST_REQUIRE(d_out && ts && (dw_rs || !reduce) && workspace && (last || d_a), "fst_wn_wgrad_rs: null operand");
   FST_REQUIRE(n_sets >= 1 && n_sets <= WW_MAX_SETS, "fst_wn_wgrad_rs: %d operand sets (1..%d)", n_sets, WW_MAX_SETS);
   FST_REQUIRE(fst_wn_wgrad_ok(1, B, L, n, 0, 4), "fst_wn_wgrad_rs: unsupported shape B=%d L=%d n=%d (needs L %% 32 == 0, n < 128)", B, L, n);
   FST_REQUIRE((long long)B * n * L == (long long)numel_a, "fst_wn_wgrad_rs: B*n*L does not match the element count %lld", (long long)numel_a);
@@ -541,11 +647,7 @@
   const int KT = ww_geometry(1, B, L, n, 0, last, n_sets, &p);
   FST_REQUIRE(workspace_floats >= (int64_t)p.ksplit * WW_MROWS * (p.Kcols + 2), "fst_wn_wgrad_rs: workspace of %lld floats is too small",
               (long long)workspace_floats);
-  p.n_dy = last ? 1 : 2;
-  p.dy[0] = {{}, (long long)n * L, 0, n, 0, 0, 0, 0, 0};
-  p.dy[1] = {{}, (long long)n * L, 0, n, 0, 0, 0, 0, 0};
-  p.n_x = 1;
-  p.x[0] = {{}, (long long)2 * n * L, (long long)n * L, n, 0, 0, 0, 1, n};
+  ww_rs_segments(p, n, L, last);
   for (int s = 0; s < n_sets; ++s) {
     FST_REQUIRE(d_out[s] && ts[s] && (last || d_a[s]), "fst_wn_wgrad_rs: null operand in set %d", s);
     FST_REQUIRE(fst_aligned16(d_out[s]) && fst_aligned16(ts[s]) && (last || fst_aligned16(d_a[s])), "fst_wn_wgrad_rs: operands must be 16-byte aligned");
@@ -556,7 +658,56 @@
   p.slab = workspace;
   p.slab_extra = workspace + (long long)p.ksplit * WW_MROWS * p.Kcols;
   p.w[0] = dw_rs; p.w[1] = nullptr;
-  return ww_launch(p, KT, stream);
+  return ww_launch(p, KT, stream, reduce);
+}
+
+extern "C" int fst_wn_wgrad_rs(const float* const* d_a, const float* const* d_out, const float* const* ts, int n_sets, float* dw_rs,
+                               float* workspace, int64_t workspace_floats, int last, int B, int L, int n, int64_t numel_a,
+                               void* stream) {
+  return ww_rs(d_a, d_out, ts, n_sets, dw_rs, workspace, workspace_floats, last, B, L, n, numel_a, stream, true);
+}
+
+extern "C" int fst_wn_wgrad_rs_slabs(const float* const* d_a, const float* const* d_out, const float* const* ts, int n_sets,
+                                     float* workspace, int64_t workspace_floats, int last, int B, int L, int n, int64_t numel_a,
+                                     void* stream) {
+  return ww_rs(d_a, d_out, ts, n_sets, nullptr, workspace, workspace_floats, last, B, L, n, numel_a, stream, false);
+}
+
+extern "C" int fst_wn_wgrad_reduce_many(const int32_t* kind, const int32_t* last, const int32_t* n_sets, float* const* workspace,
+                                        const int64_t* workspace_floats, float* const* dw0, float* const* dw1, int n_entries, int B,
+                                        int L, int n, int h, void* stream) {
+  fst_wn_clear_route();
+  FST_REQUIRE(kind && last && n_sets && workspace && workspace_floats && dw0 && dw1, "fst_wn_wgrad_reduce_many: null table");
+  FST_REQUIRE(n_entries >= 1 && n_entries <= WW_MAX_RED, "fst_wn_wgrad_reduce_many: %d entries (1..%d)", n_entries, WW_MAX_RED);
+  WwRedParams rp = {};
+  unsigned gx = 1;
+  for (int j = 0; j < n_entries; ++j) {
+    FST_REQUIRE(kind[j] == 0 || kind[j] == 1, "fst_wn_wgrad_reduce_many: entry %d has kind %d (0 or 1)", j, (int)kind[j]);
+    FST_REQUIRE(fst_wn_wgrad_ok(kind[j], B, L, n, h, 4), "fst_wn_wgrad_reduce_many: unsupported shape B=%d L=%d n=%d h=%d", B, L, n, h);
+    FST_REQUIRE(n_sets[j] >= 1 && n_sets[j] <= WW_MAX_SETS, "fst_wn_wgrad_reduce_many: entry %d has %d operand sets (1..%d)", j,
+                (int)n_sets[j], WW_MAX_SETS);
+    FST_REQUIRE(workspace[j] && dw0[j] && (kind[j] == 1 || dw1[j]), "fst_wn_wgrad_reduce_many: null operand in entry %d", j);
+    FST_REQUIRE(fst_aligned16(workspace[j]), "fst_wn_wgrad_reduce_many: workspaces must be 16-byte aligned");
+    WwParams p = {};
+    const int lastj = kind[j] == 1 && last[j];
+    ww_geometry(kind[j], B, L, n, h, lastj, n_sets[j], &p);
+    FST_REQUIRE(workspace_floats[j] >= (int64_t)p.ksplit * WW_MROWS * (p.Kcols + 2),
+                "fst_wn_wgrad_reduce_many: workspace %d of %lld floats is too small", j, (long long)workspace_floats[j]);
+    if (kind[j] == 0) ww_in_segments(p, n, h, L, 4, 0);
+    else ww_rs_segments(p, n, L, lastj);
+    WwRedEntry& e = rp.e[j];
+    e.slab = workspace[j];
+    e.slab_extra = workspace[j] + (long long)p.ksplit * WW_MROWS * p.Kcols;
+    e.w[0] = dw0[j]; e.w[1] = kind[j] == 0 ? dw1[j] : nullptr;
+    e.ksplit = p.ksplit; e.Kcols = p.Kcols; e.K_main = p.K_main; e.K = p.K; e.n_extra = p.n_extra; e.M = p.M; e.n_x = p.n_x;
+    for (int i = 0; i < p.n_x; ++i) e.x[i] = {p.x[i].rows, p.x[i].out, p.x[i].out_off, p.x[i].out_sc, p.x[i].out_sm};
+    e.quad_blocks = (p.M * (p.Kcols / 4) + 63) / 64;
+    const unsigned blocks = (unsigned)e.quad_blocks + (unsigned)((p.K_main < p.K ? p.M * p.n_extra : 0) + 255) / 256;
+    if (blocks > gx) gx = blocks;
+  }
+  hipLaunchKernelGGL(wn_wgrad_reduce_many_kernel, dim3(gx, 1, (unsigned)n_entries), dim3(256), 0, (hipStream_t)stream, rp);
+  FST_LAUNCH_CHECK();
+  return 0;
 }
 
 extern "C" int64_t fst_nt_gemm_workspace_floats(int M, int N, int K) {
diff --git a/feature_level_style_transfer_for_tsc_amd/ops.py b/feature_level_style_transfer_for_tsc_amd/ops.py
--- a/feature_level_style_transfer_for_tsc_amd/ops.py
+++ b/feature_level_style_transfer_for_tsc_amd/ops.py
@@ -872,7 +872,7 @@
     return list(x) if isinstance(x, (list, tuple)) else [x]
 
 
-def wn_wgrad_in(dg, a, u0, dw_in: Tensor, dw_cond: Tensor, n: int, h: int, dil: int) -> None:
+def wn_wgrad_in(dg, a, u0, dw_in: Tensor, dw_cond: Tensor, n: int, h: int, dil: int, slabs: Optional[list] = None) -> None:
     lib = _lib.load()
     dgs, as_, u0s = _sets(dg), _sets(a), _sets(u0)
     if not (1 <= len(dgs) <= WN_WGRAD_MAX_SETS and len(as_) == len(dgs) and len(u0s) == len(dgs)):
@@ -894,13 +894,18 @@
     ws = torch.empty(ws_n, device=dgs[0].device, dtype=torch.float32)
     ns = len(dgs)
     t0 = KERNEL_TIMER.begin() if KERNEL_TIMER is not None else None
-    check(lib.fst_wn_wgrad_in(_ptr_sets(dgs), _ptr_sets(as_), _ptr_sets(u0s), ns, u0_bs, ptr(dw_in), ptr(dw_cond), ptr(ws), ws_n, B, L,
-                              n, h, dil, int(slack), numel, stream_ptr()), "fst_wn_wgrad_in")
+    if slabs is not None:
+        check(lib.fst_wn_wgrad_in_slabs(_ptr_sets(dgs), _ptr_sets(as_), _ptr_sets(u0s), ns, u0_bs, ptr(ws), ws_n, B, L, n, h, dil,
+                                        int(slack), numel, stream_ptr()), "fst_wn_wgrad_in_slabs")
+        slabs.append((0, False, ns, ws, dw_in, dw_cond))
+    else:
+        check(lib.fst_wn_wgrad_in(_ptr_sets(dgs), _ptr_sets(as_), _ptr_sets(u0s), ns, u0_bs, ptr(dw_in), ptr(dw_cond), ptr(ws), ws_n,
+                                  B, L, n, h, dil, int(slack), numel, stream_ptr()), "fst_wn_wgrad_in")
     if t0 is not None:
         KERNEL_TIMER.end("wn_wgrad_kernel<2, 3> bf3", t0, 2.0 * ns * B * L * 2 * n * (3 * n + h), 4.0 * ns * B * L * (2 * n + n + h))
 
 
-def wn_wgrad_rs(d_a, d_out, ts, dw_rs: Tensor, last: bool, n: int) -> None:
+def wn_wgrad_rs(d_a, d_out, ts, dw_rs: Tensor, last: bool, n: int, slabs: Optional[list] = None) -> None:
     lib = _lib.load()
     d_outs, tss = _sets(d_out), _sets(ts)
     d_as = [None] * len(d_outs) if d_a is None else _sets(d_a)
@@ -918,10 +923,31 @@
     ws = torch.empty(ws_n, device=d_outs[0].device, dtype=torch.float32)
     ns = len(d_outs)
     t0 = KERNEL_TIMER.begin() if KERNEL_TIMER is not None else None
-    check(lib.fst_wn_wgrad_rs(None if last else _ptr_sets(d_as), _ptr_sets(d_outs), _ptr_sets(tss), ns, ptr(dw_rs), ptr(ws), ws_n,
-                              int(last), B, L, n, numel, stream_ptr()), "fst_wn_wgrad_rs")
+    if slabs is not None:
+        check(lib.fst_wn_wgrad_rs_slabs(None if last else _ptr_sets(d_as), _ptr_sets(d_outs), _ptr_sets(tss), ns, ptr(ws), ws_n,
+                                        int(last), B, L, n, numel, stream_ptr()), "fst_wn_wgrad_rs_slabs")
+        slabs.append((1, bool(last), ns, ws, dw_rs, None))
+    else:
+        check(lib.fst_wn_wgrad_rs(None if last else _ptr_sets(d_as), _ptr_sets(d_outs), _ptr_sets(tss), ns, ptr(dw_rs), ptr(ws), ws_n,
+                                  int(last), B, L, n, numel, stream_ptr()), "fst_wn_wgrad_rs")
     if t0 is not None:
         KERNEL_TIMER.end("wn_wgrad_kernel<2, 2> bf3", t0, 2.0 * ns * B * L * M * n, 4.0 * ns * B * L * (M + 2 * n))
+
+
+WN_WGRAD_MAX_REDUCE = 16
+
+
+def wn_wgrad_reduce_many(slabs: list, B: int, L: int, n: int, h: int) -> None:
+    lib = _lib.load()
+    for c0 in range(0, len(slabs), WN_WGRAD_MAX_REDUCE):
+        chunk = slabs[c0: c0 + WN_WGRAD_MAX_REDUCE]
+        ne = len(chunk)
+        ints = lambda vals: (ctypes.c_int32 * ne)(*[int(v) for v in vals])
+        check(lib.fst_wn_wgrad_reduce_many(ints(e[0] for e in chunk), ints(e[1] for e in chunk), ints(e[2] for e in chunk),
+                                           _ptr_table([e[3] for e in chunk]), (ctypes.c_int64 * ne)(*[e[3].numel() for e in chunk]),
+                                           _ptr_table([e[4] for e in chunk]), _ptr_table([e[5] for e in chunk]), ne, B, L, n, h,
+                                           stream_ptr()), "fst_wn_wgrad_reduce_many")
+    del slabs[:]
 
 
 def dense_tap_wgrad(dy: Tensor, x: Tensor, dw: Tensor, M: int, C: int, K: int, pad_left: int) -> None:
@@ -1003,6 +1029,7 @@
         nl, n, h = S.n_layers, S.n, S.h
         dw = S.unflatten(g)
         g_cond_w, g_in_w, g_rs_w = dw[2], dw[6: 6 + nl], dw[6 + 2 * nl: 6 + 3 * nl]
+        slabs, later, BL = [], [], None
         for (kind, i), sets in pending.items():
             for c0 in range(0, len(sets), WN_WGRAD_MAX_SETS):
                 chunk = sets[c0: c0 + WN_WGRAD_MAX_SETS]
@@ -1011,16 +1038,21 @@
                     t_in, t_cond = g_in_w[i], g_cond_w[2 * n * i: 2 * n * (i + 1)]
                     if c0:
                         t_in, t_cond = torch.empty_like(t_in), torch.empty_like(t_cond)
-                    wn_wgrad_in(cols[0], cols[1], cols[2], t_in, t_cond, n, h, 2 ** i)
-                    if c0:
-                        g_in_w[i].add_(t_in)
-                        g_cond_w[2 * n * i: 2 * n * (i + 1)].add_(t_cond)
+                        later += [(g_in_w[i], t_in), (g_cond_w[2 * n * i: 2 * n * (i + 1)], t_cond)]
+                    wn_wgrad_in(cols[0], cols[1], cols[2], t_in, t_cond, n, h, 2 ** i, slabs=None if c0 else slabs)
+                    BL = (cols[0][0].size(0), cols[0][0].size(2))
                 else:
                     last = i == nl - 1
-                    t_rs = torch.empty_like(g_rs_w[i]) if c0 else g_rs_w[i]
-                    wn_wgrad_rs(None if last else cols[0], cols[1], cols[2], t_rs, last, n)
+                    t_rs = g_rs_w[i]
                     if c0:
-                        g_rs_w[i].add_(t_rs)
+                        t_rs = torch.empty_like(t_rs)
+                        later.append((g_rs_w[i], t_rs))
+                    wn_wgrad_rs(None if last else cols[0], cols[1], cols[2], t_rs, last, n, slabs=None if c0 else slabs)
+                    BL = (cols[1][0].size(0), cols[1][0].size(2))
+        if slabs:
+            wn_wgrad_reduce_many(slabs, BL[0], BL[1], n, h)
+        for seg, t in later:
+            seg.add_(t)
         return None, None, g
 
 
@@ -1131,6 +1163,71 @@
     return img
 
 
+WN_PACK_MAX_LAYERS = 10
+
+
+def _pack_stack(keys, nl: int, launch_one, launch_stack, keep):
+    if _PACK_CACHE is not None:
+        hits = [_PACK_CACHE.get(k) for k in keys]
+        if all(hit is not None for hit in hits):
+            return [hit[0] for hit in hits]
+    if nl > WN_PACK_MAX_LAYERS or (_PACK_CACHE is not None and any(hit is not None for hit in hits)):
+        return [launch_one(i) for i in range(nl)]
+    imgs = launch_stack()
+    if _PACK_CACHE is not None:
+        for i, (k, img) in enumerate(zip(keys, imgs)):
+            _PACK_CACHE[k] = keep(i, img)
+    return imgs
+
+
+def wn_pack_layers(layers: Sequence[Sequence[Tensor]], n: int, h: int) -> List[Tensor]:
+    lib, nl = _lib.load(), len(layers)
+    for in_w in (l[0] for l in layers):
+        if in_w.dim() != 3 or in_w.size(0) != 2 * n or in_w.size(1) != n:
+            raise ValueError(f"wn_pack_layers: in_w must be [2n, n, taps], got {tuple(in_w.shape)} for n={n}")
+    keys = [("wn", n, h, i == nl - 1) + tuple((t.data_ptr(), t._version) for t in layers[i]) for i in range(nl)]
+    src = [[t.contiguous() for t in l] for l in layers]
+
+    def launch_stack():
+        nbytes = lib.fst_wn_image_bytes(n, h)
+        imgs = [torch.empty(nbytes // 4, device=src[0][0].device, dtype=torch.float32) for _ in range(nl)]
+        check(lib.fst_wn_pack_stack(*[_ptr_table([l[j] for l in src]) for j in range(6)], nl, n, h, layers[0][0].size(2),
+                                    _ptr_table(imgs), nbytes, stream_ptr()), "fst_wn_pack_stack")
+        return imgs
+    return _pack_stack(keys, nl, lambda i: wn_pack_layer(*layers[i], n, h, i == nl - 1), launch_stack,
+                       lambda i, img: (img, *layers[i], src[i]))
+
+
+def wn_pack_bwd_layers(rs_ws: Sequence[Tensor], n: int, acc_order: bool = False) -> List[Tensor]:
+    lib, nl = _lib.load(), len(rs_ws)
+    keys = [("wn_bwd", n, i == nl - 1, acc_order, w.data_ptr(), w._version) for i, w in enumerate(rs_ws)]
+    src = [w.contiguous() for w in rs_ws]
+
+    def launch_stack():
+        imgs = [torch.empty(lib.fst_wn_bwd_image_bytes(n, int(i == nl - 1)) // 4, device=src[0].device, dtype=torch.float32)
+                for i in range(nl)]
+        check(lib.fst_wn_pack_bwd_stack(_ptr_table(src), nl, n, int(acc_order), _ptr_table(imgs), lib.fst_wn_bwd_image_bytes(n, 0),
+                                        stream_ptr()), "fst_wn_pack_bwd_stack")
+        return imgs
+    return _pack_stack(keys, nl, lambda i: wn_pack_bwd(rs_ws[i], n, i == nl - 1, acc_order), launch_stack,
+                       lambda i, img: (img, rs_ws[i], src[i]))
+
+
+def wn_pack_dgrad_layers(in_ws: Sequence[Tensor], cond_ws: Sequence[Tensor], n: int, h: int) -> List[Tensor]:
+    lib, nl = _lib.load(), len(in_ws)
+    keys = [("wn_dgrad", n, h, a.data_ptr(), a._version, c.data_ptr(), c._version) for a, c in zip(in_ws, cond_ws)]
+    src = [(a.contiguous(), c.contiguous()) for a, c in zip(in_ws, cond_ws)]
+
+    def launch_stack():
+        nbytes = lib.fst_wn_dgrad_image_bytes(n)
+        imgs = [torch.empty(nbytes // 4, device=src[0][0].device, dtype=torch.float32) for _ in range(nl)]
+        check(lib.fst_wn_pack_dgrad_stack(_ptr_table([s_[0] for s_ in src]), _ptr_table([s_[1] for s_ in src]), nl, n, h,
+                                          in_ws[0].size(2), _ptr_table(imgs), nbytes, stream_ptr()), "fst_wn_pack_dgrad_stack")
+        return imgs
+    return _pack_stack(keys, nl, lambda i: wn_pack_dgrad(in_ws[i], cond_ws[i], n, h), launch_stack,
+                       lambda i, img: (img, in_ws[i], cond_ws[i], src[i]))
+
+
 def wn_layer_fwd(a: Tensor, u0: Tensor, img: Tensor, ts: Tensor, acts: Optional[Tensor], a_next: Optional[Tensor], out: Tensor,
                  first: bool, last: bool, n: int, h: int, dil: int) -> None:
     lib = _lib.load()
@@ -1344,7 +1441,7 @@
     fused = wn_fused_ok(n, h, L, a, u0, kernel=S.kernel)
     if fused:
         out = torch.empty(B, n, L, device=dev, dtype=torch.float32)
-        imgs = [wn_pack_layer(*_wn_layer(S, W, i), n, h, i == nl - 1) for i in range(nl)]
+        imgs = wn_pack_layers([_wn_layer(S, W, i) for i in range(nl)], n, h)
         a_list = [a] + [empty_with_slack(B, n, L, dev) for _ in range(nl - 1)]
         ts_list = [torch.empty(B, 2 * n, L, device=dev, dtype=torch.float32) for _ in range(nl)]
         if wn_stack_fwd_ok(n, h, L, nl, B):
@@ -1449,8 +1546,8 @@
 def _wn_backward_stack(S: WNSpecs, W, G, a_list, ts_list, u0: Tensor, d_out: Tensor, d_u0: Tensor, pool):
     nl, n, h = S.n_layers, S.n, S.h
     B, _, L = d_out.shape
-    imgs_b = [wn_pack_bwd(_wn_layer(S, W, i)[4], n, i == nl - 1, acc_order=True) for i in range(nl)]
-    imgs_d = [wn_pack_dgrad(*_wn_layer(S, W, i)[:2], n, h) for i in range(nl)]
+    imgs_b = wn_pack_bwd_layers([_wn_layer(S, W, i)[4] for i in range(nl)], n, acc_order=True)
+    imgs_d = wn_pack_dgrad_layers([_wn_layer(S, W, i)[0] for i in range(nl)], [_wn_layer(S, W, i)[1] for i in range(nl)], n, h)
     new = lambda *shape: torch.empty(*shape, device=d_out.device, dtype=torch.float32)
     if G is None:
         dgs, da_out = [new(B, 2 * n, L)] * nl, [new(B, n, L)] + [None] * (nl - 1)
diff --git a/include/fst_hip.h b/include/fst_hip.h
--- a/include/fst_hip.h
+++ b/include/fst_hip.h
@@ -7,7 +7,7 @@
 extern "C" {
 #endif
 
-#define FST_ABI_VERSION 16
+#define FST_ABI_VERSION 17
 
 int fst_version(void);
 const char* fst_last_error(void);
@@ -107,6 +107,13 @@
 int64_t fst_wn_image_bytes(int n, int h);
 int fst_wn_pack(const float* in_w, const float* cond_w, const float* in_b, const float* cond_b,
                 const float* rs_w, const float* rs_b, int n, int h, int ntaps , int last, void* image, int64_t image_bytes, void* stream);
+int fst_wn_pack_stack(const float* const* in_w, const float* const* cond_w, const float* const* in_b, const float* const* cond_b,
+                      const float* const* rs_w, const float* const* rs_b, int nl, int n, int h, int ntaps, void* const* images,
+                      int64_t image_bytes, void* stream);
+int fst_wn_pack_bwd_stack(const float* const* rs_w, int nl, int n, int acc_order, void* const* images, int64_t image_bytes,
+                          void* stream);
+int fst_wn_pack_dgrad_stack(const float* const* in_w, const float* const* cond_w, int nl, int n, int h, int ntaps,
+                            void* const* images, int64_t image_bytes, void* stream);
 int fst_wn_layer_fwd(const float* a, int64_t a_bs, const float* u0, int64_t u0_bs, const void* image, int64_t image_bytes,
                      float* ts, float* acts, float* a_next, float* out, int first, int last,
                      int B, int L, int n, int h, int dil, int64_t numel_a, void* stream);
@@ -147,6 +154,14 @@
 int fst_wn_wgrad_rs(const float* const* d_a , const float* const* d_out, const float* const* ts, int n_sets,
                     float* dw_rs, float* workspace, int64_t workspace_floats, int last, int B, int L, int n, int64_t numel_a,
                     void* stream);
+int fst_wn_wgrad_in_slabs(const float* const* dg, const float* const* a, const float* const* u0, int n_sets, int64_t u0_bs,
+                          float* workspace, int64_t workspace_floats, int B, int L, int n, int h, int dil, int a_slack,
+                          int64_t numel_a, void* stream);
+int fst_wn_wgrad_rs_slabs(const float* const* d_a , const float* const* d_out, const float* const* ts, int n_sets,
+                          float* workspace, int64_t workspace_floats, int last, int B, int L, int n, int64_t numel_a, void* stream);
+int fst_wn_wgrad_reduce_many(const int32_t* kind, const int32_t* last, const int32_t* n_sets, float* const* workspace,
+                             const int64_t* workspace_floats, float* const* dw0, float* const* dw1, int n_entries, int B, int L,
+                             int n, int h, void* stream);
 
 int64_t fst_nt_gemm_workspace_floats(int M, int N, int K);
 int fst_nt_gemm(const float* A, const float* Bm, float* C, float* workspace, int64_t workspace_floats, int M, int N, int K,
```
